# tum-pbs/DMCF

Measured on AMD Instinct MI355X. Metric: rollout_particle_steps_per_sec, higher is better.
Workload: dtype f32

## Files before the change

dmcf_amd/_lib.py:

```python
import ctypes
import os
import subprocess

_PKG = os.path.dirname(os.path.abspath(__file__))
LIB_PATH = os.path.join(_PKG, "libdmcf_hip.so")
_lib = None


class DmcfError(RuntimeError):
    pass


class CconvArgs(ctypes.Structure):
    _fields_ = [
        ("filters", ctypes.c_void_p),
        ("filter_dims", ctypes.c_int32 * 5),
        ("sym_axis", ctypes.c_int32),
        ("out_positions", ctypes.c_void_p),
        ("n_out", ctypes.c_int64),
        ("inp_positions", ctypes.c_void_p),
        ("n_inp", ctypes.c_int64),
        ("inp_features", ctypes.c_void_p),
        ("inp_importance", ctypes.c_void_p),
        ("neighbors_index", ctypes.c_void_p),
        ("neighbors_row_splits", ctypes.c_void_p),
        ("neighbors_value", ctypes.c_void_p),
        ("extent", ctypes.c_float),
        ("window_fac", ctypes.c_float),
        ("window", ctypes.c_int32),
        ("coordinate_mapping", ctypes.c_int32),
        ("interpolation", ctypes.c_int32),
        ("flags", ctypes.c_int32),
        ("bias", ctypes.c_void_p),
        ("out", ctypes.c_void_p),
        ("n_pairs", ctypes.c_int64),
        ("neighbors_row_count", ctypes.c_void_p),
        ("filter_tile_mask", ctypes.c_uint32),
        ("row_length_hint", ctypes.c_int32),
    ]


class CconvBackwardArgs(ctypes.Structure):
    _fields_ = [
        ("struct_size", ctypes.c_uint32),
        ("flags", ctypes.c_int32),
        ("grad_out", ctypes.c_void_p),
        ("inv_index", ctypes.c_void_p),
        ("inv_pair", ctypes.c_void_p),
        ("inv_row_splits", ctypes.c_void_p),
        ("inv_n_rows", ctypes.c_int64),
        ("inv_n_pairs", ctypes.c_int64),
        ("grad_filters", ctypes.c_void_p),
        ("grad_inp_features", ctypes.c_void_p),
    ]


class NeighborDenseArgs(ctypes.Structure):
    _fields_ = [
        ("struct_size", ctypes.c_uint32),
        ("flags", ctypes.c_int32),
        ("x", ctypes.c_void_p),
        ("n_in", ctypes.c_int64),
        ("cin", ctypes.c_int32),
        ("cout", ctypes.c_int32),
        ("kernel", ctypes.c_void_p),
        ("bias", ctypes.c_void_p),
        ("residual", ctypes.c_void_p),
        ("mask", ctypes.c_void_p),
        ("neighbors_index", ctypes.c_void_p),
        ("neighbors_row_splits", ctypes.c_void_p),
        ("neighbors_row_count", ctypes.c_void_p),
        ("n_out", ctypes.c_int64),
        ("n_pairs", ctypes.c_int64),
        ("host_row_splits", ctypes.c_void_p),
        ("out", ctypes.c_void_p),
        ("record_s", ctypes.c_void_p),
        ("record_count", ctypes.c_void_p),
    ]


class NeighborDenseBackwardArgs(ctypes.Structure):
    _fields_ = [
        ("struct_size", ctypes.c_uint32),
        ("flags", ctypes.c_int32),
        ("x", ctypes.c_void_p),
        ("n_in", ctypes.c_int64),
        ("cin", ctypes.c_int32),
        ("cout", ctypes.c_int32),
        ("kernel", ctypes.c_void_p),
        ("grad_out", ctypes.c_void_p),
        ("n_out", ctypes.c_int64),
# ... 63 lines not shown
        ("bias", ctypes.c_void_p),
        ("out", ctypes.c_void_p),
        ("error_flag", ctypes.c_void_p),
    ]


class AdamTensor(ctypes.Structure):
    _fields_ = [
        ("param", ctypes.c_void_p),
        ("grad", ctypes.c_void_p),
        ("m", ctypes.c_void_p),
        ("v", ctypes.c_void_p),
        ("n", ctypes.c_int64),
    ]


class AdamArgs(ctypes.Structure):
    _fields_ = [
        ("struct_size", ctypes.c_uint32),
        ("n_tensors", ctypes.c_int32),
        ("tensors", ctypes.c_void_p),
        ("device_tensors", ctypes.c_void_p),
        ("lr", ctypes.c_float),
        ("beta_1", ctypes.c_float),
        ("beta_2", ctypes.c_float),
        ("epsilon", ctypes.c_float),
        ("beta_1_power", ctypes.c_float),
        ("beta_2_power", ctypes.c_float),
        ("clip_norm", ctypes.c_float),
        ("reserved", ctypes.c_int32),
    ]


class Sph1dParams(ctypes.Structure):
    _fields_ = [
        ("struct_size", ctypes.c_uint32),
        ("bcnt", ctypes.c_int32),
        ("max_iter", ctypes.c_int32),
        ("reserved", ctypes.c_int32),
        ("h", ctypes.c_double),
        ("rest_dens", ctypes.c_double),
        ("stiffness", ctypes.c_double),
        ("visc", ctypes.c_double),
        ("gravity", ctypes.c_double),
        ("dt", ctypes.c_double),
        ("eps", ctypes.c_double),
    ]


SYMBOLS = [
    "dmcf_version", "dmcf_error_string", "dmcf_last_hip_error",
    "dmcf_frs_workspace_bytes", "dmcf_frs_build", "dmcf_frs_count", "dmcf_frs_write", "dmcf_frs_search_padded", "dmcf_frs_window_sum",
    "dmcf_radius_search_count", "dmcf_radius_search_write",
    "dmcf_cconv_workspace_bytes", "dmcf_cconv_forward", "dmcf_cconv_kernel_name",
    "dmcf_cconv_forward_extents", "dmcf_cconv_extents_kernel_name",
    "dmcf_invert_neighbors_list_workspace_bytes", "dmcf_invert_neighbors_list",
    "dmcf_cconv_backward_workspace_bytes", "dmcf_cconv_backward", "dmcf_cconv_backward_kernel_names",
    "dmcf_cconv_backward_extents", "dmcf_cconv_backward_extents_kernel_names",
    "dmcf_cconv_scatter_plan_bytes", "dmcf_cconv_scatter_plan", "dmcf_cconv_scatter_workspace_bytes", "dmcf_cconv_scatter_forward",
    "dmcf_lattice_conv_workspace_bytes", "dmcf_lattice_conv_forward",
    "dmcf_lattice_conv_batch_workspace_bytes", "dmcf_lattice_conv_forward_batch",
    "dmcf_lattice_conv_backward_workspace_bytes", "dmcf_lattice_conv_backward",
    "dmcf_reduce_subarrays_sum", "dmcf_points_aabb_workspace_bytes", "dmcf_points_aabb", "dmcf_dense_forward",
    "dmcf_fps_workspace_bytes", "dmcf_farthest_point_sample", "dmcf_gather_point",
    "dmcf_grid_pos_workspace_bytes", "dmcf_grid_pos_bounds", "dmcf_grid_pos_count", "dmcf_grid_pos_write",
    "dmcf_ghost_workspace_bytes", "dmcf_ghost_count", "dmcf_ghost_write",
    "dmcf_nn_distance_workspace_bytes", "dmcf_nn_distance", "dmcf_approx_match_workspace_bytes", "dmcf_approx_match",
    "dmcf_match_cost_workspace_bytes", "dmcf_match_cost", "dmcf_emd_workspace_bytes", "dmcf_emd",
    "dmcf_neighbor_dense_forward", "dmcf_neighbor_dense_backward_workspace_bytes", "dmcf_neighbor_dense_backward",
    "dmcf_neighbor_dense_kernel_names", "dmcf_adam_step_workspace_bytes", "dmcf_adam_step", "dmcf_adam_step_kernel_names",
    "dmcf_raster_workspace_bytes", "dmcf_raster_count", "dmcf_raster_discs",
    "dmcf_nn_distance_backward_workspace_bytes", "dmcf_nn_distance_backward", "dmcf_match_cost_backward_workspace_bytes",
    "dmcf_match_cost_backward", "dmcf_emd_with_levels", "dmcf_emd_backward_workspace_bytes", "dmcf_emd_backward",
    "dmcf_gather_point_backward_workspace_bytes", "dmcf_gather_point_backward",
    "dmcf_frs_window_sum_backward",
    "dmcf_sph1d_rollout",
]


def build(force=False):
    csrc = os.path.join(_PKG, "csrc")
    args = ["make", "-C", csrc, "-j4"]
    if force:
        args.append("-B")
    subprocess.check_call(args, stdout=subprocess.DEVNULL)
    return LIB_PATH


def lib():
    global _lib
    if _lib is not None:
        return _lib
    if not os.path.exists(LIB_PATH):
        raise DmcfError(
            f"{LIB_PATH} is missing: the HIP extension has not been built "
            "(run `python -c 'import __graft_entry__ as g; g.build()'`). There is no CPU fallback.")
    L = ctypes.CDLL(LIB_PATH)
    c = ctypes
    L.dmcf_version.restype = c.c_int
    L.dmcf_error_string.restype = c.c_char_p
    L.dmcf_error_string.argtypes = [c.c_int]
    L.dmcf_last_hip_error.restype = c.c_int
    L.dmcf_frs_workspace_bytes.restype = c.c_size_t
    L.dmcf_frs_workspace_bytes.argtypes = [c.c_int64, c.c_int64]
    L.dmcf_frs_build.restype = c.c_int
    L.dmcf_frs_build.argtypes = [c.c_void_p, c.c_int64, c.c_float, c.c_void_p, c.c_size_t, c.c_void_p]
    L.dmcf_frs_count.restype = c.c_int
    L.dmcf_frs_count.argtypes = [c.c_void_p, c.c_int64, c.c_int64, c.c_float, c.c_int, c.c_void_p, c.c_size_t,
                                 c.c_void_p, c.c_void_p]
    L.dmcf_frs_write.restype = c.c_int
    L.dmcf_frs_write.argtypes = [c.c_void_p, c.c_int64, c.c_int64, c.c_float, c.c_int, c.c_void_p, c.c_size_t,
                                 c.c_void_p, c.c_void_p, c.c_void_p, c.c_int64, c.c_void_p]
    L.dmcf_frs_search_padded.restype = c.c_int
    L.dmcf_frs_search_padded.argtypes = [c.c_void_p, c.c_int64, c.c_int64, c.c_float, c.c_int, c.c_void_p, c.c_size_t, c.c_int64,
                                         c.c_void_p, c.c_void_p, c.c_void_p, c.c_void_p, c.c_void_p, c.c_void_p]
    L.dmcf_frs_window_sum.restype = c.c_int
    L.dmcf_frs_window_sum.argtypes = [c.c_void_p, c.c_int64, c.c_int64, c.c_float, c.c_int, c.c_int, c.c_void_p, c.c_size_t,
                                      c.c_void_p, c.c_void_p]
    L.dmcf_radius_search_count.restype = c.c_int
    L.dmcf_radius_search_count.argtypes = [c.c_void_p, c.c_int64, c.c_int64, c.c_void_p, c.c_float, c.c_int, c.c_void_p, c.c_size_t,
                                           c.c_void_p, c.c_void_p]
    L.dmcf_radius_search_write.restype = c.c_int
    L.dmcf_radius_search_write.argtypes = [c.c_void_p, c.c_int64, c.c_int64, c.c_void_p, c.c_float, c.c_int, c.c_void_p, c.c_size_t,
                                           c.c_void_p, c.c_void_p, c.c_void_p, c.c_int64, c.c_void_p]
    L.dmcf_cconv_workspace_bytes.restype = c.c_size_t
    L.dmcf_cconv_workspace_bytes.argtypes = [c.POINTER(CconvArgs)]
    L.dmcf_cconv_forward.restype = c.c_int
    L.dmcf_cconv_forward.argtypes = [c.POINTER(CconvArgs), c.c_void_p, c.c_size_t, c.c_void_p]
    L.dmcf_cconv_kernel_name.restype = c.c_int
    L.dmcf_cconv_kernel_name.argtypes = [c.POINTER(CconvArgs), c.c_char_p, c.c_size_t]
    L.dmcf_cconv_forward_extents.restype = c.c_int
    L.dmcf_cconv_forward_extents.argtypes = [c.POINTER(CconvArgs), c.c_void_p, c.c_void_p, c.c_size_t, c.c_void_p]
    L.dmcf_cconv_extents_kernel_name.restype = c.c_int
    L.dmcf_cconv_extents_kernel_name.argtypes = [c.POINTER(CconvArgs), c.c_char_p, c.c_size_t]
    L.dmcf_invert_neighbors_list_workspace_bytes.restype = c.c_size_t
    L.dmcf_invert_neighbors_list_workspace_bytes.argtypes = [c.c_int64]
    L.dmcf_invert_neighbors_list.restype = c.c_int
    L.dmcf_invert_neighbors_list.argtypes = [c.c_int64, c.c_void_p, c.c_void_p, c.c_void_p, c.c_int64, c.c_int64, c.c_void_p,
                                             c.c_void_p, c.c_void_p, c.c_void_p, c.c_void_p, c.c_void_p, c.c_size_t, c.c_void_p]
    L.dmcf_cconv_backward_workspace_bytes.restype = c.c_size_t
    L.dmcf_cconv_backward_workspace_bytes.argtypes = [c.POINTER(CconvArgs), c.POINTER(CconvBackwardArgs)]
    L.dmcf_cconv_backward.restype = c.c_int
    L.dmcf_cconv_backward.argtypes = [c.POINTER(CconvArgs), c.POINTER(CconvBackwardArgs), c.c_void_p, c.c_size_t, c.c_void_p]
    L.dmcf_cconv_backward_kernel_names.restype = c.c_int
    L.dmcf_cconv_backward_kernel_names.argtypes = [c.POINTER(CconvArgs), c.POINTER(CconvBackwardArgs), c.c_char_p, c.c_size_t]
    L.dmcf_cconv_backward_extents.restype = c.c_int
    L.dmcf_cconv_backward_extents.argtypes = [c.POINTER(CconvArgs), c.POINTER(CconvBackwardArgs), c.c_void_p, c.c_void_p, c.c_size_t,
                                              c.c_void_p]
    L.dmcf_cconv_backward_extents_kernel_names.restype = c.c_int
    L.dmcf_cconv_backward_extents_kernel_names.argtypes = [c.POINTER(CconvArgs), c.POINTER(CconvBackwardArgs), c.c_char_p, c.c_size_t]
    L.dmcf_cconv_scatter_plan_bytes.restype = c.c_size_t
    L.dmcf_cconv_scatter_plan_bytes.argtypes = [c.c_int64]
    L.dmcf_cconv_scatter_plan.restype = c.c_int
    L.dmcf_cconv_scatter_plan.argtypes = [c.c_void_p, c.c_int64, c.c_void_p, c.c_int64, c.c_float, c.c_float, c.c_int32, c.c_void_p,
                                          c.c_size_t, c.c_void_p]
    L.dmcf_cconv_scatter_workspace_bytes.restype = c.c_size_t
    L.dmcf_cconv_scatter_workspace_bytes.argtypes = [c.POINTER(CconvScatterArgs)]
    L.dmcf_cconv_scatter_forward.restype = c.c_int
    L.dmcf_cconv_scatter_forward.argtypes = [c.POINTER(CconvScatterArgs), c.c_void_p, c.c_size_t, c.c_void_p]
    L.dmcf_lattice_conv_workspace_bytes.restype = c.c_size_t
    L.dmcf_lattice_conv_workspace_bytes.argtypes = [c.POINTER(LatticeConvArgs)]
    L.dmcf_lattice_conv_forward.restype = c.c_int
    L.dmcf_lattice_conv_forward.argtypes = [c.POINTER(LatticeConvArgs), c.c_void_p, c.c_size_t, c.c_void_p]
    L.dmcf_lattice_conv_batch_workspace_bytes.restype = c.c_size_t
    L.dmcf_lattice_conv_batch_workspace_bytes.argtypes = [c.POINTER(LatticeConvArgs), c.c_int32]
    L.dmcf_lattice_conv_forward_batch.restype = c.c_int
    L.dmcf_lattice_conv_forward_batch.argtypes = [c.POINTER(LatticeConvArgs), c.c_int32, c.c_void_p, c.c_size_t, c.c_void_p]
    L.dmcf_lattice_conv_backward_workspace_bytes.restype = c.c_size_t
    L.dmcf_lattice_conv_backward_workspace_bytes.argtypes = [c.POINTER(LatticeConvArgs), c.c_int32]
    L.dmcf_lattice_conv_backward.restype = c.c_int
    L.dmcf_lattice_conv_backward.argtypes = [c.POINTER(LatticeConvArgs), c.c_int32, c.c_void_p, c.c_void_p, c.c_void_p, c.c_void_p,
                                             c.c_size_t, c.c_void_p]
    L.dmcf_dense_forward.restype = c.c_int
    L.dmcf_dense_forward.argtypes = [c.c_void_p, c.c_int64, c.c_int32, c.c_void_p, c.c_int32, c.c_void_p, c.c_void_p, c.c_void_p,
                                     c.c_void_p]
    L.dmcf_ghost_workspace_bytes.restype = c.c_size_t
    L.dmcf_ghost_workspace_bytes.argtypes = [c.c_int64, c.c_int32, c.c_int32]
    L.dmcf_ghost_count.restype = c.c_int
    L.dmcf_ghost_count.argtypes = [c.c_void_p, c.c_int64, c.c_void_p, c.c_int32, c.c_void_p, c.c_int32, c.c_void_p, c.c_void_p,
                                   c.c_size_t, c.c_void_p]
    L.dmcf_ghost_write.restype = c.c_int
    L.dmcf_ghost_write.argtypes = [c.c_void_p, c.c_int64, c.c_void_p, c.c_int32, c.c_void_p, c.c_int32, c.c_void_p, c.c_void_p,
                                   c.c_void_p, c.c_void_p, c.c_size_t, c.c_void_p]
# ... 98 lines not shown
```

dmcf_amd/csrc/cconv.hip:

```cpp
#include <type_traits>

#include <stdio.h>

#include "cconv_common.h"

namespace dmcf {

constexpr int kThreads = 512;
constexpr int kWaves = kThreads / 64;
constexpr int TM = 16;
constexpr int kMaxNT = 4;
constexpr int kWStride = 8;
constexpr int kFStride = 8;
constexpr int kStage = 64 * (kWStride + kFStride + 1);


template <int CC, bool GENERIC>
__global__ __launch_bounds__(kThreads, 4) void cconv_kernel(const CconvParams p) {
    constexpr bool EXT = false;
    const float* const out_ext = nullptr;
#include "cconv_generic_body.inc"
}

template <int CC>
// ... 73 lines not shown
        const size_t kcp = KCx + ((4 - KCx % 64) + 64) % 64;
        size_t bf = (size_t)TM * kcp;
        const size_t rf = (size_t)kWaves * TM * 16 * ((cout + 15) / 16);
        if (bf < rf) bf = rf;
        return (bf + TM + (size_t)kWaves * kStage + (has_dead ? 2 * kThreads : 0)) * sizeof(float);
    };
    const int PS0 = (PR + 7) / 8 * 8;
    const size_t step = lds_bytes(PS0) <= 80 * 1024 ? 80 * 1024 : 160 * 1024;
    int best = PS0, best_bad = 1 << 30, best_group = 0;
    for (int zgroup = 0; zgroup < 2 && best_bad > 0; ++zgroup)
        for (int k = 0; k < 12; ++k) {
            const int PS = PS0 + 8 * k;
            if (k > 0 && (sz < 2 || lds_bytes(PS) > step)) break;
            const int bad = conflicts(PS, zgroup);
            if (bad < best_bad) { best_bad = bad; best = PS; best_group = zgroup; }
            if (bad == 0) break;
        }
    c.PS = best;
    c.zgroup = best_group;
    const int KC = (sz * c.PS + 15) / 16 * 16;
    c.nblocks = KC / 16;
    c.KCp = KC + ((4 - KC % 64) + 64) % 64;
    c.NT = (cout + 15) / 16;
    c.nchunks = (cin + c.CC - 1) / c.CC;
    size_t b_floats = (size_t)TM * c.KCp;
    const size_t red_floats = (size_t)kWaves * TM * 16 * c.NT;
    if (b_floats < red_floats) b_floats = red_floats;
    c.bfloats = b_floats;
    c.lds = lds_bytes(c.PS);
    c.packed_floats = (size_t)c.nchunks * c.nblocks * 4 * c.NT * 16 * 4;
    return c;
}

}

using namespace dmcf;

extern "C" {

static int validate(const dmcf_cconv_args* a, bool forward = true) {
    if (!a) return DMCF_EINVAL;
    for (int d = 0; d < 5; ++d)
        if (a->filter_dims[d] < 1) return DMCF_EINVAL;
    if (a->n_out < 0 || a->n_inp < 0) return DMCF_EINVAL;
    if (!(a->extent > 0.0f)) return DMCF_EINVAL;
    if (a->window < DMCF_WINDOW_NONE || a->window > DMCF_WINDOW_CUBIC_GRAD) return DMCF_EINVAL;
    if (a->coordinate_mapping < 0 || a->coordinate_mapping > 2) return DMCF_EINVAL;
    if (a->interpolation < 0 || a->interpolation > 2) return DMCF_EINVAL;
    if (a->flags & DMCF_FLAG_SYMMETRIC) {
        if (a->sym_axis < 0 || a->sym_axis > 2) return DMCF_EINVAL;
        if (a->n_inp < a->n_out) return DMCF_EINVAL;
    }
    if (a->filter_dims[4] > 16 * kMaxNT) return DMCF_EUNSUPPORTED;
    if (a->n_out > 0) {
        if (!a->out_positions || !a->neighbors_row_splits) return DMCF_EINVAL;
        if (forward && (!a->filters || !a->out || !a->inp_features)) return DMCF_EINVAL;
        if (a->window == DMCF_WINDOW_EXPLICIT && !a->neighbors_value) return DMCF_EINVAL;
    }
    return DMCF_OK;
}

static void full_dims(const dmcf_cconv_args* a, int& dz, int& dy, int& dx) {
    dz = a->filter_dims[0]; dy = a->filter_dims[1]; dx = a->filter_dims[2];
    if (a->flags & DMCF_FLAG_SYMMETRIC) {
        if (a->sym_axis == 0) dz *= 2;
        if (a->sym_axis == 1) dy *= 2;
        if (a->sym_axis == 2) dx *= 2;
    }
}

static void fill_params(const dmcf_cconv_args* a, int dz, int dy, int dx, CconvParams& p) {
    p.partial = nullptr;
    p.csplit = 0;
    p.cin = a->filter_dims[3];
    p.cout = a->filter_dims[4];
    p.sx = dx; p.sy = dy; p.sz = dz;
    p.K = dx * dy * dz;
    p.out_pos = a->out_positions;
    p.inp_pos = a->inp_positions;
    p.inp_feat = a->inp_features;
    p.inp_imp = a->inp_importance;
    p.idx = a->neighbors_index;
    p.rs = a->neighbors_row_splits;
    p.cnt = a->neighbors_row_count;
    p.wmask = (a->filter_tile_mask && a->filter_dims[3] <= 32 && a->filter_dims[4] <= 64) ? a->filter_tile_mask : 0xffffffffu;
    p.nval = a->neighbors_value;
    p.n_out = a->n_out;
    p.n_inp = a->n_inp;
    p.pair_cap = a->n_pairs;
    p.inv_extent = 1.0f / a->extent;
    const float radius = 0.5f * a->extent;
    p.inv_r2 = 1.0f / (radius * radius);
    p.window_fac = a->window_fac;
    p.window = a->window;
    p.mapping = a->coordinate_mapping;
    p.interp = a->interpolation;
    p.flags = a->flags;
    p.bias = a->bias;
    p.out = a->out;
}

static void generic_pick(const dmcf_cconv_args* a, int dz, int dy, int dx, bool ext, CconvPick& k) {
    const LaunchCfg cfg = make_cfg(dx, dy, dz, a->filter_dims[3], a->filter_dims[4]);
    const bool generic = !cconv_specialised(a);
    CconvKernel f;
    if (ext)
// ... 3 lines not shown
    else
        f = {generic ? (const void*)cconv_kernel<4, true> : (const void*)cconv_kernel<4, false>, "cconv_kernel<4>"};
    k = {f.fn, f.name, cfg.lds, kThreads, cfg.packed_floats};
}

static int generic_launch(CconvParams p, const dmcf_cconv_args* a, int dz, int dy, int dx, const CconvPick& k, const float* out_ext,
                          void* workspace, hipStream_t stream) {
    const LaunchCfg cfg = make_cfg(dx, dy, dz, p.cin, p.cout);
    if (cfg.lds > 160 * 1024) return DMCF_EUNSUPPORTED;
    float* packed = (float*)workspace;
    const unsigned g = (unsigned)((cfg.packed_floats + 255) / 256);
    if (out_ext || !(a->flags & DMCF_FLAG_FILTER_PACKED))
        hipLaunchKernelGGL(pack_filter, dim3(g < 2048u ? g : 2048u), dim3(256), 0, stream, a->filters, packed, dz, dy, dx,
                           p.cin, p.cout, cfg.CC, cfg.PS, cfg.nchunks, cfg.nblocks, cfg.NT,
                           (a->flags & DMCF_FLAG_SYMMETRIC) ? 1 : 0, a->sym_axis);
    p.Wp = packed;
    p.KCp = cfg.KCp;
    p.PS = cfg.PS;
    p.zgroup = cfg.zgroup;
    p.nblocks = cfg.nblocks;
    p.NT = cfg.NT;
    p.nchunks = cfg.nchunks;
    p.bfloats = (int)cfg.bfloats;
    if (!cconv_set_tiles(p, TM)) return DMCF_EUNSUPPORTED;
    void* kargs[] = {(void*)&p, (void*)&out_ext};
    return cconv_launch_kernel(k, dim3((unsigned)p.tiles_per_xcd * 8u), kargs, stream);
}

static const CconvForm generic_form = {
    0, [](const dmcf_cconv_args*, int, int, int, bool) { return true; },
    [](const dmcf_cconv_args* a, int dz, int dy, int dx, CconvPick& k) { generic_pick(a, dz, dy, dx, false, k); },
    [](const dmcf_cconv_args* a, int dz, int dy, int dx, bool) {
        return make_cfg(dx, dy, dz, a->filter_dims[3], a->filter_dims[4]).packed_floats;
    },
    [](CconvParams p, const dmcf_cconv_args* a, int dz, int dy, int dx, const CconvPick& k, void* workspace, hipStream_t stream) {
        return generic_launch(p, a, dz, dy, dx, k, nullptr, workspace, stream);
    }};

static const CconvForm* const kForms[] = {&cconv_direct_form, &cconv_ws_form,  &cconv_pair_form, &cconv_p16_form, &cconv_z3_form,
                                          &cconv_cls_form,    &cconv_blk_form, &cconv_mfma_form, &generic_form};

static bool form_accepts(const CconvForm& f, const dmcf_cconv_args* a, int dz, int dy, int dx, int forced) {
    if (f.key && forced >= 0 && forced != f.key) return false;
    return f.eligible(a, dz, dy, dx, forced >= 0);
}

static int cconv_select(const dmcf_cconv_args* a, int dz, int dy, int dx, const CconvForm*& form, CconvPick& k) {
    const int forced = cconv_forced_key();
    for (const CconvForm* f : kForms) {
        if (!form_accepts(*f, a, dz, dy, dx, forced)) continue;
        if ((a->flags & DMCF_FLAG_SKIP_SELF) && f != &cconv_direct_form) return DMCF_EUNSUPPORTED;
        form = f;
        f->pick(a, dz, dy, dx, k);
        return DMCF_OK;
    }
    return DMCF_EUNSUPPORTED;
}

size_t dmcf_cconv_workspace_bytes(const dmcf_cconv_args* a) {
    if (!a || validate(a) != DMCF_OK) return 256;
    int dz, dy, dx;
    full_dims(a, dz, dy, dx);
    const int forced = cconv_forced_key();
    size_t floats = 0;
    for (const CconvForm* f : kForms) {
        const size_t ff = f->workspace_floats(a, dz, dy, dx, form_accepts(*f, a, dz, dy, dx, forced));
        if (floats < ff) floats = ff;
    }
    return 256 + align_up(floats * sizeof(float), 256);
}

int dmcf_cconv_forward(const dmcf_cconv_args* a, void* workspace, size_t workspace_bytes, dmcf_stream_t stream_) {
    int rc = validate(a);
    if (rc != DMCF_OK) return rc;
    if (a->n_out == 0) return DMCF_OK;
    if (!workspace || ((uintptr_t)workspace & 255)) return DMCF_EINVAL;
    if (workspace_bytes < dmcf_cconv_workspace_bytes(a)) return DMCF_EWORKSPACE;

    CconvParams p;
    int dz, dy, dx;
    full_dims(a, dz, dy, dx);
    fill_params(a, dz, dy, dx, p);
    const CconvForm* form;
    CconvPick k;
    rc = cconv_select(a, dz, dy, dx, form, k);
    if (rc != DMCF_OK) return rc;
    return form->launch(p, a, dz, dy, dx, k, workspace, (hipStream_t)stream_);
}

static int validate_extents(const dmcf_cconv_args* a, const float* out_extents, dmcf_cconv_args& b) {
    if (!a) return DMCF_EINVAL;
    b = *a;
    b.extent = 1.0f;
    const int rc = validate(&b);
    if (rc != DMCF_OK) return rc;
    if (a->flags & DMCF_FLAG_SKIP_SELF) return DMCF_EUNSUPPORTED;
    if (a->n_out > 0 && !out_extents) return DMCF_EINVAL;
    return DMCF_OK;
}

int dmcf_cconv_forward_extents(const dmcf_cconv_args* a, const float* out_extents, void* workspace, size_t workspace_bytes,
                               dmcf_stream_t stream_) {
    hipStream_t stream = (hipStream_t)stream_;
    dmcf_cconv_args b;
    const int rc = validate_extents(a, out_extents, b);
    if (rc != DMCF_OK) return rc;
    if (b.n_out == 0) return DMCF_OK;
    if (!workspace || ((uintptr_t)workspace & 255)) return DMCF_EINVAL;
    if (workspace_bytes < dmcf_cconv_workspace_bytes(&b)) return DMCF_EWORKSPACE;
    CconvParams p;
    int dz, dy, dx;
    full_dims(&b, dz, dy, dx);
    fill_params(&b, dz, dy, dx, p);
    CconvPick k;
    generic_pick(&b, dz, dy, dx, true, k);
    return generic_launch(p, &b, dz, dy, dx, k, out_extents, workspace, stream);
}

int dmcf_cconv_kernel_name(const dmcf_cconv_args* a, char* name, size_t name_bytes) {
    if (!name || name_bytes < 2) return DMCF_EINVAL;
    int rc = validate(a, false);
    if (rc != DMCF_OK) return rc;
    int dz, dy, dx;
    full_dims(a, dz, dy, dx);
    const CconvForm* form;
    CconvPick k;
    rc = cconv_select(a, dz, dy, dx, form, k);
    if (rc != DMCF_OK) return rc;
    snprintf(name, name_bytes, "%s", k.name);
    return DMCF_OK;
}

int dmcf_cconv_extents_kernel_name(const dmcf_cconv_args* a, char* name, size_t name_bytes) {
    if (!name || name_bytes < 2 || !a) return DMCF_EINVAL;
    dmcf_cconv_args b = *a;
    b.extent = 1.0f;
    const int rc = validate(&b, false);
    if (rc != DMCF_OK) return rc;
    if (a->flags & DMCF_FLAG_SKIP_SELF) return DMCF_EUNSUPPORTED;
    int dz, dy, dx;
    full_dims(&b, dz, dy, dx);
    CconvPick k;
    generic_pick(&b, dz, dy, dx, true, k);
    snprintf(name, name_bytes, "%s", k.name);
    return DMCF_OK;
}

}
```

dmcf_amd/csrc/cconv_cls.hip:

```cpp

#include "cconv_common.h"

namespace dmcf {

constexpr int kCWaves = 8;
constexpr int kCThreads = 64 * kCWaves;
constexpr int CTM = 2 * kCWaves;
constexpr int kCRows = 16;
constexpr int CCH = 16;
constexpr int kCRow = 1024;
constexpr int kSlots = 96;
constexpr int kHalfSlots = 48;
constexpr int kGrp = 20;
constexpr int kXst = 512;
constexpr int kCMaxNT = 4;
constexpr int kNoPair = 9;

#define CLS_TILE_REGS                                                                                                     \
    "v92", "v93", "v94", "v95", "v96", "v97", "v98", "v99", "v100", "v101", "v102", "v103", "v104", "v105", "v106", "v107", \
        "v108", "v109", "v110", "v111", "v112", "v113", "v114", "v115", "v116", "v117", "v118", "v119", "v120", "v121",    \
        "v122", "v123", "v124", "v125", "v126", "v127"
constexpr int kClsCompilerVgprs = 46;

__device__ __forceinline__ void cls_zero_tiles() {
    asm volatile(
        "v_mov_b32 v92, 0\n\tv_mov_b32 v93, 0\n\tv_mov_b32 v94, 0\n\tv_mov_b32 v95, 0\n\t"
        "v_mov_b32 v96, 0\n\tv_mov_b32 v97, 0\n\tv_mov_b32 v98, 0\n\tv_mov_b32 v99, 0\n\t"
        "v_mov_b32 v100, 0\n\tv_mov_b32 v101, 0\n\tv_mov_b32 v102, 0\n\tv_mov_b32 v103, 0\n\t"
        "v_mov_b32 v104, 0\n\tv_mov_b32 v105, 0\n\tv_mov_b32 v106, 0\n\tv_mov_b32 v107, 0\n\t"
        "v_mov_b32 v108, 0\n\tv_mov_b32 v109, 0\n\tv_mov_b32 v110, 0\n\tv_mov_b32 v111, 0\n\t"
        "v_mov_b32 v112, 0\n\tv_mov_b32 v113, 0\n\tv_mov_b32 v114, 0\n\tv_mov_b32 v115, 0\n\t"
        "v_mov_b32 v116, 0\n\tv_mov_b32 v117, 0\n\tv_mov_b32 v118, 0\n\tv_mov_b32 v119, 0\n\t"
        "v_mov_b32 v120, 0\n\tv_mov_b32 v121, 0\n\tv_mov_b32 v122, 0\n\tv_mov_b32 v123, 0\n\t"
        "v_mov_b32 v124, 0\n\tv_mov_b32 v125, 0\n\tv_mov_b32 v126, 0\n\tv_mov_b32 v127, 0"
        ::: "memory", CLS_TILE_REGS);
}

struct ClsRec {
    float x;
    f32x4 w;
};

__device__ __forceinline__ uint32_t cls_lds_addr(const void* q) {
    return (uint32_t)(uintptr_t)(const __attribute__((address_space(3))) void*)q;
}

__device__ __forceinline__ void xfence() {
    __builtin_amdgcn_fence(__ATOMIC_RELEASE, "wavefront");
    __builtin_amdgcn_wave_barrier();
    __builtin_amdgcn_fence(__ATOMIC_ACQUIRE, "wavefront");
}

template <int NTT, bool NARROW, bool SYM, bool SINGLE, bool PLAIN>
__global__ __launch_bounds__(kCThreads, 4) __attribute__((amdgpu_num_vgpr(kClsCompilerVgprs))) void cconv_cls_kernel(const CconvParams p) {
    extern __shared__ __attribute__((aligned(16))) float smem[];
    const int tid = threadIdx.x, lane = tid & 63;
    const int wave = __builtin_amdgcn_readfirstlane(tid >> 6);
    const int cin = p.cin, cout = p.cout;
    float* Bt = smem;
    float* Gs = smem + CTM * kCRow + wave * kXst;
    unsigned char* Cst = (unsigned char*)(Gs + 24 * kGrp);
    float* Fst = Bt + (wave + kCWaves) * kCRow;
    int* Jst = (int*)(Fst + kHalfSlots * 16);
    const int tile = (int)(blockIdx.x % 8) * p.tiles_per_xcd + (int)(blockIdx.x / 8);
    if (tile >= p.ntiles) return;
    const int64_t pt0 = (int64_t)tile * CTM;
    const int window = PLAIN ? (int)DMCF_WINDOW_POLY6 : p.window;
    const float* const nval = PLAIN ? nullptr : p.nval;
    const float* const imp = PLAIN ? nullptr : p.inp_imp;
    constexpr bool symmetric = SYM;

    const int mk = lane >> 4, mn = lane & 15;
    const float xm = (float)(lane & 3);
    const int widx = (lane >> 2) & 3;
    const int mi = lane & 15, mg = lane >> 4;
    const uint32_t gs_lds = cls_lds_addr(Gs), fst_lds = cls_lds_addr(Fst);
    constexpr uint32_t kOob = 0xffffffffu;
    const uint32_t rowB = (uint32_t)cin * 4u;
    const __amdgpu_buffer_rsrc_t rF = __builtin_amdgcn_make_buffer_rsrc((void*)p.inp_feat, 0, (int)((uint32_t)p.n_inp * rowB), 0x00020000);

    f32x4 acc[NTT];
#pragma unroll
    for (int n = 0; n < NTT; ++n) acc[n] = (f32x4){0.0f, 0.0f, 0.0f, 0.0f};

    float out_prev = 0.0f;
    for (int chunk = 0; chunk < p.nchunks; ++chunk) {
        const int c0 = chunk * CCH;
        const int nch = min(CCH, cin - c0);
        constexpr bool narrow = NARROW;
        const int fr = narrow ? lane >> 1 : lane >> 2, fc4 = narrow ? lane & 1 : lane & 3;
        const int spi = narrow ? 32 : 16;
        const int fstride = narrow ? 8 : 16;
        const bool fch_ok = c0 + 4 * fc4 < cin;
        const int fch = fch_ok ? c0 + 4 * fc4 : 0;
        int64_t rbs[2];
        int nts[2], nbs[2];
        float oxs[2], oys[2], ozs[2];
#pragma unroll
        for (int pp = 0; pp < 2; ++pp) {
            const int64_t i = pt0 + wave + kCWaves * pp;
            rbs[pp] = 0;
            nts[pp] = 0;
            oxs[pp] = oys[pp] = ozs[pp] = 0.0f;
            if (i < p.n_out) {
                const int64_t rb = p.rs[i];
                int64_t re = p.cnt ? rb + p.cnt[i] : p.rs[i + 1];
                if (re > p.pair_cap) re = rb;
                rbs[pp] = rb;
                nts[pp] = (int)min(re - rb, (int64_t)0x7fffffc0);
                oxs[pp] = p.out_pos[3 * i];
                oys[pp] = p.out_pos[3 * i + 1];
                ozs[pp] = p.out_pos[3 * i + 2];
            }
            nbs[pp] = (nts[pp] + 63) >> 6;
        }
        const int nbA = nbs[0], NB = nbs[0] + nbs[1];
        cls_zero_tiles();

        const int nt0 = __builtin_amdgcn_readfirstlane(nts[0]), nt1 = __builtin_amdgcn_readfirstlane(nts[1]);
        const int64_t rb0 = ((int64_t)__builtin_amdgcn_readfirstlane((int)(rbs[0] >> 32)) << 32) | (uint32_t)__builtin_amdgcn_readfirstlane((int)rbs[0]);
        const int64_t rb1 = ((int64_t)__builtin_amdgcn_readfirstlane((int)(rbs[1] >> 32)) << 32) | (uint32_t)__builtin_amdgcn_readfirstlane((int)rbs[1]);
        const int64_t gapB = nt1 > 0 ? rb1 - rb0 : 0;
        const bool near = gapB >= 0 && gapB + nt1 < ((int64_t)1 << 29) && nt0 < (1 << 29);
        const __amdgpu_buffer_rsrc_t rI = __builtin_amdgcn_make_buffer_rsrc(
            (void*)(p.idx + rb0), 0, near ? (int)(max((int64_t)nt0, gapB + nt1) * 4) : 0, 0x00020000);
        const uint32_t offB = (uint32_t)gapB * 4u;
        auto valid = [&](int t) -> bool {
            const bool pp = t >= nbA;
            return t < NB && 64 * (t - (pp ? nbA : 0)) + lane < (pp ? nt1 : nt0);
        };
        auto ld_idx = [&](int t, int& j, float& nv) {
            const bool pp = t >= nbA, ok = valid(t);
            const int o = 64 * (t - (pp ? nbA : 0)) + lane;
            j = 0;
            nv = 0.0f;
            if (near) {
                j = (int)__builtin_amdgcn_raw_buffer_load_b32(rI, ok ? (uint32_t)o * 4u + (pp ? offB : 0u) : kOob, 0, 0);
            } else if (ok) {
                j = p.idx[(pp ? rb1 : rb0) + o];
            }
            if (nval && ok) nv = nval[(pp ? rb1 : rb0) + o];
        };
        auto ld_pos = [&](int j, float& x, float& y, float& z) {
            const float* q = (const float*)((const char*)p.inp_pos + (size_t)__umul24((uint32_t)j, 12u));
            x = q[0];
            y = q[1];
            z = q[2];
        };
        auto geom = [&](int t, int j, float nv, float x, float y, float z, int& cls) -> ClsRec {
            ClsRec c;
            const bool pp = t >= nbA;
            x -= pp ? oxs[1] : oxs[0];
            y -= pp ? oys[1] : oys[0];
            z -= pp ? ozs[1] : ozs[0];
            float a = window_value(window, nval ? nv : rel_dist2(x, y, z), p.inv_r2, p.window_fac);
            if (imp) a *= imp[j];
            filter_coords<false>(x, y, z, p);
            c.x = fminf(3.0f, fmaxf(0.0f, x));
            y = fminf(3.0f, fmaxf(0.0f, y));
            z = fminf(3.0f, fmaxf(0.0f, z));
            const float yf = fminf(floorf(y), 2.0f), zf = fminf(floorf(z), 2.0f);
            const float fy = y - yf, fz = z - zf;
            cls = valid(t) ? 3 * (int)zf + (int)yf : kNoPair;
            const float a0 = a * (1.0f - fz), a1 = a * fz;
            c.w = (f32x4){a0 * (1.0f - fy), a0 * fy, a1 * (1.0f - fy), a1 * fy};
            return c;
        };
        struct Order {
            int pos;
            int cb[10];
        };
        auto order = [&](int cls) -> Order {
            Order o;
            o.pos = 0;
            int base = 0;
#pragma unroll
            for (int c = 0; c < 9; ++c) {
                const uint64_t m = __ballot(cls == c);
                const int rank = __builtin_amdgcn_mbcnt_hi((uint32_t)(m >> 32), __builtin_amdgcn_mbcnt_lo((uint32_t)m, base));
                o.pos = cls == c ? rank : o.pos;
                o.cb[c] = base;
                base += (__builtin_popcountll(m) + 3) & ~3;
            }
            o.cb[9] = base;
            return o;
        };
        auto push_index = [&](int j, int cls, int pos) {
            Jst[lane] = -1;
            if (lane < kSlots - 64) Jst[64 + lane] = -1;
            xfence();
            if (cls != kNoPair) Jst[pos] = (int)__umul24((uint32_t)j, rowB);
        };
        auto push_rec = [&](const ClsRec& c, int cls, int pos) {
            *(f32x4*)(Gs + 4 * lane) = (f32x4){0.0f, 0.0f, 0.0f, 0.0f};
            if (lane < kGrp * 6 - 64) *(f32x4*)(Gs + 4 * (64 + lane)) = (f32x4){0.0f, 0.0f, 0.0f, 0.0f};
            xfence();
            if (cls != kNoPair) {
                float* g = Gs + (pos >> 2) * kGrp + (pos & 3);
                g[16] = c.x;
                *(f32x4*)(g + 3 * (pos & 3)) = c.w;
                if ((pos & 3) == 0) Cst[pos >> 2] = (unsigned char)(4 * cls);
            }
        };
        const uint32_t cbyte = fch_ok ? 4u * (uint32_t)fch : kOob;
        auto f_issue = [&](int h, f32x4 (&f)[3]) {
            uint32_t jo[3];
#pragma unroll
            for (int k = 0; k < 3; ++k) jo[k] = (uint32_t)Jst[kHalfSlots * h + spi * k + fr];
#pragma unroll
            for (int k = 0; k < 3; ++k)
// ... 44 lines not shown
            __builtin_amdgcn_s_setprio(3);
            asm volatile(
#include "cconv_cls_splat8.inc"
                : [xa] "=&v"(xa), [wa] "=&v"(wa), [fa] "=&v"(fa), [xb] "=&v"(xb), [wb] "=&v"(wb), [fb] "=&v"(fb),
                  [a] "=&v"(av), [sc] "=&s"(sc)
                : [px] "v"(px), [pw] "v"(pw), [pf] "v"(pf), [xm] "v"(xm), [ng] "s"(ng), [c0] "s"(c[0]), [c1] "s"(c[1]),
                  [c2] "s"(c[2]), [c3] "s"(c[3]), [c4] "s"(c[4]), [c5] "s"(c[5])
                : "scc", "m0", "memory", CLS_TILE_REGS);
            __builtin_amdgcn_s_setprio(0);
        };
        auto merge = [&](int pt) {
            float* Brow = Bt + pt * kCRow;
            const int gz = lane >> 5, gy = (lane >> 4) & 1;
            const int col = (mn ^ (pt & 15)) << 2;
            const uint32_t mb = cls_lds_addr(Brow + (gz * 4 + gy) * 64 + col);
            xfence();
            asm volatile(
                "s_nop 7\n\ts_nop 7\n\ts_nop 7\n\t"
                "ds_write_b128 %[b], v[92:95] offset:0\n\t"
                "ds_write_b128 %[b], v[100:103] offset:512\n\t"
                "ds_write_b128 %[b], v[116:119] offset:2048\n\t"
                "ds_write_b128 %[b], v[124:127] offset:2560\n\t"
                "ds_read_b128 v[92:95], %[b] offset:256\n\t"
                "s_waitcnt lgkmcnt(0)\n\t"
                "v_add_f32 v92, v92, v96\n\tv_add_f32 v93, v93, v97\n\tv_add_f32 v94, v94, v98\n\tv_add_f32 v95, v95, v99\n\t"
                "ds_write_b128 %[b], v[92:95] offset:256\n\t"
                "ds_read_b128 v[92:95], %[b] offset:2304\n\t"
                "s_waitcnt lgkmcnt(0)\n\t"
                "v_add_f32 v92, v92, v120\n\tv_add_f32 v93, v93, v121\n\tv_add_f32 v94, v94, v122\n\tv_add_f32 v95, v95, v123\n\t"
                "ds_write_b128 %[b], v[92:95] offset:2304\n\t"
                "ds_read_b128 v[92:95], %[b] offset:1024\n\t"
                "s_waitcnt lgkmcnt(0)\n\t"
                "v_add_f32 v92, v92, v104\n\tv_add_f32 v93, v93, v105\n\tv_add_f32 v94, v94, v106\n\tv_add_f32 v95, v95, v107\n\t"
                "ds_write_b128 %[b], v[92:95] offset:1024\n\t"
                "ds_read_b128 v[92:95], %[b] offset:1536\n\t"
                "s_waitcnt lgkmcnt(0)\n\t"
                "v_add_f32 v92, v92, v112\n\tv_add_f32 v93, v93, v113\n\tv_add_f32 v94, v94, v114\n\tv_add_f32 v95, v95, v115\n\t"
                "ds_write_b128 %[b], v[92:95] offset:1536\n\t"
                "ds_read_b128 v[92:95], %[b] offset:1280\n\t"
                "s_waitcnt lgkmcnt(0)\n\t"
                "v_add_f32 v92, v92, v108\n\tv_add_f32 v93, v93, v109\n\tv_add_f32 v94, v94, v110\n\tv_add_f32 v95, v95, v111\n\t"
                "ds_write_b128 %[b], v[92:95] offset:1280\n\t"
                "s_waitcnt lgkmcnt(0)"
                :
                : [b] "v"(mb)
                : "memory", CLS_TILE_REGS);
            cls_zero_tiles();
            xfence();
        };

        if (nbA == 0) merge(wave);
        if (NB > 0) {
            int jA, jB, cl;
            float nvA, nvB, px, py, pz;
            ld_idx(0, jA, nvA);
            ld_idx(1, jB, nvB);
            ld_pos(jA, px, py, pz);
            const ClsRec first = geom(0, jA, nvA, px, py, pz, cl);
            Order oc = order(cl);
            f32x4 ff[3];
            push_index(jA, cl, oc.pos);
            push_rec(first, cl, oc.pos);
            xfence();
            f_issue(0, ff);
            jA = jB;
            nvA = nvB;
            ld_pos(jA, px, py, pz);
            if constexpr (narrow) {
                for (int t = 0; t + 1 < NB; ++t) {
                    const int nslots = oc.cb[9];
                    f_publish(t, ff);
                    ld_idx(t + 2, jB, nvB);
                    const ClsRec nxt = geom(t + 1, jA, nvA, px, py, pz, cl);
                    const Order on = order(cl);
                    push_index(jA, cl, on.pos);
                    jA = jB;
                    nvA = nvB;
                    ld_pos(jA, px, py, pz);
                    xfence();
                    f_issue(0, ff);
                    splat8(nslots);
                    push_rec(nxt, cl, on.pos);
                    oc = on;
                    if (t == nbA - 1) merge(wave);
                }
                f_publish(NB - 1, ff);
                xfence();
                splat8(oc.cb[9]);
                if (NB - 1 == nbA - 1) merge(wave);
            } else {
                for (int t = 0; t + 1 < NB; ++t) {
                    const int nslots = oc.cb[9];
                    const bool two = nslots > kHalfSlots;
                    f_publish(t, ff);
                    ld_idx(t + 2, jB, nvB);
                    if (two) f_issue(1, ff);
                    xfence();
                    splat(0, nslots);
                    const ClsRec nxt = geom(t + 1, jA, nvA, px, py, pz, cl);
                    const Order on = order(cl);
                    push_index(jA, cl, on.pos);
                    xfence();
                    if (two) f_publish(t, ff);
                    jA = jB;
                    nvA = nvB;
                    ld_pos(jA, px, py, pz);
                    f_issue(0, ff);
                    if (two) {
                        xfence();
                        splat(1, nslots);
                    }
                    push_rec(nxt, cl, on.pos);
                    oc = on;
                    if (t == nbA - 1) merge(wave);
                }
                {
                    const int nslots = oc.cb[9];
                    const bool two = nslots > kHalfSlots;
                    f_publish(NB - 1, ff);
                    if (two) f_issue(1, ff);
                    xfence();
                    splat(0, nslots);
                    if (two) {
                        xfence();
                        f_publish(NB - 1, ff);
                        xfence();
                        splat(1, nslots);
                    }
                    if (NB - 1 == nbA - 1) merge(wave);
                }
            }
        }
        if (chunk == p.nchunks - 1) out_prev = epilogue_prefetch(p, pt0, CTM, tid);
        const int nq = (nch + 3) >> 2;
        constexpr int kIt = 64 / kCWaves;
        constexpr int kPre = SINGLE ? (NTT <= 1 ? 8 : (NTT <= 2 ? 4 : 2)) : (NTT <= 1 ? 4 : (NTT <= 2 ? 2 : 1));
        const __amdgpu_buffer_rsrc_t rW = __builtin_amdgcn_make_buffer_rsrc(
            (void*)p.Wp, 0, (int)((uint32_t)p.nchunks * 64u * (uint32_t)p.NT * 1024u), 0x00020000);
        const uint32_t w_lane = ((uint32_t)mg * (uint32_t)p.NT * 16u + (uint32_t)mi) * 16u;
        auto w_issue = [&](int it0, f32x4 (&bw)[kPre][NTT]) {
#pragma unroll
            for (int q = 0; q < kPre; ++q) {
                const int t = wave + kCWaves * (it0 + q);
                if (t < 16 * nq) {
                    int tq, tr;
                    blk_divmod(t, nq, tq, tr);
                    const int blk = tq * 4 + tr;
                    const uint32_t w_blk = (uint32_t)(chunk * 64 + blk) * (uint32_t)p.NT * 1024u;
                    const int wq = 4 * chunk + tr;
                    const uint32_t wm = wq < 8 ? p.wmask >> (4 * wq) : 0xfu;
#pragma unroll
                    for (int n = 0; n < NTT; ++n)
                        if (n < p.NT && ((wm >> n) & 1))
                            bw[q][n] = __builtin_bit_cast(f32x4, __builtin_amdgcn_raw_buffer_load_b128(rW, w_lane, w_blk + 256u * (uint32_t)n, 0));
                }
            }
        };
        f32x4 bw[kPre][NTT];
#pragma unroll
// ... 74 lines not shown
                       (symmetric && sym_axis == 2) ? 2 : 4};
    for (int64_t e = (int64_t)blockIdx.x * blockDim.x + threadIdx.x; e < total; e += (int64_t)gridDim.x * blockDim.x) {
        int64_t s = e;
        const int q = (int)(s & 3); s >>= 2;
        const int j = (int)(s & 15); s >>= 4;
        const int n = (int)(s % NT); s /= NT;
        const int g = (int)(s & 3); s >>= 2;
        const int blk = (int)(s & 63); s >>= 6;
        const int chunk = (int)s;
        const int ci = chunk * CCH + 4 * (blk & 3) + g, o = 16 * n + j;
        float v = 0.0f;
        if (chunk < nchunks && ci < cin && o < cout) {
            int c3[3] = {blk >> 4, (blk >> 2) & 3, q};
            float sign = 1.0f;
            if (symmetric) {
                const int hh = hd[sym_axis];
                if (c3[sym_axis] >= hh) {
                    c3[sym_axis] -= hh;
                } else {
                    sign = -1.0f;
                    for (int a = 0; a < 3; ++a) c3[a] = hd[a] - 1 - c3[a];
                }
            }
            v = sign * src[((((int64_t)c3[0] * hd[1] + c3[1]) * hd[2] + c3[2]) * cin + ci) * cout + o];
        }
        dst[e] = v;
    }
}

static bool cls_eligible(const dmcf_cconv_args* a, int dz, int dy, int dx, bool forced) {
    if (!cconv_fast444(a, dz, dy, dx) || !cconv_offsets_fit_24bit(a)) return false;
    if (a->filter_dims[4] > 16 * kCMaxNT) return false;
    if (forced) return true;
    return a->filter_dims[3] >= 8;
}

size_t cconv_cls_workspace_floats(const dmcf_cconv_args* a, int, int, int, bool) {
    return cconv_cls_packed_floats(a->filter_dims[3], a->filter_dims[4]);
}

bool cconv_cls_prepare(CconvParams& p, const dmcf_cconv_args* a, int tm, void* workspace, hipStream_t stream) {
    float* packed = (float*)workspace;
    p.NT = (p.cout + 15) / 16;
    p.nchunks = (p.cin + CCH - 1) / CCH;
    const int64_t total = (int64_t)cconv_cls_packed_floats(p.cin, p.cout);
    const unsigned g = (unsigned)((total + 255) / 256);
    if (!(a->flags & DMCF_FLAG_FILTER_PACKED))
        hipLaunchKernelGGL(pack_filter_cls, dim3(g < 2048u ? g : 2048u), dim3(256), 0, stream, a->filters, packed, p.cin, p.cout,
                           p.nchunks, p.NT, (a->flags & DMCF_FLAG_SYMMETRIC) ? 1 : 0, a->sym_axis);
    p.Wp = packed;
    return cconv_set_tiles(p, tm);
}

static void cls_pick(const dmcf_cconv_args* a, int, int, int, CconvPick& k) {
    const int cin = a->filter_dims[3], NT = (a->filter_dims[4] + 15) / 16;
    const bool sym = (a->flags & DMCF_FLAG_SYMMETRIC) != 0;
    const bool plain = !sym && cconv_plain(a);
#define CLS_PICK(NARROW, SINGLE)                                                                \
    (sym ? CCONV_KERNEL_NT(NT, cconv_cls_kernel, NARROW, true, SINGLE, false)                   \
         : (plain ? CCONV_KERNEL_NT(NT, cconv_cls_kernel, NARROW, false, SINGLE, true)          \
                  : CCONV_KERNEL_NT(NT, cconv_cls_kernel, NARROW, false, SINGLE, false)))
    const CconvKernel f = cin <= 8 ? CLS_PICK(true, true) : (cin <= CCH ? CLS_PICK(false, true) : CLS_PICK(false, false));
#undef CLS_PICK
    k = {f.fn, f.name, kClsLds, kCThreads, cconv_cls_packed_floats(cin, a->filter_dims[4])};
}

static int cls_launch(CconvParams p, const dmcf_cconv_args* a, int, int, int, const CconvPick& k, void* workspace, hipStream_t stream) {
    if (!cconv_cls_prepare(p, a, CTM, workspace, stream)) return DMCF_EUNSUPPORTED;
    void* kargs[] = {(void*)&p};
    return cconv_launch_kernel(k, dim3((unsigned)p.tiles_per_xcd * 8u), kargs, stream);
}

CconvForm cconv_cls_form = {'c', cls_eligible, cls_pick, cconv_cls_workspace_floats, cls_launch};

}
```

dmcf_amd/csrc/cconv_common.h:

```cpp
#pragma once
#include <stdlib.h>

#include "common.h"

namespace dmcf {

typedef float f32x4_t __attribute__((ext_vector_type(4)));

struct CconvParams {
    const float* Wp;
    int sx, sy, sz, K, cin, cout;
    const float* out_pos;
    const float* inp_pos;
    const float* inp_feat;
    const float* inp_imp;
    const int32_t* idx;
    const int64_t* rs;
    const int32_t* cnt;
    const float* nval;
    int64_t n_out;
    int64_t n_inp;
    int64_t pair_cap;
    float inv_extent, inv_r2, window_fac;
    int window, mapping, interp, flags;
// ... 124 lines not shown
            if (q <= 1.0f) r = (s <= 0.5f) ? 18.0f * q - 12.0f * s : -6.0f * (1.0f - s) * (1.0f - s);
            return fac * (4.0f / 3.0f) * r;
        }
    }
    return 1.0f;
}

__device__ __forceinline__ void axis_weights(float x, int s, int interp, int& b, float& w0, float& w1) {
    const int bmax = s >= 2 ? s - 2 : 0;
    if (interp == DMCF_INTERP_NEAREST) {
        int c = (int)roundf(x);
        c = min(max(c, 0), s - 1);
        b = min(c, bmax);
        w0 = (c == b) ? 1.0f : 0.0f;
        w1 = 1.0f - w0;
        return;
    }
    if (interp == DMCF_INTERP_LINEAR) {
        x = fminf((float)(s - 1), fmaxf(0.0f, x));
        const float xf = fminf(floorf(x), (float)bmax);
        b = (int)xf;
        const float a = x - xf;
        w0 = 1.0f - a;
        w1 = a;
        if (s == 1) { w0 = 1.0f; w1 = 0.0f; }
        return;
    }
    const float xf = floorf(x);
    const float a = x - xf;
    const float c0 = xf, c1 = xf + 1.0f;
    const bool in0 = c0 >= 0.0f && c0 <= (float)(s - 1), in1 = c1 >= 0.0f && c1 <= (float)(s - 1);
    const float v0 = in0 ? 1.0f - a : 0.0f, v1 = in1 ? a : 0.0f;
    if (!in0 && !in1) { b = 0; w0 = w1 = 0.0f; return; }
    if (in0 && in1) { b = (int)c0; w0 = v0; w1 = v1; return; }
    if (in0) {
        if (s >= 2) { b = s - 2; w0 = 0.0f; w1 = v0; } else { b = 0; w0 = v0; w1 = 0.0f; }
        return;
    }
    b = 0; w0 = v1; w1 = 0.0f;
}

__device__ __forceinline__ void axis_weights_linear(float x, int s, int& b, float& w0, float& w1) {
    const float bmax = (float)(s >= 2 ? s - 2 : 0);
    x = fminf((float)(s - 1), fmaxf(0.0f, x));
    const float xf = fminf(floorf(x), bmax);
    b = (int)xf;
    const float a = x - xf;
    w0 = 1.0f - a;
    w1 = a;
}

typedef float f32x4 __attribute__((ext_vector_type(4)));
typedef float f32x2 __attribute__((ext_vector_type(2)));

__device__ __forceinline__ void blk_divmod(int t, int nq, int& quot, int& rem) {
    const int m = nq == 1 ? 128 : (nq == 2 ? 64 : (nq == 3 ? 43 : 32));
    quot = (t * m) >> 7;
    rem = t - quot * nq;
}



__global__ void pack_filter(const float* __restrict__ src, float* __restrict__ dst, int d0, int d1, int d2, int cin,
                            int cout, int CC, int PS, int nchunks, int nblocks, int NT, int symmetric, int sym_axis);

__device__ __forceinline__ float epilogue_prefetch(const CconvParams& p, int64_t pt0, int pts, int tid) {
    if (!(p.flags & DMCF_FLAG_ACCUMULATE)) return 0.0f;
    const int64_t lim = min((int64_t)pts, p.n_out - pt0) * p.cout;
    return tid < lim ? p.out[pt0 * p.cout + tid] : 0.0f;
}


struct CconvPick {
    const void* fn;
    const char* name;
    size_t lds;
    int threads;
    size_t packed_floats;
};

struct CconvKernel {
    const void* fn;
    const char* name;
};
#define CCONV_KERNEL(...) CconvKernel{(const void*)__VA_ARGS__, #__VA_ARGS__}
#define CCONV_KERNEL_NT(nt, K, ...) \
    ((nt) <= 1 ? CCONV_KERNEL(K<1, __VA_ARGS__>) : ((nt) <= 2 ? CCONV_KERNEL(K<2, __VA_ARGS__>) : CCONV_KERNEL(K<4, __VA_ARGS__>)))

struct CconvForm {
    char key;
    bool (*eligible)(const dmcf_cconv_args* a, int dz, int dy, int dx, bool forced);
    void (*pick)(const dmcf_cconv_args* a, int dz, int dy, int dx, CconvPick& k);
    size_t (*workspace_floats)(const dmcf_cconv_args* a, int dz, int dy, int dx, bool selectable);
    int (*launch)(CconvParams p, const dmcf_cconv_args* a, int dz, int dy, int dx, const CconvPick& k, void* workspace,
                  hipStream_t stream);
};
extern CconvForm cconv_direct_form, cconv_ws_form, cconv_pair_form, cconv_p16_form, cconv_z3_form, cconv_cls_form,
    cconv_blk_form, cconv_mfma_form;

inline int cconv_forced_key() {
    const char* e = getenv("DMCF_CCONV_KERNEL");
    return e ? (unsigned char)e[0] : -1;
}

inline bool cconv_specialised(const dmcf_cconv_args* a) {
    return a->coordinate_mapping == DMCF_MAP_BALL_TO_CUBE_VOLUME_PRESERVING && a->interpolation == DMCF_INTERP_LINEAR &&
           (a->flags & DMCF_FLAG_ALIGN_CORNERS);
}

inline bool cconv_fast444(const dmcf_cconv_args* a, int dz, int dy, int dx) {
    return dx == 4 && dy == 4 && dz == 4 && cconv_specialised(a) && !(a->flags & DMCF_FLAG_NORMALIZE) && !(a->filter_dims[3] & 3) &&
           !((uintptr_t)a->inp_features & 15);
}

inline bool cconv_offsets_fit_24bit(const dmcf_cconv_args* a) {
    return a->n_inp < (1 << 24) && a->n_inp * (int64_t)a->filter_dims[3] * 4 < ((int64_t)1 << 31);
}

inline bool cconv_plain(const dmcf_cconv_args* a) {
    return a->window == DMCF_WINDOW_POLY6 && !a->neighbors_value && !a->inp_importance;
}

inline bool cconv_set_tiles(CconvParams& p, int tm) {
    const int64_t ntiles = (p.n_out + tm - 1) / tm;
    if (ntiles > 0x7fffffff / 8) return false;
    p.ntiles = (int)ntiles;
    p.tiles_per_xcd = (int)((ntiles + 7) / 8);
    return true;
}

inline int cconv_launch_kernel(const CconvPick& k, dim3 grid, void** kargs, hipStream_t stream) {
    hipError_t e = hipFuncSetAttribute(k.fn, hipFuncAttributeMaxDynamicSharedMemorySize, (int)k.lds);
// ... 14 lines not shown
```

dmcf_amd/csrc/cconv_ws.hip:

```cpp

#include "cconv_common.h"

namespace dmcf {

#ifdef WS_TRACE
__device__ unsigned long long g_wtrace[32];
#define WT(k) { const uint64_t now_ = __builtin_readcyclecounter(); wt[k] += now_ - wlast; wlast = now_; }
#else
#define WT(k)
#endif

constexpr int kWProd = 4, kWCons = 4;
constexpr int kWThreads = 64 * (kWProd + kWCons);
constexpr int WTM = 16;
constexpr int kWPts = WTM / kWProd;
constexpr int kWRow = 2048;
constexpr int kWRecG = 36;
constexpr int kWRec = 16 * kWRecG;
constexpr int kWWaveF = kWRec + 64 + 384;
constexpr int kWMaxNT = 2;
constexpr int kWRed = 2 * kWCons * WTM * 16 * kWMaxNT;
constexpr int kWCompilerVgprs = 56;

#define WS_FIXED_REGS                                                                                                      \
// ... 31 lines not shown
};

constexpr uint32_t kWOob = 0xffffffffu;

typedef const __attribute__((address_space(4))) CconvParams* WsKP;

__device__ __forceinline__ void ws_filter_coords(float& x, float& y, float& z, float inv_extent) {
    const float s = 2.0f * inv_extent;
    x *= s; y *= s; z *= s;
    sphere_to_cyl(x, y, z);
    cyl_to_cube(x, y);
    x *= 0.5f; y *= 0.5f; z *= 0.5f;
    x = (x + 0.5f) * 3.0f;
    y = (y + 0.5f) * 3.0f;
    z = (z + 0.5f) * 3.0f;
}

#define WS_PULL(IT, ADDR) \
    asm volatile("ds_read_b128 v[128+4*(" #IT "):128+4*(" #IT ")+3], %0" ::"v"(ADDR) : "memory", WS_FIXED_REGS)
#define WS_MFMA(IT, N, BV)                                                                                                  \
    asm volatile("v_mfma_f32_16x16x4_f32 v[112+4*" #N ":112+4*" #N "+3], v[128+4*(" #IT ")+0], %0, v[112+4*" #N ":112+4*" #N "+3]\n\t" \
                 "v_mfma_f32_16x16x4_f32 v[112+4*" #N ":112+4*" #N "+3], v[128+4*(" #IT ")+1], %1, v[112+4*" #N ":112+4*" #N "+3]\n\t" \
                 "v_mfma_f32_16x16x4_f32 v[112+4*" #N ":112+4*" #N "+3], v[128+4*(" #IT ")+2], %2, v[112+4*" #N ":112+4*" #N "+3]\n\t" \
                 "v_mfma_f32_16x16x4_f32 v[112+4*" #N ":112+4*" #N "+3], v[128+4*(" #IT ")+3], %3, v[112+4*" #N ":112+4*" #N "+3]"       \
                 :                                                                                                          \
                 : "v"((BV).x), "v"((BV).y), "v"((BV).z), "v"((BV).w)                                                      \
                 : WS_FIXED_REGS)
#define WS_MFMA2(IT, BV0, BV1)                                                                                              \
    asm volatile("v_mfma_f32_16x16x4_f32 v[112:115], v[128+4*(" #IT ")+0], %0, v[112:115]\n\t"                               \
                 "v_mfma_f32_16x16x4_f32 v[116:119], v[128+4*(" #IT ")+0], %4, v[116:119]\n\t"                               \
                 "v_mfma_f32_16x16x4_f32 v[112:115], v[128+4*(" #IT ")+1], %1, v[112:115]\n\t"                               \
                 "v_mfma_f32_16x16x4_f32 v[116:119], v[128+4*(" #IT ")+1], %5, v[116:119]\n\t"                               \
                 "v_mfma_f32_16x16x4_f32 v[112:115], v[128+4*(" #IT ")+2], %2, v[112:115]\n\t"                               \
                 "v_mfma_f32_16x16x4_f32 v[116:119], v[128+4*(" #IT ")+2], %6, v[116:119]\n\t"                               \
                 "v_mfma_f32_16x16x4_f32 v[112:115], v[128+4*(" #IT ")+3], %3, v[112:115]\n\t"                               \
                 "v_mfma_f32_16x16x4_f32 v[116:119], v[128+4*(" #IT ")+3], %7, v[116:119]"                                    \
                 :                                                                                                          \
                 : "v"((BV0).x), "v"((BV0).y), "v"((BV0).z), "v"((BV0).w), "v"((BV1).x), "v"((BV1).y), "v"((BV1).z), "v"((BV1).w) \
                 : WS_FIXED_REGS)
#define WS_ACC_READ(N, DST)                                                                                                 \
    asm volatile("v_mov_b32 %0, v[112+4*" #N "+0]\n\tv_mov_b32 %1, v[112+4*" #N "+1]\n\tv_mov_b32 %2, v[112+4*" #N "+2]\n\t"     \
                 "v_mov_b32 %3, v[112+4*" #N "+3]"                                                                          \
                 : "=v"((DST).x), "=v"((DST).y), "=v"((DST).z), "=v"((DST).w)                                             \
                 :                                                                                                          \
                 : WS_FIXED_REGS)



struct WsRing {
    int start, end, rblo, rbhi, span;
};

__device__ __forceinline__ void ws_ld_idx(int sp, int r4, int o1, int o2, int o3, const float* Tab, __amdgpu_buffer_rsrc_t rI, const float* nval,
                                          int64_t rb0, int& j, float& nv, int& kk) {
    kk = (r4 + (sp >= o1 ? 1 : 0) + (sp >= o2 ? 1 : 0) + (sp >= o3 ? 1 : 0)) & 63;
    const f32x2 ed = *(const f32x2*)(Tab + 2 * kk);
    const int e = __float_as_int(ed.x), d = __float_as_int(ed.y);
    const bool ok = sp < e;
    const uint32_t o = (uint32_t)sp * 4u + (uint32_t)d;
    j = (int)__builtin_amdgcn_raw_buffer_load_b32(rI, ok ? o : kWOob, 0, 0);
    nv = 0.0f;
    if (nval && ok) nv = nval[rb0 + (o >> 2)];
}

__device__ __forceinline__ void ws_ld_pos(const float* inp_pos, int j, float& x, float& y, float& z) {
    const float* q = (const float*)((const char*)inp_pos + (size_t)__umul24((uint32_t)j, 12u));
    x = q[0];
    y = q[1];
    z = q[2];
}

__device__ __forceinline__ WsRec ws_geom(int sp, int kk, const float* Tab, int window, const float* nval, const float* imp,
                                         float inv_r2, float window_fac, float inv_extent, int j, float nv, float x, float y, float z, bool& ok) {
    WsRec c;
    const f32x4 o = *(const f32x4*)(Tab + 128 + 4 * kk);
    ok = sp < __float_as_int(o.w);
    x -= o.x;
    y -= o.y;
    z -= o.z;
    float a = window_value(window, nval ? nv : rel_dist2(x, y, z), inv_r2, window_fac);
    if (imp) a *= imp[j];
    a = ok ? a : 0.0f;
    ws_filter_coords(x, y, z, inv_extent);
    x = fminf(3.0f, fmaxf(0.0f, x));
    y = fminf(3.0f, fmaxf(0.0f, y));
    z = fminf(3.0f, fmaxf(0.0f, z));
    const float xf = fminf(floorf(x), 2.0f), yf = fminf(floorf(y), 2.0f), zf = fminf(floorf(z), 2.0f);
    const float fx = x - xf, fy = y - yf, fz = z - zf;
    c.cls4 = ok ? 4 * (((int)zf * 3 + (int)yf) * 3 + (int)xf) : 0;
    const float a0 = a * (1.0f - fz), a1 = a * fz;
    const float y00 = (1.0f - fy) * (1.0f - fx), y01 = (1.0f - fy) * fx, y10 = fy * (1.0f - fx), y11 = fy * fx;
    c.lo = (f32x4){a0 * y00, a0 * y01, a0 * y10, a0 * y11};
    c.hi = (f32x4){a1 * y00, a1 * y01, a1 * y10, a1 * y11};
    return c;
}

__device__ __forceinline__ void ws_refill(WsKP kp0, int wi, int lane, int wave, int t_begin, int t_end, int nslots, float* Tab, int& stream_end,
                                          WsRing& ring) {
    WsKP kp = kp0;
    asm volatile("" : "+s"(kp));
    const int lb = 32 * (wi & 1);
    const bool act = (unsigned)(lane - lb) < 32u;
    const int r = 32 * wi + (lane - lb);
    const int tile = t_begin + (r >> 2) * nslots;
    const int64_t i = (int64_t)tile * WTM + kWPts * wave + (r & 3);
    int64_t rb = 0;
    int nt = 0;
    float ox = 0.0f, oy = 0.0f, oz = 0.0f;
    if (act && tile < t_end && i < kp->n_out) {
        const int64_t* const rs = kp->rs;
        const int32_t* const cnt = kp->cnt;
        const float* const out_pos = kp->out_pos;
        const int64_t b = rs[i];
        int64_t e = cnt ? b + cnt[i] : rs[i + 1];
        if (e > kp->pair_cap) e = b;
        rb = b;
        nt = (int)min(e - b, (int64_t)0x01ffffc0);
        ox = out_pos[3 * i];
        oy = out_pos[3 * i + 1];
        oz = out_pos[3 * i + 2];
    }
    const int slots = (max(nt, 1) + 7) & ~7;
    const int q = lane & 3;
    const int s1 = __shfl_up(slots, 1), s2 = __shfl_up(slots, 2), s3 = __shfl_up(slots, 3);
    const int intra = (q >= 1 ? s1 : 0) + (q >= 2 ? s2 : 0) + (q >= 3 ? s3 : 0);
    const int ttot = (__shfl(intra + slots, lane | 3) + 63) & ~63;
    int tp = 0, wtot = 0;
#pragma unroll
    for (int m = 0; m < 8; ++m) {
        const int tm = __builtin_amdgcn_readlane(ttot, lb + 4 * m);
        if (((lane - lb) >> 2) > m) tp += tm;
        wtot += tm;
    }
    const int start = stream_end + tp + intra;
    const int64_t rb0 = ((int64_t)__shfl((int)(rb >> 32), lane & ~3) << 32) | (uint32_t)__shfl((int)rb, lane & ~3);
    const int64_t gap = nt > 0 ? rb - rb0 : 0;
    if (__builtin_amdgcn_ballot_w64(act && (gap < 0 || gap + nt >= ((int64_t)1 << 29))) != 0) __builtin_trap();
    int sp = (int)gap + nt;
    sp = max(sp, __shfl_xor(sp, 1));
    sp = max(sp, __shfl_xor(sp, 2));
    if (act) {
        const int e = start + nt;
        const int d = (int)(((uint32_t)(int)gap - (uint32_t)start) * 4u);
        *(f32x2*)(Tab + 2 * lane) = (f32x2){__int_as_float(e), __int_as_float(d)};
        *(f32x4*)(Tab + 128 + 4 * lane) = (f32x4){ox, oy, oz, __int_as_float(e)};
        ring.start = start;
        ring.end = e;
        ring.rblo = (int)rb0;
        ring.rbhi = (int)(rb0 >> 32);
        ring.span = sp;
    }
    stream_end += wtot;
    wfence();
}

template <int NTT, bool PLAIN>
__global__ __launch_bounds__(kWThreads, 1) __attribute__((amdgpu_num_vgpr(kWCompilerVgprs))) void cconv_ws_kernel(const CconvParams p_arg) {
    extern __shared__ __attribute__((aligned(16))) float smem[];
    const WsKP kp0 = (WsKP)__builtin_amdgcn_kernarg_segment_ptr();
    const int tid = threadIdx.x, lane = tid & 63;
    const int wave = wsgpr(tid >> 6);
    const int cin = kp0->cin, cout = kp0->cout;
    float* Bt = smem;
    const int xcd = (int)(blockIdx.x & 7), slot = (int)(blockIdx.x >> 3), nslots = (int)(gridDim.x >> 3);
    const int t_begin = xcd * kp0->tiles_per_xcd + slot;
    const int t_end = min((xcd + 1) * kp0->tiles_per_xcd, kp0->ntiles);
    if (t_begin >= t_end) return;

    if (wave < kWProd) {
        float* Rec = smem + WTM * kWRow + wave * kWWaveF;
        uint32_t* Jof = (uint32_t*)(Rec + kWRec);
        float* Tab = Rec + kWRec + 64;
        float* Fst = Bt + (kWPts * wave + kWPts - 1) * kWRow;
        const int ch = lane & 31, half = lane >> 5;
        const int fr = lane >> 3, fq = lane & 7;
        const uint32_t rowBy = (uint32_t)cin * 4u;
        const uint32_t cbyte = 4 * fq < cin ? 16u * (uint32_t)fq : kWOob;
        const int pg = fr >> 2, ptq = fr & 3;
        float* const w01 = Fst + pg * 128 + 4 * fq + ptq;
        float* const w23 = Fst + pg * 128 + 4 * ((fq + 4) & 7) + ptq;
        const uint32_t a_rec0 = wlds(Rec + 4 * (4 * half + (lane & 3)));
        const uint32_t a_fst0 = wlds(Fst + 4 * (8 * (ch & 3) + (((ch >> 2) + 4 * ((ch >> 1) & 1)) & 7)));
        const uint32_t row_lane = wlds(Bt + (ch >> 4) * 1024 + half * 512);

        asm volatile(
            ".irp r,148,150,152,154,156,158,160,162,164,166,168,170,172,174,176,178,180,182,184,186,188,190,192,194,196,198,200,202,"
            "204,206,208,210,212,214,216,218,220,222,224,226,228,230,232,234,236,238,240,242,244,246,248,250,252,254\n\t"
            "v_mov_b64 v[\\r:\\r+1], 0\n\t.endr" ::: "memory", WS_FIXED_REGS);

        const int T = (t_end - t_begin + nslots - 1) / nslots;
        WsRing ring = {0, 0, 0, 0, 0};
        int stream_end = 0;
        ws_refill(kp0, 0, lane, wave, t_begin, t_end, nslots, Tab, stream_end, ring);
        ws_refill(kp0, 1, lane, wave, t_begin, t_end, nslots, Tab, stream_end, ring);

        WsKP kp = kp0;
        asm volatile("" : "+s"(kp));
        const int window = PLAIN ? (int)DMCF_WINDOW_POLY6 : kp->window;
        const float* const nval = PLAIN ? nullptr : kp->nval;
        const float* const imp = PLAIN ? nullptr : kp->inp_imp;
        const float inv_r2 = kp->inv_r2, window_fac = kp->window_fac, inv_extent = kp->inv_extent;
        const float* const inp_pos = kp->inp_pos;
        const int32_t* const idx = kp->idx;
        const __amdgpu_buffer_rsrc_t rF = __builtin_amdgcn_make_buffer_rsrc((void*)kp->inp_feat, 0, (int)((uint32_t)kp->n_inp * rowBy), 0x00020000);

        auto push_index = [=](int j, bool ok) { Jof[lane] = ok ? __umul24((uint32_t)j, rowBy) : kWOob; };
        auto push_rec = [=](const WsRec& c) {
            float* r = Rec + (lane >> 2) * kWRecG + (lane & 3);
            r[0] = c.lo.x; r[4] = c.lo.y; r[8] = c.lo.z; r[12] = c.lo.w;
            r[16] = c.hi.x; r[20] = c.hi.y; r[24] = c.hi.z; r[28] = c.hi.w;
        };
        int pk_cur = 0;
        auto pack_classes = [=](int cls4, uint32_t (&c)[16]) -> int {
            int pk = cls4 | (__builtin_amdgcn_mov_dpp(cls4, 0xb1, 0xf, 0xf, true) << 8);
            pk = pk | (__builtin_amdgcn_mov_dpp(pk, 0x4e, 0xf, 0xf, true) << 16);
#pragma unroll
            for (int m = 0; m < 16; ++m) c[m] = (uint32_t)__builtin_amdgcn_readlane(pk, 4 * m);
            return pk;
        };
        auto f_issue = [=](int np, f32x4 (&f)[8]) {
#pragma unroll
            for (int hh = 0; hh < 2; ++hh) {
                if (hh == 0 || np > 32) {
                    uint32_t jo[4];
#pragma unroll
                    for (int r = 0; r < 4; ++r) jo[r] = Jof[8 * (4 * hh + r) + fr];
#pragma unroll
                    for (int r = 0; r < 4; ++r)
                        f[4 * hh + r] = __builtin_bit_cast(f32x4, __builtin_amdgcn_raw_buffer_load_b128(rF, __builtin_elementwise_add_sat(jo[r], cbyte), 0, 0));
                }
            }
        };
        auto f_publish = [=](int np, const f32x4 (&f)[8]) {
#pragma unroll
            for (int r = 0; r < 8; ++r) {
                if (r < 4 || np > 32) {
                    w01[256 * r] = f[r].x;
                    w01[256 * r + 32] = f[r].y;
                    w23[256 * r + 64] = f[r].z;
                    w23[256 * r + 96] = f[r].w;
                }
            }
        };
        auto splat = [=](int nblk, const uint32_t (&c)[16], uint32_t a_rec, uint32_t a_fst) {
            uint32_t s0;
            __builtin_amdgcn_s_setprio(3);
            asm volatile(
#include "cconv_pair_splat.inc"
                : [s0] "=&s"(s0)
                : [pa] "v"(a_rec), [pf] "v"(a_fst), [nb] "s"(wsgpr(nblk)), [c0] "s"(wsgpr(c[0])), [c1] "s"(wsgpr(c[1])), [c2] "s"(wsgpr(c[2])),
                  [c3] "s"(wsgpr(c[3])), [c4] "s"(wsgpr(c[4])), [c5] "s"(wsgpr(c[5])), [c6] "s"(wsgpr(c[6])), [c7] "s"(wsgpr(c[7])),
                  [c8] "s"(wsgpr(c[8])), [c9] "s"(wsgpr(c[9])), [c10] "s"(wsgpr(c[10])), [c11] "s"(wsgpr(c[11])), [c12] "s"(wsgpr(c[12])),
                  [c13] "s"(wsgpr(c[13])), [c14] "s"(wsgpr(c[14])), [c15] "s"(wsgpr(c[15]))
                : "scc", "m0", "memory", WS_FIXED_REGS);
            __builtin_amdgcn_s_setprio(0);
        };

        int tq = 0, gq = 0, o1 = 0, o2 = 0, o3 = 0, gendq = 0, elastq = 0;
        int64_t rb0q = 0;
        __amdgpu_buffer_rsrc_t rI;
#define WS_TILE_CTX()                                                                                                        \
    {                                                                                                                        \
        const int l0_ = (4 * tq) & 63;                                                                                       \
        o1 = __builtin_amdgcn_readlane(ring.start, l0_ + 1);                                                                 \
        o2 = __builtin_amdgcn_readlane(ring.start, l0_ + 2);                                                                 \
        o3 = __builtin_amdgcn_readlane(ring.start, l0_ + 3);                                                                 \
        elastq = __builtin_amdgcn_readlane(ring.end, l0_ + 3);                                                               \
        gendq = __builtin_amdgcn_readlane(ring.start, (l0_ + 4) & 63) >> 6;                                                  \
        rb0q = ((int64_t)__builtin_amdgcn_readlane(ring.rbhi, l0_) << 32) | (uint32_t)__builtin_amdgcn_readlane(ring.rblo, l0_); \
        rI = __builtin_amdgcn_make_buffer_rsrc((void*)(idx + rb0q), 0, __builtin_amdgcn_readlane(ring.span, l0_) * 4, 0x00020000); \
    }
#define WS_IDX_STAGE(J, NV, KK, NP)                                                                                          \
    {                                                                                                                        \
        if (gq >= gendq) {                                                                                                   \
            ++tq;                                                                                                            \
            WS_TILE_CTX()                                                                                                    \
        }                                                                                                                    \
        ws_ld_idx(64 * gq + lane, 4 * tq, o1, o2, o3, Tab, rI, nval, rb0q, J, NV, KK);                                       \
        NP = max(0, min(64, elastq - 64 * gq));                                                                              \
        ++gq;                                                                                                                \
    }
        WS_TILE_CTX()

        int ti = 0;
        int rdone = 0;
        auto complete = [=, &rdone]() {
            const int row = kWPts * wave + (rdone & 3);
            const uint32_t b = row_lane + (uint32_t)row * (kWRow * 4u) + ((uint32_t)((ch & 15) ^ (row & 15)) << 4);
            asm volatile(
#include "cconv_pair_merge.inc"
                ::: "memory", WS_FIXED_REGS);
            asm volatile(
#include "cconv_ws_store.inc"
                :: [b] "v"(b) : "memory", WS_FIXED_REGS);
            asm volatile(
#include "cconv_pair_zero.inc"
                ::: "memory", WS_FIXED_REGS);
            ++rdone;
        };

#ifdef WS_TRACE
        uint64_t wt[16] = {0, 0, 0, 0, 0, 0, 0, 0, 0, 0, 0, 0, 0, 0, 0, 0};
        uint64_t wlast = __builtin_readcyclecounter();
        const uint64_t wstart = wlast;
        int nbatches = 0;
#endif
        int j1, j2, kk1, kk2, np0, np1, np2;
        float nv1, nv2, px, py, pz;
        uint32_t cc[16];
        f32x4 ff[8];
        {
            int j0, kk0;
            float nv0, qx, qy, qz;
            bool ok0;
            WS_IDX_STAGE(j0, nv0, kk0, np0)
            WS_IDX_STAGE(j1, nv1, kk1, np1)
            WS_IDX_STAGE(j2, nv2, kk2, np2)
            ws_ld_pos(inp_pos, j0, qx, qy, qz);
            ws_ld_pos(inp_pos, j1, px, py, pz);
            const WsRec first = ws_geom(lane, kk0, Tab, window, nval, imp, inv_r2, window_fac, inv_extent, j0, nv0, qx, qy, qz, ok0);
            push_index(j0, ok0);
            push_rec(first);
            pk_cur = pack_classes(first.cls4, cc);
            wfence();
            f_issue(np0, ff);
        }
        WT(0)
        WS_BARRIER();
        WT(5)
        f_publish(np0, ff);
        wfence();
        WT(6)
        int nblk_tile = (max(__builtin_amdgcn_readlane(ring.end, 3), __builtin_amdgcn_readlane(ring.start, 3) + 1) + 7) >> 3;
        int gend = __builtin_amdgcn_readlane(ring.start, 4) >> 6;
#pragma unroll 1
        for (int g = 0;; ++g) {
            const bool tile_last = g + 1 == gend;
            const bool more = !(tile_last && ti + 1 == T);
            WsRec nxt;
            int jn, kkn, npn;
            float nvn, qx, qy, qz;
            if (more) {
                bool ok1;
                nxt = ws_geom(64 * (g + 1) + lane, kk1, Tab, window, nval, imp, inv_r2, window_fac, inv_extent, j1, nv1, px, py, pz, ok1);
                push_index(j1, ok1);
                wfence();
                f_issue(np1, ff);
            }
            ws_ld_pos(inp_pos, j2, qx, qy, qz);
            WS_IDX_STAGE(jn, nvn, kkn, npn)
            WT(0)
            const int blo = 8 * g, bhi = min(8 * g + 8, nblk_tile);
            int b0 = blo;
            bool tile_done = false;
            for (;;) {
                const int gbk = (rdone & 3) == 3 ? nblk_tile : (__builtin_amdgcn_readlane(ring.start, (rdone + 1) & 63) >> 3);
                const int b1 = min(gbk, bhi);
                if (b1 > b0) {
                    const int sh = b0 - blo;
                    if (sh > 0) {
#pragma unroll
                        for (int m = 0; m < 16; ++m) cc[m] = (uint32_t)__builtin_amdgcn_readlane(pk_cur, (4 * m + 8 * sh) & 63);
                    }
                    splat(b1 - b0, cc, a_rec0 + (uint32_t)(2 * kWRecG * 4) * (uint32_t)sh, a_fst0 + 1024u * (uint32_t)sh);
                    b0 = b1;
                    WT(1)
                }
                if (gbk > bhi) break;
                const bool last_row = (rdone & 3) == 3;
                complete();
                WT(2)
                if (last_row) {
                    tile_done = true;
                    break;
                }
            }
            asm volatile("" : "+v"(jn), "+v"(nvn), "+v"(qx), "+v"(qy), "+v"(qz), "+v"(kkn));
#ifdef WS_TRACE
            ++nbatches;
#endif
            WT(7)
            if (tile_done) {
                WS_BARRIER();
                WT(3)
                ++ti;
                if ((ti & 7) == 0) ws_refill(kp0, (ti >> 3) + 1, lane, wave, t_begin, t_end, nslots, Tab, stream_end, ring);
                nblk_tile = (max(__builtin_amdgcn_readlane(ring.end, (4 * ti + 3) & 63), __builtin_amdgcn_readlane(ring.start, (4 * ti + 3) & 63) + 1) + 7) >> 3;
                gend = __builtin_amdgcn_readlane(ring.start, (4 * ti + 4) & 63) >> 6;
                WT(4)
                WS_BARRIER();
                WT(5)
            }
            if (!more) break;
            wfence();
            f_publish(np1, ff);
            push_rec(nxt);
            pk_cur = pack_classes(nxt.cls4, cc);
            j1 = j2;
            nv1 = nv2;
            kk1 = kk2;
            np1 = np2;
            j2 = jn;
            nv2 = nvn;
            kk2 = kkn;
            np2 = npn;
            px = qx;
            py = qy;
            pz = qz;
            wfence();
            WT(6)
        }
        WS_BARRIER();
#ifdef WS_TRACE
        if (lane == 0 && wave == 0 && (blockIdx.x & 15) == 0) {
            for (int k = 0; k < 8; ++k) atomicAdd(&g_wtrace[k], wt[k]);
            atomicAdd(&g_wtrace[8], wlast - wstart);
            atomicAdd(&g_wtrace[9], (unsigned long long)T);
            atomicAdd(&g_wtrace[10], (unsigned long long)nbatches);
        }
#endif
    } else {
        const int cw = wave - kWProd;
        const int ctid = tid - 64 * kWProd;
        const int mi = lane & 15, mg = lane >> 4;
        float* const red0 = smem + WTM * kWRow + kWProd * kWWaveF;
        const int red_half = kWCons * WTM * 16 * kWMaxNT;
        int tpar = 0;
        const int NT = kp0->NT, ncol = 16 * NT;
        constexpr int kRing = 8;
        const int cin_ring = (cin + kRing - 1) & ~(kRing - 1);
        const int nqt = cin >> 2;
        int a_tab, w_tab, w_next;
        {
            const int b = cw + 4 * (lane & 31);
            const int zy = b / nqt, qg = b - zy * nqt;
            const int chunk = qg >> 2, blk = zy * 4 + (qg & 3);
            const bool real = (lane & 31) < cin;
            a_tab = real ? chunk * 4096 + blk * 64 : -1;
            w_tab = real ? (chunk * 64 + blk) * NT * 1024 : 0x7fff0000;
            int nx = (lane & 31) + kRing;
            if (nx >= cin_ring) nx -= cin_ring;
            w_next = __shfl(w_tab, nx);
        }
        const __amdgpu_buffer_rsrc_t rW = __builtin_amdgcn_make_buffer_rsrc(
            (void*)kp0->Wp, 0, (int)((uint32_t)kp0->nchunks * 64u * (uint32_t)NT * 1024u), 0x00020000);
        uint32_t w_lane = ((uint32_t)mg * (uint32_t)NT * 16u + (uint32_t)mi) * 16u;
        f32x4 bw[kRing][NTT];
        uint32_t a_lane = wlds(Bt + mi * kWRow);
        const uint32_t lane_x = (uint32_t)((mg << 2) ^ (mi << 2)) << 2;
        int e_pt[NTT], e_o[NTT];
        float e_bias[NTT];
        const float* const bias = kp0->bias;
        const bool accumulate = (kp0->flags & DMCF_FLAG_ACCUMULATE) != 0;
#pragma unroll
        for (int r = 0; r < NTT; ++r) {
            const int e = ctid + 256 * r;
            e_pt[r] = e / cout;
            e_o[r] = e - e_pt[r] * cout;
            e_bias[r] = (bias && e < WTM * cout) ? bias[e_o[r]] : 0.0f;
        }
        float prev[NTT];
// ... 97 lines not shown
                WS_ACC_READ(3, acc[3 % NTT]);
            }
#pragma unroll
            for (int n = 0; n < NTT; ++n) {
                if (n < NT) {
#pragma unroll
                    for (int r = 0; r < 4; ++r) red0[tpar * red_half + (cw * 16 + 4 * mg + r) * ncol + n * 16 + mi] = acc[n][r];
                }
            }
            tpar ^= 1;
            WT(3)
        }
        WS_BARRIER();
#ifdef WS_TRACE
        if (lane == 0 && cw == 0 && (blockIdx.x & 15) == 0) {
            for (int k = 0; k < 4; ++k) atomicAdd(&g_wtrace[16 + k], wt[k]);
            atomicAdd(&g_wtrace[20], wlast - wstart);
        }
#endif
#ifndef WS_DBG_NOCONS
        reduce_store(kp0, red0 + (tpar ^ 1) * red_half);
#endif
    }
}

#ifdef WS_TRACE
}
extern "C" int dmcf_wtrace(unsigned long long* out) {
    unsigned long long z[32] = {0};
    (void)hipMemcpyFromSymbol(out, HIP_SYMBOL(dmcf::g_wtrace), sizeof(z));
    (void)hipMemcpyToSymbol(HIP_SYMBOL(dmcf::g_wtrace), z, sizeof(z));
    return 0;
}
namespace dmcf {
#endif

static constexpr size_t kWsLds = (size_t)(WTM * kWRow + kWProd * kWWaveF + kWRed) * sizeof(float);

static bool ws_eligible(const dmcf_cconv_args* a, int dz, int dy, int dx, bool forced) {
    if (!cconv_fast444(a, dz, dy, dx) || !cconv_offsets_fit_24bit(a) || (a->flags & DMCF_FLAG_SYMMETRIC)) return false;
    const int cin = a->filter_dims[3], cout = a->filter_dims[4];
    if (cin > 32 || cout > 16 * kWMaxNT) return false;
    if (forced) return true;
    return a->row_length_hint == 1 && cin >= 24;
}

static void ws_pick(const dmcf_cconv_args* a, int, int, int, CconvPick& k) {
    const int NT = (a->filter_dims[4] + 15) / 16;
    CconvKernel f;
    if (cconv_plain(a))
        f = NT <= 1 ? CCONV_KERNEL(cconv_ws_kernel<1, true>) : CCONV_KERNEL(cconv_ws_kernel<2, true>);
    else
        f = NT <= 1 ? CCONV_KERNEL(cconv_ws_kernel<1, false>) : CCONV_KERNEL(cconv_ws_kernel<2, false>);
    k = {f.fn, f.name, kWsLds, kWThreads, cconv_cls_packed_floats(a->filter_dims[3], a->filter_dims[4])};
}

static int ws_launch(CconvParams p, const dmcf_cconv_args* a, int, int, int, const CconvPick& k, void* workspace, hipStream_t stream) {
    if (!cconv_cls_prepare(p, a, WTM, workspace, stream)) return DMCF_EUNSUPPORTED;
    const int per_xcd = max(1, min(device_cu_count() / 8, p.tiles_per_xcd));
    void* kargs[] = {(void*)&p};
    return cconv_launch_kernel(k, dim3((unsigned)per_xcd * 8u), kargs, stream);
}

CconvForm cconv_ws_form = {'w', ws_eligible, ws_pick, cconv_cls_workspace_floats, ws_launch};

}
```

dmcf_amd/csrc/misc.hip:

```cpp
#include "common.h"

namespace dmcf {

thread_local int g_last_hip_error = 0;

constexpr int kScanThreads = 256;
constexpr int kScanItems = 8;
constexpr int kScanTile = kScanThreads * kScanItems;

template <typename T>
__device__ __forceinline__ T wave_inclusive_scan(T v) {
#pragma unroll
    for (int d = 1; d < kWave; d <<= 1) {
        T o = __shfl_up(v, d, kWave);
        if (lane_id() >= d) v += o;
    }
    return v;
}

template <typename T>
__device__ __forceinline__ T block_exclusive_scan(T v, T* total, T* smem ) {
    const int wave = threadIdx.x >> 6;
    const T inc = wave_inclusive_scan(v);
    if (lane_id() == kWave - 1) smem[wave] = inc;
// ... 188 lines not shown
        float* o = part + (size_t)blockIdx.x * 8;
        const bool b = fmaxf(fmaxf(red[2][a][0], red[2][a][1]), fmaxf(red[2][a][2], red[2][a][3])) > 0.0f;
        o[a] = b ? NAN : fminf(fminf(red[0][a][0], red[0][a][1]), fminf(red[0][a][2], red[0][a][3]));
        o[3 + a] = b ? NAN : fmaxf(fmaxf(red[1][a][0], red[1][a][1]), fmaxf(red[1][a][2], red[1][a][3]));
    }
}

__global__ void aabb_finish(const float* __restrict__ part, int nblocks, float* __restrict__ out) {
    const int lane = lane_id();
#pragma unroll
    for (int a = 0; a < 3; ++a) {
        float mn = INFINITY, mx = -INFINITY, b = 0.0f;
        for (int k = lane; k < nblocks; k += kWave) {
            const float lo = part[(size_t)k * 8 + a], hi = part[(size_t)k * 8 + 3 + a];
            b = fmaxf(b, lo != lo ? 1.0f : 0.0f);
            mn = fminf(mn, lo);
            mx = fmaxf(mx, hi);
        }
#pragma unroll
        for (int d = 32; d >= 1; d >>= 1) {
            mn = fminf(mn, __shfl_xor(mn, d, kWave));
            mx = fmaxf(mx, __shfl_xor(mx, d, kWave));
            b = fmaxf(b, __shfl_xor(b, d, kWave));
        }
        if (lane == 0) {
            out[a] = b > 0.0f ? NAN : mn;
            out[3 + a] = b > 0.0f ? NAN : mx;
        }
    }
}

__global__ __launch_bounds__(256) void reduce_subarrays_sum_kernel(const float* __restrict__ values,
                                                                   const int64_t* __restrict__ row_splits,
                                                                   int64_t n_rows, float* __restrict__ out) {
    const int64_t row = ((int64_t)blockIdx.x * blockDim.x + threadIdx.x) >> 4;
    const int sub = threadIdx.x & 15;
    if (row >= n_rows) return;
    const int64_t b = row_splits[row], e = row_splits[row + 1];
    float s = 0.0f;
    if (values) {
        for (int64_t k = b + sub; k < e; k += 16) s += values[k];
    } else {
        for (int64_t k = b + sub; k < e; k += 16) s += 1.0f;
    }
#pragma unroll
    for (int d = 8; d >= 1; d >>= 1) s += __shfl_xor(s, d, 16);
    if (sub == 0) out[row] = s;
}

}

extern "C" {

int dmcf_version(void) { return 21700; }

const char* dmcf_error_string(int code) {
    switch (code) {
        case DMCF_OK: return "ok";
        case DMCF_EINVAL: return "invalid argument";
        case DMCF_EWORKSPACE: return "workspace too small";
        case DMCF_ELAUNCH: return "HIP error while enqueuing (see dmcf_last_hip_error)";
        case DMCF_EUNSUPPORTED: return "option not implemented on the HIP path";
        default: return "unknown error code";
    }
}

int dmcf_last_hip_error(void) { return dmcf::g_last_hip_error; }

int dmcf_dense_forward(const float* x, int64_t n, int32_t k, const float* W, int32_t m, const float* bias,
                       const float* residual, float* out, dmcf_stream_t stream) {
    if (n < 0 || k <= 0 || m <= 0 || (n > 0 && (!x || !W || !out))) return DMCF_EINVAL;
    if ((k & 3) || k > 64 || m > 64) return DMCF_EUNSUPPORTED;
    if ((uintptr_t)x & 15) return DMCF_EUNSUPPORTED;
    if (n == 0) return DMCF_OK;
    const int64_t ntiles = (n + 15) / 16;
    const int64_t want = (ntiles + 3) / 4;
    const unsigned grid = (unsigned)(want < 2048 ? want : 2048);
    const int nt = (m + 15) / 16;
#define DMCF_DENSE(NTT)                                                                                                   \
    hipLaunchKernelGGL(dmcf::dense_rows<NTT>, dim3(grid), dim3(256), 0, (hipStream_t)stream, x, n, (int)k, W, (int)m, bias,  \
                       residual, out, ntiles)
    if (nt <= 1) DMCF_DENSE(1);
    else if (nt == 2) DMCF_DENSE(2);
    else DMCF_DENSE(4);
#undef DMCF_DENSE
    return dmcf::check_launch();
}

size_t dmcf_points_aabb_workspace_bytes(void) { return (size_t)dmcf::kAabbBlocks * 8 * sizeof(float); }

int dmcf_points_aabb(const float* points, int64_t n, float* out, void* workspace, size_t workspace_bytes,
                     dmcf_stream_t stream) {
    if (n < 0 || !out || (n > 0 && !points)) return DMCF_EINVAL;
    if (!workspace || workspace_bytes < dmcf_points_aabb_workspace_bytes()) return DMCF_EWORKSPACE;
    const int64_t want = (n + 1023) / 1024;
    const int nb = (int)(want < 1 ? 1 : (want > dmcf::kAabbBlocks ? dmcf::kAabbBlocks : want));
    hipLaunchKernelGGL(dmcf::aabb_partial, dim3(nb), dim3(256), 0, (hipStream_t)stream, points, n, (float*)workspace);
    hipLaunchKernelGGL(dmcf::aabb_finish, dim3(1), dim3(64), 0, (hipStream_t)stream, (const float*)workspace, nb, out);
    return dmcf::check_launch();
}

int dmcf_reduce_subarrays_sum(const float* values, const int64_t* row_splits, int64_t n_rows, float* out,
                              dmcf_stream_t stream) {
    if (n_rows < 0 || (n_rows > 0 && (!row_splits || !out))) return DMCF_EINVAL;
    if (n_rows == 0) return DMCF_OK;
    const int64_t threads = n_rows * 16;
    const unsigned grid = (unsigned)((threads + 255) / 256);
// ... 7 lines not shown
```

dmcf_amd/models/pbf_model.py:

```python
import os

import numpy as np
import torch

from .. import ops
from ..utils import convolutions as _convs
from ..utils.convolutions import ContinuousConv, PointSampling
from ..utils.tools.losses import (get_loss, compute_density, compute_pressure, compute_transformed_dx, get_dilated_pos,
                                  get_window_func)
from .base_model import BaseModel, Dense


def align_vector(v0, v1):
    v0n = v0 / (torch.linalg.norm(v0) + 1e-9)
    v1n = v1 / (torch.linalg.norm(v1) + 1e-9)
    v = torch.linalg.cross(v0n, v1n)
    c = torch.dot(v0n, v1n)
    s = torch.linalg.norm(v)
    if float(s) < 1e-6:
        return torch.eye(3, device=v0.device) * (-1.0 if float(c) < 0 else 1.0)
    zero = torch.zeros((), device=v0.device)
    vx = torch.stack([torch.stack([zero, -v[2], v[1]]), torch.stack([v[2], zero, -v[0]]),
                      torch.stack([-v[1], v[0], zero])])
    return torch.eye(3, device=v0.device) + vx + (vx @ vx) / (1 + c)
# ... 237 lines not shown
        if self.shard is not None:
            dilated_pos, idx = self.shard.dilated_pos(all_pos if self.use_bnds else pos)
        else:
            dilated_pos, _, idx = get_dilated_pos(all_pos if self.use_bnds else pos, self.strides,
                                                  voxel_size=self.voxel_size, centralize=self.centralize,
                                                  pad=self.sample_pad, hyst=self.sample_hyst)
        if self.dens_norm:
            dens = [(dens if self.use_bnds else dens[:pos.shape[0]]).unsqueeze(-1)]
            for scale in range(1, len(self.dens_radius)):
                d = self.sampling(dens[-1], dilated_pos[scale - 1], dilated_pos[scale], self.dens_radius[scale], None)
                dens.append(torch.clamp(d, min=1e-2))
        else:
            dens = None
        self.dilated_pos = dilated_pos
        return [dilated_pos, fluid_feats, idx, dens]

    def fused_input_operands(self, fluid_feats, box_feats):
        a, b = self.fluid_convs, self.obs_convs
        if (os.environ.get("DMCF_FUSE_INPUT_CONVS", "1") == "0" or _convs._CACHE.depth == 0 or not fluid_feats.is_cuda
                or self.recording()):
            return None
        if ops.search_set() != "distance":
            return None
        wa, wb = a.window_function, b.window_function
        if a.kernel is None or b.kernel is None:
            return None
        same = (isinstance(wa, _convs.WindowFunction) and isinstance(wb, _convs.WindowFunction) and wa.name == wb.name
                and wa.fac == wb.fac and tuple(a.kernel.shape[:3]) == tuple(b.kernel.shape[:3]) and a.filters == b.filters
                and all(getattr(a, k) == getattr(b, k) for k in (
                    "align_corners", "coordinate_mapping", "interpolation", "normalize", "use_bias",
                    "radius_search_ignore_query_points", "radius_search_metric", "use_dense_layer_for_center"))
                and not (a.symmetric or b.symmetric or a.circular or b.circular or a.normalize
                         or a.radius_search_ignore_query_points or a.use_dense_layer_for_center)
                and a.activation is None and b.activation is None
                and a.kernel.shape[3] == fluid_feats.shape[1] and b.kernel.shape[3] == box_feats.shape[1])
        if not same:
            return None
        n, m, cf, cb, co = fluid_feats.shape[0], box_feats.shape[0], fluid_feats.shape[1], box_feats.shape[1], a.filters
        cin = -(-(cf + cb) // 4) * 4
        feats = fluid_feats.new_zeros((n + m, cin))
        feats[:n, :cf] = fluid_feats * self.part_scale
        feats[n:, cf:cf + cb] = box_feats * self.part_scale
        kernel = a.kernel.new_zeros(tuple(a.kernel.shape[:3]) + (cin, 2 * co))
        kernel[..., :cf, :co] = a.kernel
        kernel[..., cf:cf + cb, co:] = b.kernel
        bias = torch.cat([a.bias, b.bias]) if a.use_bias else None
        return feats, kernel, bias

    def fused_input_conv(self, kernel, bias, feats, inp_pos, out_pos, extent):
        a = self.fluid_convs
        radius = float(np.float32(0.5) * np.float32(extent))
        nns = _convs._CACHE.search(a.fixed_radius_search, inp_pos, out_pos, radius, distances=False)
        index, row_splits, raw_dist = nns.raw()
        out = ops.cconv_forward(kernel, out_pos, extent, inp_pos, feats, index, row_splits, neighbors_value=raw_dist,
                                window=a.window_function.name, window_fac=a.window_function.fac,
                                align_corners=a.align_corners, coordinate_mapping=a.coordinate_mapping,
                                interpolation=a.interpolation, bias=bias, n_pairs_ref=_convs.pairs_ref(nns),
                                neighbors_row_count=getattr(nns, "row_count", None))
        a.nns = self.obs_convs.nns = None
        return out, nns

    def _fused_input_convs(self, fluid_feats, box_feats, pos, all_pos, extent):
        operands = self.fused_input_operands(fluid_feats, box_feats)
        if operands is None:
            return None
        feats, kernel, bias = operands
        n, co = fluid_feats.shape[0], self.fluid_convs.filters
        if self.conv_hook is not None:
            out = self.apply_conv(lambda f, pi, po, ext, _: self.fused_input_conv(kernel, bias, f, pi, po, ext)[0],
                                  feats, all_pos, all_pos, extent)
            self._fluid_counts = None
            return out[:, :co].contiguous(), out[:, co:].contiguous()
        out, nns = self.fused_input_conv(kernel, bias, feats, all_pos, all_pos, extent)
        index = nns.raw()[0]
        row_count = getattr(nns, "row_count", None)
        if row_count is not None:
            stride = nns.stride

            def count():
                rows = index[:n * stride].view(n, stride)
                cols = torch.arange(stride, device=index.device, dtype=torch.int32)
                return ((rows < n) & (cols[None, :] < row_count[:n, None])).sum(dim=1).to(torch.float32)
        else:
            idx, rs = nns.neighbors_index, nns.neighbors_row_splits

            def count():
                return ops.reduce_subarrays_sum((idx < n).to(torch.float32), rs)[:n]
        self._fluid_counts = count
        return out[:, :co].contiguous(), out[:, co:].contiguous()

    def loss_keys(self):
        return self.loss_fn.keys()

    def loss(self, results, data):
        pred, target = results[0], data[1]
        return {n: l(target, pred, num_fluid_neighbors=self.num_fluid_neighbors, input=data[0], target_prev=data[2],
                     pre_steps=data[3], pos_correction=self.pos_correction)
                for n, l in self.loss_fn.items()}

    def postprocess(self, prev, data, training=True, vel_corr=None, **kwargs):
        pos, vel, acc = data[:3]
        pcnt = pos.shape[0]
        if self.shard is not None:
            self._num_fluid_neighbors = None
        elif self.fluid_convs.nns is None and getattr(self, "_fluid_counts", None) is not None:
            self._num_fluid_neighbors = None
        else:
            counts = ops.neighbor_counts(self.fluid_convs.nns)
            self.num_fluid_neighbors = counts[:pcnt]

        out = prev
# ... 24 lines not shown
```

dmcf_amd/ops.py:

```python
import collections
import os
import ctypes

import threading

import numpy as np
import torch

from . import _lib

class NeighborCapacityExceeded(RuntimeError):
    """A search enqueued with estimated buffer sizes produced more pairs than the buffers hold."""


class NeighborSearchResult:

    def __init__(self, index_buf, row_splits, dist_buf, total=None, redo=None):
        self._index_buf, self._dist_buf = index_buf, dist_buf
        self.neighbors_row_splits = row_splits
        self._total = total
        self._redo = redo

    def raw(self):
        return self._index_buf, self.neighbors_row_splits, self._dist_buf

    def release(self):
        if self._index_buf is not None:
            self._capacity = self._index_buf.shape[0]
        self._index_buf = self._dist_buf = None
        self._redo = None

    @property
    def total_ref(self):
        return self.neighbors_row_splits[-1]

    @property
    def capacity(self):
        return self._index_buf.shape[0] if self._index_buf is not None else self._capacity

    def resolve(self):
        if self._total is None:
            total = int(self.neighbors_row_splits[-1].item())
            if total > self._index_buf.shape[0]:
                self._index_buf, self._dist_buf = self._redo(pair_capacity(total))
            self._total = total
        return self._total

    def overflowed(self, total):
        return self._total is None and total > self.capacity

    @property
    def neighbors_index(self):
        return self._index_buf[:self.resolve()]

    @property
    def neighbors_distance(self):
        n = self.resolve()
        return self._dist_buf[:n] if self._dist_buf.shape[0] >= n else self._dist_buf

    def __iter__(self):
        return iter((self.neighbors_index, self.neighbors_row_splits, self.neighbors_distance))

    def __getitem__(self, i):
        return tuple(self)[i]

    def __len__(self):
        return 3

class PaddedNeighborList(NeighborSearchResult):

    def __init__(self, index_buf, row_begin, dist_buf, counts, max_count, stride, redo_exact):
        super().__init__(index_buf, row_begin, dist_buf, total=None, redo=None)
        self.row_count = counts
        self.max_count = max_count
        self.stride = int(stride)
        self._redo_exact = redo_exact
        self._compact = None

    @property
    def total_ref(self):
        t = getattr(self, "_total_ref", None)
        if t is None:
            small = self.row_count.shape[0] * self.stride < 2 ** 31
            t = self._total_ref = self.row_count.sum(dtype=torch.int32) if small else self.row_count.sum()
        return t

    def release(self):
        super().release()
        self._redo_exact = None
        self._compact = None

    def overflowed(self, max_count):
        return max_count > self.stride

    def resolve(self):
        if self._compact is None:
            if int(self.max_count.item()) > self.stride:
                self._compact = self._redo_exact()
            else:
                m = self.row_count.shape[0]
                cnt = self.row_count.long()
                rs = torch.zeros(m + 1, dtype=torch.int64, device=cnt.device)
                torch.cumsum(cnt, 0, out=rs[1:])
                total = int(rs[-1].item())
                row = torch.repeat_interleave(torch.arange(m, device=cnt.device), cnt, output_size=total)
                src = row * self.stride + (torch.arange(total, device=cnt.device) - rs[:-1][row])
                dist = self._dist_buf[src] if self._dist_buf.shape[0] else self._dist_buf
                self._compact = NeighborSearchResult(self._index_buf[src], rs, dist, total=total)
        return self._compact

    @property
    def neighbors_index(self):
        return self.resolve().neighbors_index

    @property
    def neighbors_distance(self):
        return self.resolve().neighbors_distance

    @property
    def csr_row_splits(self):
        return self.resolve().neighbors_row_splits

    def __iter__(self):
        c = self.resolve()
        return iter((c.neighbors_index, c.neighbors_row_splits, c.neighbors_distance))


MAPPINGS = {"ball_to_cube_radial": 0, "ball_to_cube_volume_preserving": 1, "identity": 2}
INTERPOLATIONS = {"linear": 0, "linear_border": 1, "nearest_neighbor": 2}
WINDOWS = {None: 0, "explicit": 1, "poly6": 2, "cubic": 3, "linear": 4, "peak": 5, "cubic_grad": 6}

FLAG_ALIGN_CORNERS, FLAG_NORMALIZE, FLAG_SYMMETRIC, FLAG_ACCUMULATE, FLAG_SKIP_SELF, FLAG_FILTER_PACKED = 1, 2, 4, 8, 16, 32


class LaunchTimer:

    def __init__(self):
        self.records = []

    def begin(self):
        ev = torch.cuda.Event(enable_timing=True)
        ev.record(torch.cuda.current_stream())
        return ev

    def end(self, kind, meta, start):
        ev = torch.cuda.Event(enable_timing=True)
        ev.record(torch.cuda.current_stream())
        self.records.append((kind, meta, start, ev))

    def results(self):
        out = []
        for k, m, s, e in self.records:
            m = {a: (int(b.item()) if isinstance(b, torch.Tensor) else b) for a, b in m.items()}
            out.append((k, m, s.elapsed_time(e)))
        return out


timer = None


_raw_stream = getattr(torch._C, "_cuda_getCurrentRawStream", None)


def _stream():
    if _raw_stream is not None:
        return ctypes.c_void_p(_raw_stream(torch.cuda.current_device()))
    return ctypes.c_void_p(torch.cuda.current_stream().cuda_stream)


def _dev_f32(t, name, cols=None):
    if not isinstance(t, torch.Tensor):
        raise TypeError(f"{name} must be a torch tensor")
    if not t.is_cuda:
        raise _lib.DmcfError(f"{name} is on {t.device}: the DMCF hot path runs on the GPU only (no CPU fallback)")
    if t.dtype != torch.float32:
        raise TypeError(f"{name} must be float32, got {t.dtype}")
    if cols is not None and (t.dim() != 2 or t.shape[1] != cols):
        raise ValueError(f"{name} must have shape [n,{cols}], got {tuple(t.shape)}")
    t = t.contiguous()
    if t.data_ptr() % 16:
        t = t.clone()
    return t


def _ptr(t):
# ... 238 lines not shown
        self.normalize_distances = normalize_distances

    def __call__(self, points, queries, radii, points_row_splits=None, queries_row_splits=None):
        if points_row_splits is not None or queries_row_splits is not None:
            raise NotImplementedError("batched row_splits are not used by DMCF (batch items are looped, "
                                      "pipelines/simulator.py:68-70)")
        return radius_search(points, queries, radii, self.ignore_query_point, self.return_distances, self.normalize_distances)

    call = __call__

    def index_only(self):
        twin = getattr(self, "_index_only", None)
        if twin is None:
            twin = self._index_only = RadiusSearch(self.metric, self.ignore_query_point, False, False)
        return twin


def per_point_extents(extent, n_out):
    if not isinstance(extent, torch.Tensor) or extent.numel() == 1:
        return None
    if extent.dim() == 2 and extent.shape[1] == 3:
        raise NotImplementedError("anisotropic extents [n, 3] are not implemented")
    if tuple(extent.shape) not in ((n_out,), (n_out, 1)):
        raise ValueError(f"per-point extents must have shape [{n_out}] or [{n_out}, 1], got {tuple(extent.shape)}")
    return extent.reshape(n_out)


def _empty(t):
    return t is None or (isinstance(t, torch.Tensor) and t.numel() == 0)


def _extent_operands(extent, n_out):
    ext = per_point_extents(extent, n_out)
    if ext is None:
        return None, extent
    ext = _dev_f32(ext, "extents")
    if n_out > 0 and not bool((torch.isfinite(ext) & (ext > 0)).all()):
        raise ValueError("per-point extents must be finite and positive")
    return ext, 1.0


def _kernel_name(fn, *args, size=96, what=None):
    name = ctypes.create_string_buffer(size)
    rc = fn(*args, name, size)
    if what is not None:
        _lib.check(rc, what)
    return name.value


def _cconv_args(filters, out_positions, extent, inp_positions, inp_features, neighbors_index, neighbors_row_splits, *,
                neighbors_value=None, window=None, window_fac=1.0, inp_importance=None, align_corners=True,
                coordinate_mapping="ball_to_cube_volume_preserving", interpolation="linear", normalize=False, symmetric=False,
                sym_axis=2, bias=None, out=None, accumulate=False, neighbors_row_count=None, filter_tile_mask=0,
                skip_self=False, row_length_hint=0):
    filters = _dev_f32(filters, "filters")
    if filters.dim() != 5:
        raise ValueError("filters must have shape [D,H,W,Cin,Cout]")
    out_positions = _dev_f32(out_positions, "out_positions", 3)
    inp_positions = _dev_f32(inp_positions, "inp_positions", 3)
    cin, cout = filters.shape[3], filters.shape[4]
    if inp_features is not None:
        inp_features = _dev_f32(inp_features, "inp_features", cin)
        if inp_features.shape[0] != inp_positions.shape[0]:
            raise ValueError("inp_features and inp_positions disagree on the number of points")
    n_out = out_positions.shape[0]
    if neighbors_index.dtype != torch.int32 or neighbors_row_splits.dtype != torch.int64:
        raise TypeError("neighbors_index must be int32 and neighbors_row_splits int64")
    if neighbors_row_splits.shape[0] != n_out + 1:
        raise ValueError("neighbors_row_splits must have n_out+1 entries")
    if window not in WINDOWS:
        raise NotImplementedError(f"window {window!r}")
    if window is not None:
        if _empty(neighbors_value):
            if window == "explicit" and neighbors_index.numel() > 0:
                raise ValueError("explicit window but no per-neighbour values")
            neighbors_value = None
        else:
            neighbors_value = _dev_f32(neighbors_value, "neighbors_value")
            if neighbors_value.shape[0] != neighbors_index.shape[0]:
                raise ValueError("neighbors_value and neighbors_index disagree on the number of pairs")
    inp_importance = None if _empty(inp_importance) else _dev_f32(inp_importance, "inp_importance")
    if bias is not None:
        bias = _dev_f32(bias, "bias")
    neighbors_index = neighbors_index.contiguous()
    neighbors_row_splits = neighbors_row_splits.contiguous()
    a = _lib.CconvArgs()
    a.filters = filters.data_ptr()
    for d in range(5):
        a.filter_dims[d] = filters.shape[d]
    a.sym_axis = int(sym_axis)
    a.out_positions = out_positions.data_ptr()
    a.n_out = n_out
    a.inp_positions = inp_positions.data_ptr()
    a.n_inp = inp_positions.shape[0]
    a.inp_features = None if inp_features is None else inp_features.data_ptr()
    a.inp_importance = None if inp_importance is None else inp_importance.data_ptr()
    a.neighbors_index = neighbors_index.data_ptr()
    a.neighbors_row_splits = neighbors_row_splits.data_ptr()
    a.neighbors_value = None if window is None or neighbors_value is None else neighbors_value.data_ptr()
    a.extent = float(extent)
    a.window_fac = float(window_fac)
    a.window = WINDOWS[window]
    a.coordinate_mapping = MAPPINGS[coordinate_mapping]
    a.interpolation = INTERPOLATIONS[interpolation]
    a.flags = ((FLAG_ALIGN_CORNERS if align_corners else 0) | (FLAG_NORMALIZE if normalize else 0) |
               (FLAG_SYMMETRIC if symmetric else 0) | (FLAG_ACCUMULATE if accumulate else 0) | (FLAG_SKIP_SELF if skip_self else 0))
    a.bias = None if bias is None else bias.data_ptr()
    a.out = None if out is None else out.data_ptr()
    a.n_pairs = neighbors_index.shape[0]
    a.neighbors_row_count = None
    a.filter_tile_mask = int(filter_tile_mask) & 0xffffffff
    a.row_length_hint = int(row_length_hint)
    if neighbors_row_count is not None:
        if neighbors_row_count.dtype != torch.int32 or neighbors_row_count.shape[0] != n_out:
            raise TypeError("neighbors_row_count must be int32 [n_out]")
        neighbors_row_count = neighbors_row_count.contiguous()
        a.neighbors_row_count = neighbors_row_count.data_ptr()
    keep = (neighbors_row_count, filters, out_positions, inp_positions, inp_features, inp_importance, neighbors_index, neighbors_row_splits,
            neighbors_value, bias, out)
    return a, keep


_STENCILS = {}


def lattice_offsets(voxel, radius, device, shift=(0.0, 0.0, 0.0)):
    return _stencil(voxel, radius, device, shift)[0]


def lattice_reach(voxel, radius, device, shift=(0.0, 0.0, 0.0)):
    return list(_stencil(voxel, radius, device, shift)[1])


def _stencil(voxel, radius, device, shift):
    key = (tuple(float(v) for v in voxel), float(radius), tuple(float(v) for v in shift), str(device))
    st = _STENCILS.get(key)
    if st is None:
        v, sh = np.asarray(voxel, np.float32), np.asarray(shift, np.float32)
        reach = [int(np.floor((radius + abs(float(c))) / float(x))) + 1 if x > 0 else 0 for x, c in zip(v, sh)]
        ax = [np.arange(-r, r + 1, dtype=np.int32) for r in reach]
        dz, dy, dx = np.meshgrid(ax[2], ax[1], ax[0], indexing="ij")
        x, y, z = dx.astype(np.float32) * v[0] - sh[0], dy.astype(np.float32) * v[1] - sh[1], dz.astype(np.float32) * v[2] - sh[2]
        d2 = (x * x + y * y) + z * z
        keep = d2 <= np.float32(radius) * np.float32(radius)
        off = np.stack([dx[keep], dy[keep], dz[keep], np.zeros(int(keep.sum()), np.int32)], axis=1).astype(np.int32)
        rch = [int(np.abs(off[:, k]).max()) if off.shape[0] else 0 for k in range(3)]
        st = (torch.from_numpy(np.ascontiguousarray(off)).to(device), rch)
        _STENCILS[key] = st
    return st


def lattice_volume_box(base_min, base_dims, inp_step, reach, points_min=None, points_dims=None):
    lo, hi = [], []
    for k in range(3):
        ext = (int(base_dims[k]) + 15) // 16 * 16 if k == 0 else int(base_dims[k])
        l = int(base_min[k]) * inp_step - int(reach[k])
        h = (int(base_min[k]) + ext - 1) * inp_step + int(reach[k])
        if points_min is not None:
            l, h = min(l, int(points_min[k])), max(h, int(points_min[k]) + int(points_dims[k]) - 1)
        lo.append(l)
        hi.append(h)
    return lo, [hi[k] - lo[k] + 1 for k in range(3)]


def _lattice_args(filters, inp_volume, inp_min, out_table, out_min, n_out, voxel, extent, *, inp_step=1, out_stride=1,
                  out_phase=(0, 0, 0), rel_shift=(0.0, 0.0, 0.0), base_min=None, base_dims=None, window="poly6", window_fac=1.0,
                  align_corners=True, coordinate_mapping="ball_to_cube_volume_preserving", interpolation="linear", bias=None,
                  out=None, accumulate=False, parts=None):
    if inp_volume.dim() != 4 or inp_volume.shape[3] != filters.shape[3] or not inp_volume.is_contiguous() or not out_table.is_contiguous():
        raise ValueError("inp_volume must be a contiguous [dz, dy, dx, Cin] tensor, out_table a contiguous [dz, dy, dx] one")
    if parts is None:
        parts = [dict(out_phase=out_phase, rel_shift=rel_shift, base_min=base_min, base_dims=base_dims)]
# ... 96 lines not shown
    _lib.check(L.dmcf_lattice_conv_backward(arr, len(arr), _ptr(grad_out), _ptr(gv), _ptr(gw), _ptr(ws), nbytes, _stream()),
               "dmcf_lattice_conv_backward")
    if timer is not None:
        timer.end("cconv_backward", dict(n_out=int(n_out), cin=int(filters.shape[3]), cout=int(filters.shape[4]),
                                         filters=bool(need_filters), features=bool(need_volume), lattice=True, parts=len(arr),
                                         kernel="lat_bwd_filter;lat_bwd_input"), t0)
    del keep
    return gv, gw


class LatticeConvFunction(torch.autograd.Function):

    @staticmethod
    def forward(ctx, filters, inp_volume, bias, geo, info):
        ctx.geo = geo
        ctx.has_bias = bias is not None
        ctx.save_for_backward(filters, inp_volume)
        return lattice_conv(filters, inp_volume, bias=bias, **geo, **info)

    @staticmethod
    def backward(ctx, grad_out):
        filters, inp_volume = ctx.saved_tensors
        need_w, need_v = ctx.needs_input_grad[0], ctx.needs_input_grad[1]
        need_b = ctx.has_bias and ctx.needs_input_grad[2]
        grad_out = grad_out.contiguous()
        gv, gw = lattice_conv_backward(filters.detach(), inp_volume.detach(), grad_out=grad_out, need_volume=need_v,
                                       need_filters=need_w, **ctx.geo)
        gb = None
        if need_b:
            n_out = int(ctx.geo["n_out"])
            rows = ctx.geo["out_table"].reshape(-1).long()
            hit = torch.zeros(n_out + 1, dtype=grad_out.dtype, device=grad_out.device)
            hit[torch.where(rows >= 0, rows, torch.full_like(rows, n_out))] = 1.0
            gb = (grad_out * hit[:n_out, None]).sum(0)
        return gw, gv, gb, None, None


def block_diagonal_tile_mask(blocks):
    mask = 0
    for c0, c1, o0, o1 in blocks:
        if c1 > 32 or o1 > 64:
            return 0
        for q in range(c0 // 4, (c1 + 3) // 4):
            for n in range(o0 // 16, (o1 + 15) // 16):
                mask |= 1 << (4 * q + n)
    return mask


def cconv_forward(filters, out_positions, extent, inp_positions, inp_features, neighbors_index,
                  neighbors_row_splits, neighbors_value=None, window=None, window_fac=1.0, inp_importance=None,
                  align_corners=True, coordinate_mapping="ball_to_cube_volume_preserving", interpolation="linear",
                  normalize=False, symmetric=False, sym_axis=2, bias=None, out=None, accumulate=False,
                  n_pairs_ref=None, neighbors_row_count=None, filter_tile_mask=0, skip_self=False, name_only=False,
                  row_length_hint=0, packed_cache=None, record_per_point_extents=False):
    if not name_only and torch.is_grad_enabled() and (
            (isinstance(filters, torch.Tensor) and filters.requires_grad) or
            (isinstance(inp_features, torch.Tensor) and inp_features.requires_grad) or
            (isinstance(bias, torch.Tensor) and bias.requires_grad)):
        if out is not None or accumulate:
            raise ValueError("out= / accumulate=True cannot be recorded by autograd: use the returned tensor")
        ext = per_point_extents(extent, out_positions.shape[0])
        if ext is not None and not record_per_point_extents:
            raise NotImplementedError("recording CConv with per-point extents is opt-in: pass record_per_point_extents=True "
                                      "(the backward is dmcf_cconv_backward_extents; the extents get no gradient)")
        geo = dict(out_positions=out_positions, extent=float(extent) if ext is None else ext.detach(), inp_positions=inp_positions,
                   neighbors_index=neighbors_index, neighbors_row_splits=neighbors_row_splits, neighbors_value=neighbors_value,
                   window=window, window_fac=window_fac, inp_importance=inp_importance, align_corners=align_corners,
                   coordinate_mapping=coordinate_mapping, interpolation=interpolation, normalize=normalize, symmetric=symmetric,
                   sym_axis=sym_axis, neighbors_row_count=neighbors_row_count, skip_self=skip_self)
        res = CconvFunction.apply(filters, inp_features, geo, dict(filter_tile_mask=filter_tile_mask, row_length_hint=row_length_hint,
                                                                   n_pairs_ref=n_pairs_ref, packed_cache=packed_cache))
        if bias is not None:
            res = res + bias
        return res
    L = _lib.lib()
    n_out, cout = out_positions.shape[0], filters.shape[4]
    ext, extent = _extent_operands(extent, n_out)
    if out is None:
        if accumulate:
            raise ValueError("accumulate=True needs an out tensor")
        out = torch.empty((n_out, cout), dtype=torch.float32, device=filters.device)
    elif out.shape != (n_out, cout) or out.dtype != torch.float32 or not out.is_contiguous():
        raise ValueError("out has the wrong shape / dtype / layout")
    if inp_positions.shape[0] == 0 or n_out == 0:
        b = 0.0 if bias is None else bias.to(torch.float32)
        if accumulate:
            out += b
        else:
            out[:] = b
        return out
    a, keep = _cconv_args(filters, out_positions, extent, inp_positions, inp_features, neighbors_index, neighbors_row_splits,
                          neighbors_value=neighbors_value, window=window, window_fac=window_fac, inp_importance=inp_importance,
                          align_corners=align_corners, coordinate_mapping=coordinate_mapping, interpolation=interpolation,
                          normalize=normalize, symmetric=symmetric, sym_axis=sym_axis, bias=bias, out=out, accumulate=accumulate,
                          neighbors_row_count=neighbors_row_count, filter_tile_mask=filter_tile_mask, skip_self=skip_self,
                          row_length_hint=row_length_hint)
    kernel_name = L.dmcf_cconv_kernel_name if ext is None else L.dmcf_cconv_extents_kernel_name
    if name_only:
        return _kernel_name(kernel_name, ctypes.byref(a), what="dmcf_cconv_kernel_name").decode()
    nbytes = L.dmcf_cconv_workspace_bytes(ctypes.byref(a))
    ws = None
    if packed_cache is not None and ext is None:
        key = (filters._version, tuple(filters.shape), bool(symmetric), int(sym_axis),
               _kernel_name(L.dmcf_cconv_kernel_name, ctypes.byref(a)), str(filters.device))
        ws = packed_cache.get("ws")
        if packed_cache.get("src") is filters and packed_cache.get("key") == key and ws is not None and ws.numel() >= nbytes:
            a.flags |= FLAG_FILTER_PACKED
        else:
            ws = torch.empty(nbytes + nbytes // 4, dtype=torch.uint8, device=filters.device)
            packed_cache["key"], packed_cache["ws"], packed_cache["src"] = key, ws, filters
        nbytes = ws.numel()
    if ws is None:
        ws = torch.empty(nbytes, dtype=torch.uint8, device=filters.device)
    t0 = timer.begin() if timer is not None else None
    if ext is None:
        _lib.check(L.dmcf_cconv_forward(ctypes.byref(a), _ptr(ws), nbytes, _stream()), "dmcf_cconv_forward")
    else:
        _lib.check(L.dmcf_cconv_forward_extents(ctypes.byref(a), _ptr(ext), _ptr(ws), nbytes, _stream()), "dmcf_cconv_forward_extents")
    if timer is not None:
        kdims = [int(d) for d in filters.shape[:3]]
        if symmetric:
            kdims[int(sym_axis)] *= 2
        timer.end("cconv", dict(pairs=n_pairs_ref if n_pairs_ref is not None else int(a.n_pairs), n_out=n_out, cin=int(filters.shape[3]), cout=cout,
                                K=kdims[0] * kdims[1] * kdims[2], symmetric=bool(symmetric), kernel=_kernel_name(kernel_name, ctypes.byref(a)).decode(),
                                pair_values=bool(a.neighbors_value), accumulate=bool(accumulate)), t0)
    return out


InvertedNeighbors = collections.namedtuple("InvertedNeighbors",
                                           ["neighbors_index", "neighbors_row_splits", "neighbors_attributes", "pair_index"])


def invert_neighbors_list(num_points, inp_neighbors_index, inp_neighbors_row_splits, inp_neighbors_attributes=None,
                          neighbors_row_count=None):
    L = _lib.lib()
    index = inp_neighbors_index
    rs = inp_neighbors_row_splits
    if index.dtype != torch.int32 or rs.dtype != torch.int64:
        raise TypeError("inp_neighbors_index must be int32 and inp_neighbors_row_splits int64")
    if not index.is_cuda or not rs.is_cuda:
        raise _lib.DmcfError("invert_neighbors_list runs on the GPU only (no CPU fallback)")
    index, rs = index.contiguous(), rs.contiguous()
    n_inp, n_out, P = int(num_points), rs.shape[0] - 1, index.shape[0]
    dev = index.device
    attrs = None if _empty(inp_neighbors_attributes) else _dev_f32(inp_neighbors_attributes, "inp_neighbors_attributes")
    if attrs is not None and attrs.shape != (P,):
        raise ValueError("inp_neighbors_attributes must be a float32 [P] tensor")
    if neighbors_row_count is not None:
        if neighbors_row_count.dtype != torch.int32 or neighbors_row_count.shape[0] != n_out:
            raise TypeError("neighbors_row_count must be int32 [n_out]")
        neighbors_row_count = neighbors_row_count.contiguous()
    inv_index = torch.empty(P, dtype=torch.int32, device=dev)
    inv_pair = torch.empty(P, dtype=torch.int32, device=dev)
    inv_rs = torch.empty(n_inp + 1, dtype=torch.int64, device=dev)
    inv_attr = torch.empty(P, dtype=torch.float32, device=dev) if attrs is not None else torch.empty(0, dtype=torch.float32, device=dev)
    nbytes = int(L.dmcf_invert_neighbors_list_workspace_bytes(P))
    ws = torch.empty(nbytes, dtype=torch.uint8, device=dev)
    t0 = timer.begin() if timer is not None else None
    _lib.check(L.dmcf_invert_neighbors_list(n_inp, _ptr(index), _ptr(rs), _ptr(neighbors_row_count), n_out, P, _ptr(attrs),
                                            _ptr(inv_index), _ptr(inv_rs), _ptr(inv_pair), _ptr(inv_attr) if attrs is not None else None,
                                            _ptr(ws), nbytes, _stream()), "dmcf_invert_neighbors_list")
    if timer is not None:
        timer.end("invert", dict(pairs=P, n_inp=n_inp), t0)
    return InvertedNeighbors(inv_index, inv_rs, inv_attr, inv_pair)


def cconv_backward(filters, out_positions, extent, inp_positions, inp_features, neighbors_index, neighbors_row_splits, grad_out,
                   neighbors_value=None, window=None, window_fac=1.0, inp_importance=None, align_corners=True,
                   coordinate_mapping="ball_to_cube_volume_preserving", interpolation="linear", normalize=False, symmetric=False,
                   sym_axis=2, neighbors_row_count=None, skip_self=False, need_filters=True, need_features=True, inverted=None,
                   grad_filters=None, grad_inp_features=None, accumulate=False):
    L = _lib.lib()
    n_out, n_inp = out_positions.shape[0], inp_positions.shape[0]
    cin = filters.shape[3]
    dev = filters.device
    ext, extent = _extent_operands(extent, n_out)
    grad_out = _dev_f32(grad_out, "grad_out", filters.shape[4])
    if grad_out.shape[0] != n_out:
        raise ValueError("grad_out must be [n_out, Cout]")
# ... 1203 lines not shown
```

dmcf_amd/utils/convolutions.py:

```python
import math
import os
import threading

import numpy as np
import torch

from .. import ops
from .tools.losses import WindowFunction

__all__ = ["ContinuousConv", "neighbor_cache"]

SCATTER_OUT_CHANNELS = (4,)
SCATTER_MIN_INPUTS = 4096
SCATTER_MAX_LATTICE_CELLS = 1 << 16
SMALL_LIST_ENTRIES = 1 << 21


class _NeighborCache:

    def __init__(self):
        self.depth = 0
        self.hints = {}
        self.caps = {}
        self.totals = {}
        self.last_overflow = []
        self.expect = {}
        self.uses = {}
        self.slot_of = {}
        self.done = []
        self.use_hints = False
        self.nth = {}
        self.pending = []
        self.reports = []
        self.lists = {}
        self.tables = {}
        self.plans = {}
        self.keepalive = []
        self.key = None
        self.states = {}

    def select(self, key):
        if key == self.key:
            return
        self.states[self.key] = (self.hints, self.caps, self.expect, self.totals)
        while len(self.states) > 16:
            self.states.pop(next(iter(self.states)))
        self.hints, self.caps, self.expect, self.totals = self.states.pop(key, ({}, {}, {}, {}))
        self.key = key

    def __enter__(self):
        if self.depth == 0:
            self.nth = {}
            self.pending = []
            self.reports = []
        self.depth += 1
        return self

    def report(self, values, callback):
        if self.depth == 0:
            return bool(callback(values.flatten().tolist()))
        self.reports.append((values.flatten().long(), callback))
        return False

    def __exit__(self, exc_type, exc, tb):
        self.depth -= 1
        if self.depth == 0:
            pending, self.pending = self.pending, []
            self._flush()
            for _, _, r in pending:
                r.release()
            if exc_type is None:
                self.expect = dict(self.uses)
            self._maxc = None
            self.uses = {}
            self.slot_of = {}
            from .. import lattice
            lattice.clear()
            self.lists.clear()
            self.tables.clear()
            self.plans.clear()
            self.keepalive.clear()
            reports, self.reports = self.reports, []
            outgrown = False
            if exc_type is None and reports:
                flat = torch.cat([v for v, _ in reports]).tolist()
                at = 0
                for v, cb in reports:
                    outgrown = bool(cb(flat[at: at + v.shape[0]])) or outgrown
                    at += v.shape[0]
            if exc_type is None and outgrown and not pending:
                raise ops.NeighborCapacityExceeded("an estimated capacity was outgrown; repeat the step")
            if exc_type is None and pending:
                pad = [k for k, (_, _, r) in enumerate(pending) if isinstance(r, ops.PaddedNeighborList)]
                oth = [k for k, (_, _, r) in enumerate(pending) if not isinstance(r, ops.PaddedNeighborList)]
                parts = []
                if pad:
                    parts.append(torch.cat([pending[k][2].max_count for k in pad]).long())
                    small = [pending[k][2].row_count.shape[0] * pending[k][2].stride <= SMALL_LIST_ENTRIES for k in pad]
                    zero = ops.const_tensor([0], torch.int64, pending[pad[0]][2].row_count.device)[0]
                    parts.append(torch.stack([zero if sm else pending[k][2].total_ref.long() for k, sm in zip(pad, small)]))
                for k in oth:
                    rs = pending[k][2].neighbors_row_splits
                    parts.append(torch.stack([torch.diff(rs).max() if rs.shape[0] > 1 else rs.new_zeros(()), rs[-1]]))
                flat = torch.cat(parts).tolist()
                vals = [None] * len(pending)
                for i, k in enumerate(pad):
                    vals[k] = (flat[i], None if small[i] else flat[len(pad) + i])
                for i, k in enumerate(oth):
                    vals[k] = (flat[2 * len(pad) + 2 * i], flat[2 * len(pad) + 2 * i + 1])
                fresh, tot = {}, {}
                over = []
                for (hkey, slot, r), (mx, total) in zip(pending, vals):
                    if isinstance(r, ops.PaddedNeighborList):
                        if r.overflowed(mx):
                            over.append((hkey, "row", r.stride, int(mx)))
                    elif r.overflowed(total):
                        over.append((hkey, "pairs", r.capacity, int(total)))
                    fresh[hkey] = max(fresh.get(hkey, 0), int(mx))
                    if total is not None:
                        tot[slot] = int(total)
                self.hints.clear()
                self.hints.update(fresh)
                self.totals.clear()
                self.totals.update(tot)
                if over or self.use_hints:
                    self.last_overflow = over
                if over or outgrown:
                    raise ops.NeighborCapacityExceeded("a neighbour list outgrew its estimated capacity; repeat the step")
        return False

    @staticmethod
    def _key(t):
        return (t.data_ptr(), tuple(t.shape), t._version)

    def _max_count_slot(self, device):
        pool = getattr(self, "_maxc", None)
        if pool is None or pool[1] >= pool[0].shape[0] or pool[0].device != device:
            pool = self._maxc = [torch.zeros(64, dtype=torch.int32, device=device), 0]
        pool[1] += 1
        return pool[0][pool[1] - 1: pool[1]]

    def _flush(self):
        for r in self.done:
            r.release()
        self.done = []

    def _consumer(self, key, res):
        slot = self.slot_of[key]
        self.uses[slot] = self.uses.get(slot, 0) + 1
        if self.expect.get(slot) == self.uses[slot]:
            self.lists.pop(key, None)
            self.done.append(res)

    def scatter_plan(self, inp_positions, out_positions, voxel, radius, block_cells):
        key = (self._key(inp_positions), self._key(out_positions), float(radius), int(block_cells))
        plan = self.plans.get(key) if self.depth > 0 else None
        if plan is None:
            plan = ops.scatter_plan(inp_positions, out_positions, voxel, radius, block_cells)
            if self.depth > 0:
                self.plans[key] = plan
        return plan

    def with_query_points(self, frs, points, queries, radius):
        if self.depth == 0 or not frs.ignore_query_point:
            return None
        points = points.contiguous()
        queries = queries.contiguous()
        if self._key(points) != self._key(queries):
            return None
        key = ((self._key(points), float(radius)), self._key(queries), False, False)
        hit = self.lists.get(key)
        if hit is not None:
            self._flush()
            self._consumer(key, hit)
        return hit

    def search(self, frs, points, queries, radius, distances=True):
        if self.depth == 0:
            return frs(points, queries, radius)
        if not distances and frs.return_distances:
            frs = frs.index_only()
        self._flush()
        points = points.contiguous()
        queries = queries.contiguous()
        tkey = (self._key(points), float(radius))
        key = (tkey, self._key(queries), frs.ignore_query_point, frs.return_distances)
        hit = self.lists.get(key)
        if hit is not None:
            self._consumer(key, hit)
            return hit
        table = self.tables.get(tkey)
        if table is None or table.n_queries_capacity < queries.shape[0]:
            table = ops.build_spatial_hash_table(points, radius, n_queries=max(points.shape[0], queries.shape[0]))
            self.tables[tkey] = table
        hkey = _hint_key(frs, points, queries, radius)
        nth = self.nth.get(hkey, 0)
        self.nth[hkey] = nth + 1
        slot = (hkey, nth)
        hint = self.hints.get(hkey) if self.use_hints else None
        if hint is not None:
            stride, total = row_stride(hint), self.totals.get(slot)
            if total is not None and queries.shape[0] * stride > 4 * total + (1 << 22):
                res = frs(points, queries, radius, hash_table=table, capacity_hint=total + total // 4)
            else:
                res = frs(points, queries, radius, hash_table=table, row_stride=stride, capacity_hint=self.caps.get(slot),
                          max_count=self._max_count_slot(points.device))
                self.caps[slot] = getattr(res, "capacity", None)
        else:
            res = frs(points, queries, radius, hash_table=table)
        self.pending.append((hkey, slot, res))
        self.lists[key] = res
        self.slot_of[key] = slot
        self._consumer(key, res)
        self.keepalive.append((points, queries))
        return res


class _PerThreadCache:

    def __init__(self):
        object.__setattr__(self, "_tls", threading.local())

    def _get(self):
        c = getattr(self._tls, "cache", None)
        if c is None:
            c = self._tls.cache = _NeighborCache()
        return c

    def __getattr__(self, name):
        return getattr(self._get(), name)

    def __setattr__(self, name, value):
        setattr(self._get(), name, value)

    def __enter__(self):
        return self._get().__enter__()

    def __exit__(self, *exc):
        return self._get().__exit__(*exc)


_CACHE = _PerThreadCache()

class _CacheScope:

    def __init__(self, estimate, key=None):
        self.estimate = estimate
        self.key = key

    def __enter__(self):
        if _CACHE.depth == 0:
            self.prev = _CACHE.use_hints
            _CACHE.use_hints = bool(self.estimate) and os.environ.get("DMCF_NO_ESTIMATE") != "1"
            _CACHE._get().select(self.key)
            self.outer = True
        else:
            self.outer = False
        return _CACHE.__enter__()

    def __exit__(self, *exc):
        try:
            return _CACHE.__exit__(*exc)
# ... 86 lines not shown

    def __init__(self, filters, kernel_size, activation=None, use_bias=True, kernel_initializer="uniform",
                 bias_initializer="zeros", kernel_regularizer=None, bias_regularizer=None, align_corners=True,
                 coordinate_mapping="ball_to_cube_radial", interpolation="linear", normalize=True,
                 radius_search_ignore_query_points=False, radius_search_metric="L2", offset=None,
                 window_function=None, use_dense_layer_for_center=False,
                 dense_kernel_initializer="glorot_uniform", dense_kernel_regularizer=None, in_channels=None,
                 symmetric=False, sym_axis=2, circular=False, name=None, trainable=True, device=None,
                 record_per_point_extents=False, record_lattice_form=False, **kwargs):
        super().__init__()
        self.layer_name = name
        self.record_per_point_extents = bool(record_per_point_extents)
        self.record_lattice_form = bool(record_lattice_form)
        self.filters = filters
        self.kernel_size = [int(k) for k in kernel_size]
        if activation not in _ACTIVATIONS and not callable(activation):
            raise NotImplementedError(f"activation {activation!r}")
        self.activation = _ACTIVATIONS.get(activation, activation) if not callable(activation) else activation
        self.use_bias = use_bias
        self.kernel_initializer = kernel_initializer
        self.bias_initializer = bias_initializer
        self.align_corners = align_corners
        if coordinate_mapping not in ops.MAPPINGS:
            raise ValueError(f"coordinate_mapping {coordinate_mapping!r}")
        if interpolation not in ops.INTERPOLATIONS:
            raise ValueError(f"interpolation {interpolation!r}")
        self.coordinate_mapping = coordinate_mapping
        self.interpolation = interpolation
        self.normalize = normalize
        self.radius_search_ignore_query_points = radius_search_ignore_query_points
        self.radius_search_metric = radius_search_metric
        self.dense_kernel_initializer = dense_kernel_initializer
        self.symmetric = symmetric
        self.sym_axis = sym_axis
        self.circular = circular
        if offset is not None and any(float(o) != 0.0 for o in torch.as_tensor(offset).reshape(-1)):
            raise NotImplementedError("non-zero offset (never used by DMCF, convolutions.py:200-201)")
        self.offset = torch.zeros(3)
        self.window_function = window_function
        self.fixed_radius_search = ops.FixedRadiusSearch(
            metric=self.radius_search_metric, ignore_query_point=self.radius_search_ignore_query_points,
            return_distances=self.window_function is not None)
        self.radius_search = ops.RadiusSearch(
            metric=self.radius_search_metric, ignore_query_point=self.radius_search_ignore_query_points,
            return_distances=self.window_function is not None, normalize_distances=self.window_function is not None)
        self.use_dense_layer_for_center = use_dense_layer_for_center
        self.dense = None
        self.in_channels = None
        self.kernel = None
        self.bias = None
        self._device = device
        self.nns = None
        self._direct_kernel = None
        self.row_length_hint = 0
        self.accumulate_into = None
        self.extra_bias = None
        self._packed = {}

    def invalidate_packed(self):
        self._packed.clear()

    def _load_from_state_dict(self, *args, **kwargs):
        self._packed.clear()
        return super()._load_from_state_dict(*args, **kwargs)

    def build(self, in_channels, device=None):
        self._packed.clear()
        device = device or self._device or "cuda"
        self.in_channels = int(in_channels)
        if self.circular:
            kshape = (math.ceil(max(self.kernel_size) / 2), self.in_channels, self.filters)
        elif self.symmetric:
            sh = list(self.kernel_size)
            assert sh[self.sym_axis] % 2 == 0
            sh[self.sym_axis] = sh[self.sym_axis] // 2
            kshape = (*sh, self.in_channels, self.filters)
        else:
            kshape = (*self.kernel_size, self.in_channels, self.filters)
        self.kernel = torch.nn.Parameter(_init_tensor(self.kernel_initializer, kshape, device), requires_grad=False)
        if self.use_bias:
            self.bias = torch.nn.Parameter(_init_tensor(self.bias_initializer, (self.filters,), device),
                                           requires_grad=False)
        if self.use_dense_layer_for_center:
            w = _init_tensor(self.dense_kernel_initializer, (self.in_channels, self.filters), device)
            self.dense = torch.nn.Parameter(w, requires_grad=False)

    def _expanded_kernel(self):
        ks = self.kernel_size
        zr, yr, xr = torch.meshgrid(*[torch.arange(k, device=self.kernel.device) for k in ks], indexing="ij")
        size_xyz = torch.tensor(ks[::-1], dtype=torch.float32, device=self.kernel.device)
        gp = torch.stack([xr, yr, zr], dim=-1).to(torch.float32) - size_xyz / 2.0 + 0.5
        mask = (gp * 2.0) / size_xyz
        idx = torch.floor(gp.abs()).max(dim=-1).values.to(torch.int64)
        kernel = self.kernel[idx]
        if self.symmetric:
            kernel = kernel * mask.unsqueeze(-2)
        return kernel

    def forward(self, inp_features, inp_positions, out_positions, extents, inp_importance=None,
                fixed_radius_search_hash_table=None, user_neighbors_index=None, user_neighbors_row_splits=None,
                user_neighbors_importance=None):
        if self.kernel is None:
            with torch.no_grad():
                self.build(inp_features.shape[-1], inp_features.device)
        if self.recording(inp_features):
            return self._forward_train(inp_features, inp_positions, out_positions, extents, inp_importance,
# ... 166 lines not shown
                d["nns"] = None
                d["_n_out_last"] = out_positions.shape[0]
                d["_pairs_last"] = tl
                fuse_bias = self.use_bias and not self.use_dense_layer_for_center
                flag = _CACHE._max_count_slot(inp_positions.device) if _CACHE.depth > 0 else torch.zeros(1, dtype=torch.int32, device=inp_positions.device)
                out_features = ops.cconv_scatter_forward(
                    self.kernel, out_positions, extent, inp_positions, inp_features, t_idx, t_rb, getattr(tl, "row_count", None),
                    _CACHE.scatter_plan(inp_positions, out_positions, voxel, radius, m), window=self.window_function.name,
                    window_fac=self.window_function.fac, bias=self._epilogue_bias(fuse_bias, extra_bias), out=acc,
                    accumulate=acc is not None, n_pairs_ref=pairs_ref(tl), error_flag=flag)
                _CACHE.report(flag, _scatter_guard)
                d["_conv_values"], d["_conv_output"] = None, (None if _CACHE.depth > 0 else out_features)
                return self._finish(out_features, inp_features, extra_bias if self.use_dense_layer_for_center else None)
            if fixed_radius_search_hash_table is not None:
                d["nns"] = self.fixed_radius_search(inp_positions, out_positions, radius,
                                                    hash_table=fixed_radius_search_hash_table)
            else:
                shared = None
                if self._shares_list():
                    shared = _CACHE.with_query_points(self.fixed_radius_search, inp_positions, out_positions, radius)
                skip_self = shared is not None
                d["nns"] = shared if skip_self else _CACHE.search(
                    self.fixed_radius_search, inp_positions, out_positions, radius,
                    distances=not isinstance(self.window_function, WindowFunction))
            neighbors_index, neighbors_row_splits, raw_dist = self.nns.raw()
            row_count = getattr(self.nns, "row_count", None)
            n_pairs_ref = pairs_ref(self.nns)
            if self.window_function is not None:
                if isinstance(self.window_function, WindowFunction):
                    window, window_fac = self.window_function.name, self.window_function.fac
                    neighbors_value = raw_dist
                else:
                    q = self.nns.neighbors_distance / (np.float32(radius) * np.float32(radius))
                    neighbors_index = self.nns.neighbors_index
                    if row_count is not None:
                        neighbors_row_splits, row_count = self.nns.csr_row_splits, None
                    window, neighbors_value = "explicit", self.window_function(q).to(torch.float32)
        d["_n_out_last"] = out_positions.shape[0]
        d["_pairs_last"] = self.nns if (n_pairs_ref is None and getattr(self, "nns", None) is not None and user_neighbors_index is None) \
            else (n_pairs_ref if n_pairs_ref is not None else neighbors_index.shape[0])

        kernel, symmetric = self._conv_kernel()
        in_step = _CACHE.depth > 0
        d["_conv_values"] = {
            "filters": kernel, "out_positions": out_positions, "extents": extent, "offset": self.offset,
            "inp_positions": inp_positions, "inp_features": None if in_step else inp_features,
            "inp_importance": inp_importance,
            "neighbors_index": None if in_step else neighbors_index, "neighbors_row_splits": neighbors_row_splits,
            "neighbors_importance": None if in_step else neighbors_value, "align_corners": self.align_corners,
            "coordinate_mapping": self.coordinate_mapping, "interpolation": self.interpolation,
            "normalize": self.normalize,
        }
        fuse_bias = self.use_bias and not self.use_dense_layer_for_center
        out_features = ops.cconv_forward(
            kernel, out_positions, extent, inp_positions, inp_features, neighbors_index, neighbors_row_splits,
            neighbors_value=neighbors_value, window=window, window_fac=window_fac, inp_importance=inp_importance,
            align_corners=self.align_corners, coordinate_mapping=self.coordinate_mapping,
            interpolation=self.interpolation, normalize=self.normalize, symmetric=symmetric, sym_axis=self.sym_axis,
            bias=self._epilogue_bias(fuse_bias, extra_bias), n_pairs_ref=n_pairs_ref,
            neighbors_row_count=row_count, skip_self=skip_self, row_length_hint=self.row_length_hint,
            out=acc, accumulate=acc is not None,
            packed_cache=self._packed if (kernel is self.kernel and os.environ.get("DMCF_CACHE_PACKED_FILTERS", "1") != "0")
            else None)
        if self._direct_kernel is None and in_step and self.radius_search_ignore_query_points:
            self._direct_kernel = ops.cconv_forward(
                kernel, out_positions, extent, inp_positions, inp_features, neighbors_index, neighbors_row_splits,
                neighbors_value=neighbors_value, window=window, window_fac=window_fac, inp_importance=inp_importance,
                align_corners=self.align_corners, coordinate_mapping=self.coordinate_mapping,
                interpolation=self.interpolation, normalize=self.normalize, symmetric=symmetric, sym_axis=self.sym_axis,
                neighbors_row_count=row_count, name_only=True).startswith("cconv_direct_kernel")
            if self._shares_list() and user_neighbors_index is None and fixed_radius_search_hash_table is None:
                _CACHE.with_query_points(self.fixed_radius_search, inp_positions, out_positions,
                                         float(np.float32(0.5) * np.float32(extent)))
        d["_conv_output"] = None if in_step else out_features
        return self._finish(out_features, inp_features, extra_bias if self.use_dense_layer_for_center else None)

    def _conv_kernel(self):
        kernel, symmetric = self.kernel, self.symmetric
        if self.circular:
            if self.symmetric:
                raise NotImplementedError("circular + symmetric kernels (filters must be 3 in the reference; "
                                          "no shipped config uses circular: True)")
            kernel = self._expanded_kernel()
            symmetric = False
        if symmetric and self.normalize:
            raise NotImplementedError("symmetric=True with normalize=True (DMCF always uses normalize=False, "
                                      "models/pbf_model.py:203)")
        return kernel, symmetric

    def _extents_lists(self, inp_positions, out_positions, extents, user_neighbors_index, user_neighbors_row_splits,
                       user_neighbors_importance):
        n_out = out_positions.shape[0]
        if extents.shape[0] != n_out:
            raise ValueError(f"extents of rank 1 must hold one value per output point ({n_out}), got {extents.shape[0]}")
        window, window_fac, neighbors_value = None, 1.0, None
        if user_neighbors_index is not None and user_neighbors_row_splits is not None:
            neighbors_index, neighbors_row_splits = user_neighbors_index, user_neighbors_row_splits
            if user_neighbors_importance is not None and user_neighbors_importance.numel() > 0:
                window, neighbors_value = "explicit", user_neighbors_importance
        else:
            radii = 0.5 * extents
            named = isinstance(self.window_function, WindowFunction)
            search = self.radius_search.index_only() if named else self.radius_search
            self.__dict__["nns"] = search(inp_positions, out_positions, radii)
            neighbors_index, neighbors_row_splits, dist = self.nns
            if self.window_function is not None:
                if named:
                    window, window_fac = self.window_function.name, self.window_function.fac
                else:
                    window, neighbors_value = "explicit", self.window_function(dist).to(torch.float32)
        return neighbors_index, neighbors_row_splits, window, window_fac, neighbors_value

    def _forward_extents(self, inp_features, inp_positions, out_positions, extents, inp_importance, user_neighbors_index,
                         user_neighbors_row_splits, user_neighbors_importance, acc, extra_bias):
# ... 177 lines not shown
```

include/dmcf_hip.h:

```cpp
#ifndef DMCF_HIP_H_
#define DMCF_HIP_H_

#include <stddef.h>
#include <stdint.h>

#ifdef __cplusplus
extern "C" {
#endif

#define DMCF_OK 0
#define DMCF_EINVAL (-1)
#define DMCF_EWORKSPACE (-2)
#define DMCF_ELAUNCH (-3)
#define DMCF_EUNSUPPORTED (-4)

typedef void* dmcf_stream_t;

int dmcf_version(void);
const char* dmcf_error_string(int code);
int dmcf_last_hip_error(void);

#define DMCF_FRS_IGNORE_QUERY_POINT 1
#define DMCF_FRS_OPEN3D_CORNER_VOXELS 2
#define DMCF_FRS_OPEN3D_VOXEL_WALK 4
// ... 28 lines not shown
                             int64_t* row_splits, dmcf_stream_t stream);
int dmcf_radius_search_write(const float* queries, int64_t n_queries, int64_t n_points, const float* radii,
                             float max_radius, int flags, const void* workspace, size_t workspace_bytes,
                             const int64_t* row_splits, int32_t* neighbors_index, float* neighbors_distance,
                             int64_t pair_capacity, dmcf_stream_t stream);

enum dmcf_mapping {
    DMCF_MAP_BALL_TO_CUBE_RADIAL = 0,
    DMCF_MAP_BALL_TO_CUBE_VOLUME_PRESERVING = 1,
    DMCF_MAP_IDENTITY = 2
};
enum dmcf_interpolation { DMCF_INTERP_LINEAR = 0, DMCF_INTERP_LINEAR_BORDER = 1, DMCF_INTERP_NEAREST = 2 };
enum dmcf_window {
    DMCF_WINDOW_NONE = 0,
    DMCF_WINDOW_EXPLICIT = 1,
    DMCF_WINDOW_POLY6 = 2,
    DMCF_WINDOW_CUBIC = 3,
    DMCF_WINDOW_LINEAR = 4,
    DMCF_WINDOW_PEAK = 5,
    DMCF_WINDOW_CUBIC_GRAD = 6
};
#define DMCF_FLAG_ALIGN_CORNERS 1
#define DMCF_FLAG_NORMALIZE 2
#define DMCF_FLAG_SYMMETRIC 4
#define DMCF_FLAG_ACCUMULATE 8
#define DMCF_FLAG_FILTER_PACKED 32
#define DMCF_FLAG_SKIP_SELF 16

typedef struct dmcf_cconv_args {
    const float* filters;
    int32_t filter_dims[5];
    int32_t sym_axis;
    const float* out_positions;
    int64_t n_out;
    const float* inp_positions;
    int64_t n_inp;
    const float* inp_features;
    const float* inp_importance;
    const int32_t* neighbors_index;
    const int64_t* neighbors_row_splits;
    const float* neighbors_value;
    float extent;
    float window_fac;
    int32_t window;
    int32_t coordinate_mapping;
    int32_t interpolation;
    int32_t flags;
    const float* bias;
    float* out;
    int64_t n_pairs;
    const int32_t* neighbors_row_count;
    uint32_t filter_tile_mask;
    int32_t row_length_hint;
} dmcf_cconv_args;

size_t dmcf_cconv_workspace_bytes(const dmcf_cconv_args* args);

int dmcf_cconv_forward(const dmcf_cconv_args* args, void* workspace, size_t workspace_bytes,
                       dmcf_stream_t stream);
int dmcf_cconv_kernel_name(const dmcf_cconv_args* args, char* name, size_t name_bytes);

int dmcf_cconv_forward_extents(const dmcf_cconv_args* args, const float* out_extents, void* workspace,
                               size_t workspace_bytes, dmcf_stream_t stream);
int dmcf_cconv_extents_kernel_name(const dmcf_cconv_args* args, char* name, size_t name_bytes);

size_t dmcf_invert_neighbors_list_workspace_bytes(int64_t n_pairs);
int dmcf_invert_neighbors_list(int64_t n_inp, const int32_t* neighbors_index, const int64_t* neighbors_row_splits,
                               const int32_t* neighbors_row_count, int64_t n_out, int64_t n_pairs, const float* values,
                               int32_t* inv_index, int64_t* inv_row_splits, int32_t* inv_pair, float* inv_values,
                               void* workspace, size_t workspace_bytes, dmcf_stream_t stream);

#define DMCF_BWD_ACCUMULATE 1
typedef struct dmcf_cconv_backward_args {
    uint32_t struct_size;
    int32_t flags;
    const float* grad_out;
    const int32_t* inv_index;
    const int32_t* inv_pair;
    const int64_t* inv_row_splits;
    int64_t inv_n_rows;
    int64_t inv_n_pairs;
    float* grad_filters;
    float* grad_inp_features;
} dmcf_cconv_backward_args;

size_t dmcf_cconv_backward_workspace_bytes(const dmcf_cconv_args* fwd, const dmcf_cconv_backward_args* bwd);
int dmcf_cconv_backward(const dmcf_cconv_args* fwd, const dmcf_cconv_backward_args* bwd, void* workspace,
                        size_t workspace_bytes, dmcf_stream_t stream);
int dmcf_cconv_backward_kernel_names(const dmcf_cconv_args* fwd, const dmcf_cconv_backward_args* bwd, char* names,
                                     size_t name_bytes);

int dmcf_cconv_backward_extents(const dmcf_cconv_args* fwd, const dmcf_cconv_backward_args* bwd, const float* out_extents,
                                void* workspace, size_t workspace_bytes, dmcf_stream_t stream);
int dmcf_cconv_backward_extents_kernel_names(const dmcf_cconv_args* fwd, const dmcf_cconv_backward_args* bwd, char* names,
                                             size_t name_bytes);

size_t dmcf_cconv_scatter_plan_bytes(int64_t n_inp);
int dmcf_cconv_scatter_plan(const float* inp_positions, int64_t n_inp, const float* out_positions, int64_t n_out, float voxel,
                            float extent, int32_t block_cells, void* plan, size_t plan_bytes, dmcf_stream_t stream);

typedef struct dmcf_cconv_scatter_args {
    const float* filters;
    int32_t filter_dims[5];
    const float* out_positions;
    int64_t n_out;
    const float* inp_positions;
    int64_t n_inp;
// ... 237 lines not shown
```

Measured before the change: 13.39 million.

## Record per-pair filter geometry once and reuse it across CConv layers sharing neighbors

Adds an optional per-pair geometry record (filter coordinates plus window weight, 16 bytes per pair) that the first plain CConv layer writes while computing, and later layers sharing the same neighbor list read back instead of gathering input positions and recomputing window and coordinate mapping. A cache in the Python layer tracks which layers write and read, using the previous step's usage pattern. This trades gathered position loads and ALU work for an extra 16-byte streaming store and load per pair, plus new kernel template instantiations and bookkeeping.

```diff
diff --git a/dmcf_amd/_lib.py b/dmcf_amd/_lib.py
--- a/dmcf_amd/_lib.py
+++ b/dmcf_amd/_lib.py
@@ -37,6 +37,8 @@
         ("neighbors_row_count", ctypes.c_void_p),
         ("filter_tile_mask", ctypes.c_uint32),
         ("row_length_hint", ctypes.c_int32),
+        ("pair_geometry_out", ctypes.c_void_p),
+        ("pair_geometry", ctypes.c_void_p),
     ]
 
 
@@ -206,7 +208,7 @@
     "dmcf_version", "dmcf_error_string", "dmcf_last_hip_error",
     "dmcf_frs_workspace_bytes", "dmcf_frs_build", "dmcf_frs_count", "dmcf_frs_write", "dmcf_frs_search_padded", "dmcf_frs_window_sum",
     "dmcf_radius_search_count", "dmcf_radius_search_write",
-    "dmcf_cconv_workspace_bytes", "dmcf_cconv_forward", "dmcf_cconv_kernel_name",
+    "dmcf_cconv_workspace_bytes", "dmcf_cconv_forward", "dmcf_cconv_kernel_name", "dmcf_cconv_geometry_caps",
     "dmcf_cconv_forward_extents", "dmcf_cconv_extents_kernel_name",
     "dmcf_invert_neighbors_list_workspace_bytes", "dmcf_invert_neighbors_list",
     "dmcf_cconv_backward_workspace_bytes", "dmcf_cconv_backward", "dmcf_cconv_backward_kernel_names",
@@ -283,6 +285,8 @@
     L.dmcf_cconv_forward.argtypes = [c.POINTER(CconvArgs), c.c_void_p, c.c_size_t, c.c_void_p]
     L.dmcf_cconv_kernel_name.restype = c.c_int
     L.dmcf_cconv_kernel_name.argtypes = [c.POINTER(CconvArgs), c.c_char_p, c.c_size_t]
+    L.dmcf_cconv_geometry_caps.restype = c.c_int
+    L.dmcf_cconv_geometry_caps.argtypes = [c.POINTER(CconvArgs)]
     L.dmcf_cconv_forward_extents.restype = c.c_int
     L.dmcf_cconv_forward_extents.argtypes = [c.POINTER(CconvArgs), c.c_void_p, c.c_void_p, c.c_size_t, c.c_void_p]
     L.dmcf_cconv_extents_kernel_name.restype = c.c_int
diff --git a/dmcf_amd/csrc/cconv.hip b/dmcf_amd/csrc/cconv.hip
--- a/dmcf_amd/csrc/cconv.hip
+++ b/dmcf_amd/csrc/cconv.hip
@@ -149,6 +149,8 @@
         if (a->n_inp < a->n_out) return DMCF_EINVAL;
     }
     if (a->filter_dims[4] > 16 * kMaxNT) return DMCF_EUNSUPPORTED;
+    if (a->pair_geometry_out && a->pair_geometry) return DMCF_EINVAL;
+    if (((uintptr_t)a->pair_geometry_out | (uintptr_t)a->pair_geometry) & 15) return DMCF_EINVAL;
     if (a->n_out > 0) {
         if (!a->out_positions || !a->neighbors_row_splits) return DMCF_EINVAL;
         if (forward && (!a->filters || !a->out || !a->inp_features)) return DMCF_EINVAL;
@@ -258,6 +260,7 @@
         if ((a->flags & DMCF_FLAG_SKIP_SELF) && f != &cconv_direct_form) return DMCF_EUNSUPPORTED;
         form = f;
         f->pick(a, dz, dy, dx, k);
+        if (cconv_geo_mode(a) & ~k.geo_caps) return DMCF_EUNSUPPORTED;
         return DMCF_OK;
     }
     return DMCF_EUNSUPPORTED;
@@ -301,6 +304,7 @@
     const int rc = validate(&b);
     if (rc != DMCF_OK) return rc;
     if (a->flags & DMCF_FLAG_SKIP_SELF) return DMCF_EUNSUPPORTED;
+    if (a->pair_geometry_out || a->pair_geometry) return DMCF_EUNSUPPORTED;
     if (a->n_out > 0 && !out_extents) return DMCF_EINVAL;
     return DMCF_OK;
 }
@@ -337,6 +341,21 @@
     return DMCF_OK;
 }
 
+int dmcf_cconv_geometry_caps(const dmcf_cconv_args* a) {
+    if (!a) return DMCF_EINVAL;
+    dmcf_cconv_args b = *a;
+    b.pair_geometry_out = nullptr;
+    b.pair_geometry = nullptr;
+    int rc = validate(&b, false);
+    if (rc != DMCF_OK) return rc;
+    int dz, dy, dx;
+    full_dims(&b, dz, dy, dx);
+    const CconvForm* form;
+    CconvPick k;
+    rc = cconv_select(&b, dz, dy, dx, form, k);
+    return rc != DMCF_OK ? rc : k.geo_caps;
+}
+
 int dmcf_cconv_extents_kernel_name(const dmcf_cconv_args* a, char* name, size_t name_bytes) {
     if (!name || name_bytes < 2 || !a) return DMCF_EINVAL;
     dmcf_cconv_args b = *a;
diff --git a/dmcf_amd/csrc/cconv_cls.hip b/dmcf_amd/csrc/cconv_cls.hip
--- a/dmcf_amd/csrc/cconv_cls.hip
+++ b/dmcf_amd/csrc/cconv_cls.hip
@@ -51,8 +51,9 @@
     __builtin_amdgcn_fence(__ATOMIC_ACQUIRE, "wavefront");
 }
 
-template <int NTT, bool NARROW, bool SYM, bool SINGLE, bool PLAIN>
-__global__ __launch_bounds__(kCThreads, 4) __attribute__((amdgpu_num_vgpr(kClsCompilerVgprs))) void cconv_cls_kernel(const CconvParams p) {
+template <int NTT, bool NARROW, bool SYM, bool SINGLE, bool PLAIN, int GEO = 0>
+__global__ __launch_bounds__(kCThreads, 4) __attribute__((amdgpu_num_vgpr(kClsCompilerVgprs))) void cconv_cls_kernel(const CconvParams p, float* geo) {
+    static_assert(GEO == 0 || (PLAIN && SINGLE && !SYM), "the record serves the plain single-chunk layers");
     extern __shared__ __attribute__((aligned(16))) float smem[];
     const int tid = threadIdx.x, lane = tid & 63;
     const int wave = __builtin_amdgcn_readfirstlane(tid >> 6);
@@ -125,15 +126,26 @@
         const __amdgpu_buffer_rsrc_t rI = __builtin_amdgcn_make_buffer_rsrc(
             (void*)(p.idx + rb0), 0, near ? (int)(max((int64_t)nt0, gapB + nt1) * 4) : 0, 0x00020000);
         const uint32_t offB = (uint32_t)gapB * 4u;
+        const bool near16 = GEO != 0 && near && max((int64_t)nt0, gapB + nt1) < ((int64_t)1 << 27);
+        const __amdgpu_buffer_rsrc_t rG = __builtin_amdgcn_make_buffer_rsrc(
+            (void*)(geo + (GEO != 0 ? 4 * rb0 : 0)), 0, near16 ? (int)(max((int64_t)nt0, gapB + nt1) * 16) : 0, 0x00020000);
         auto valid = [&](int t) -> bool {
             const bool pp = t >= nbA;
             return t < NB && 64 * (t - (pp ? nbA : 0)) + lane < (pp ? nt1 : nt0);
         };
-        auto ld_idx = [&](int t, int& j, float& nv) {
+        auto ld_idx = [&](int t, int& j, float& nv, f32x4& g) {
             const bool pp = t >= nbA, ok = valid(t);
             const int o = 64 * (t - (pp ? nbA : 0)) + lane;
             j = 0;
             nv = 0.0f;
+            g = (f32x4){0.0f, 0.0f, 0.0f, 0.0f};
+            if constexpr (GEO == DMCF_GEOMETRY_READ) {
+                if (near16) {
+                    g = __builtin_bit_cast(f32x4, __builtin_amdgcn_raw_buffer_load_b128(rG, ok ? (uint32_t)o * 16u + (pp ? 4u * offB : 0u) : kOob, 0, kGeoAux));
+                } else if (ok) {
+                    g = *(const f32x4*)(geo + 4 * ((pp ? rb1 : rb0) + o));
+                }
+            }
             if (near) {
                 j = (int)__builtin_amdgcn_raw_buffer_load_b32(rI, ok ? (uint32_t)o * 4u + (pp ? offB : 0u) : kOob, 0, 0);
             } else if (ok) {
@@ -141,21 +153,42 @@
             }
             if (nval && ok) nv = nval[(pp ? rb1 : rb0) + o];
         };
-        auto ld_pos = [&](int j, float& x, float& y, float& z) {
-            const float* q = (const float*)((const char*)p.inp_pos + (size_t)__umul24((uint32_t)j, 12u));
-            x = q[0];
-            y = q[1];
-            z = q[2];
-        };
-        auto geom = [&](int t, int j, float nv, float x, float y, float z, int& cls) -> ClsRec {
+        auto ld_pos = [&](int j, const f32x4& g, float& x, float& y, float& z, float& w) {
+            if constexpr (GEO == DMCF_GEOMETRY_READ) {
+                x = g.x;
+                y = g.y;
+                z = g.z;
+                w = g.w;
+            } else {
+                const float* q = (const float*)((const char*)p.inp_pos + (size_t)__umul24((uint32_t)j, 12u));
+                x = q[0];
+                y = q[1];
+                z = q[2];
+                w = 0.0f;
+            }
+        };
+        auto st_geo = [&](int t, f32x4 g) {
+            const bool pp = t >= nbA, ok = valid(t);
+            const int o = 64 * (t - (pp ? nbA : 0)) + lane;
+            if (near16) {
+                __builtin_amdgcn_raw_buffer_store_b128(__builtin_bit_cast(u32v4, g), rG, ok ? (uint32_t)o * 16u + (pp ? 4u * offB : 0u) : kOob, 0, kGeoAux);
+            } else if (ok) {
+                *(f32x4*)(geo + 4 * ((pp ? rb1 : rb0) + o)) = g;
+            }
+        };
+        auto geom = [&](int t, int j, float nv, float x, float y, float z, float w, int& cls) -> ClsRec {
             ClsRec c;
-            const bool pp = t >= nbA;
-            x -= pp ? oxs[1] : oxs[0];
-            y -= pp ? oys[1] : oys[0];
-            z -= pp ? ozs[1] : ozs[0];
-            float a = window_value(window, nval ? nv : rel_dist2(x, y, z), p.inv_r2, p.window_fac);
-            if (imp) a *= imp[j];
-            filter_coords<false>(x, y, z, p);
+            float a = w;
+            if constexpr (GEO != DMCF_GEOMETRY_READ) {
+                const bool pp = t >= nbA;
+                x -= pp ? oxs[1] : oxs[0];
+                y -= pp ? oys[1] : oys[0];
+                z -= pp ? ozs[1] : ozs[0];
+                a = window_value(window, nval ? nv : rel_dist2(x, y, z), p.inv_r2, p.window_fac);
+                if (imp) a *= imp[j];
+                filter_coords<false>(x, y, z, p);
+                if constexpr (GEO == DMCF_GEOMETRY_WRITE) st_geo(t, (f32x4){x, y, z, a});
+            }
             c.x = fminf(3.0f, fmaxf(0.0f, x));
             y = fminf(3.0f, fmaxf(0.0f, y));
             z = fminf(3.0f, fmaxf(0.0f, z));
@@ -306,11 +339,12 @@
         if (nbA == 0) merge(wave);
         if (NB > 0) {
             int jA, jB, cl;
-            float nvA, nvB, px, py, pz;
-            ld_idx(0, jA, nvA);
-            ld_idx(1, jB, nvB);
-            ld_pos(jA, px, py, pz);
-            const ClsRec first = geom(0, jA, nvA, px, py, pz, cl);
+            float nvA, nvB, px, py, pz, pw;
+            f32x4 gA, gB;
+            ld_idx(0, jA, nvA, gA);
+            ld_idx(1, jB, nvB, gB);
+            ld_pos(jA, gA, px, py, pz, pw);
+            const ClsRec first = geom(0, jA, nvA, px, py, pz, pw, cl);
             Order oc = order(cl);
             f32x4 ff[3];
             push_index(jA, cl, oc.pos);
@@ -319,18 +353,20 @@
             f_issue(0, ff);
             jA = jB;
             nvA = nvB;
-            ld_pos(jA, px, py, pz);
+            gA = gB;
+            ld_pos(jA, gA, px, py, pz, pw);
             if constexpr (narrow) {
                 for (int t = 0; t + 1 < NB; ++t) {
                     const int nslots = oc.cb[9];
                     f_publish(t, ff);
-                    ld_idx(t + 2, jB, nvB);
-                    const ClsRec nxt = geom(t + 1, jA, nvA, px, py, pz, cl);
+                    ld_idx(t + 2, jB, nvB, gB);
+                    const ClsRec nxt = geom(t + 1, jA, nvA, px, py, pz, pw, cl);
                     const Order on = order(cl);
                     push_index(jA, cl, on.pos);
                     jA = jB;
                     nvA = nvB;
-                    ld_pos(jA, px, py, pz);
+                    gA = gB;
+                    ld_pos(jA, gA, px, py, pz, pw);
                     xfence();
                     f_issue(0, ff);
                     splat8(nslots);
@@ -347,18 +383,19 @@
                     const int nslots = oc.cb[9];
                     const bool two = nslots > kHalfSlots;
                     f_publish(t, ff);
-                    ld_idx(t + 2, jB, nvB);
+                    ld_idx(t + 2, jB, nvB, gB);
                     if (two) f_issue(1, ff);
                     xfence();
                     splat(0, nslots);
-                    const ClsRec nxt = geom(t + 1, jA, nvA, px, py, pz, cl);
+                    const ClsRec nxt = geom(t + 1, jA, nvA, px, py, pz, pw, cl);
                     const Order on = order(cl);
                     push_index(jA, cl, on.pos);
                     xfence();
                     if (two) f_publish(t, ff);
                     jA = jB;
                     nvA = nvB;
-                    ld_pos(jA, px, py, pz);
+                    gA = gB;
+                    ld_pos(jA, gA, px, py, pz, pw);
                     f_issue(0, ff);
                     if (two) {
                         xfence();
@@ -539,6 +576,13 @@
     return cconv_set_tiles(p, tm);
 }
 
+template <bool NARROW, int GEO>
+static const void* cls_geo_fn(int NT) {
+    return NT <= 1 ? (const void*)cconv_cls_kernel<1, NARROW, false, true, true, GEO>
+                   : (NT <= 2 ? (const void*)cconv_cls_kernel<2, NARROW, false, true, true, GEO>
+                              : (const void*)cconv_cls_kernel<4, NARROW, false, true, true, GEO>);
+}
+
 static void cls_pick(const dmcf_cconv_args* a, int, int, int, CconvPick& k) {
     const int cin = a->filter_dims[3], NT = (a->filter_dims[4] + 15) / 16;
     const bool sym = (a->flags & DMCF_FLAG_SYMMETRIC) != 0;
@@ -549,12 +593,17 @@
                   : CCONV_KERNEL_NT(NT, cconv_cls_kernel, NARROW, false, SINGLE, false)))
     const CconvKernel f = cin <= 8 ? CLS_PICK(true, true) : (cin <= CCH ? CLS_PICK(false, true) : CLS_PICK(false, false));
 #undef CLS_PICK
-    k = {f.fn, f.name, kClsLds, kCThreads, cconv_cls_packed_floats(cin, a->filter_dims[4])};
+    const int caps = plain && cin <= CCH ? DMCF_GEOMETRY_WRITE | DMCF_GEOMETRY_READ : 0;
+    k = {f.fn, f.name, kClsLds, kCThreads, cconv_cls_packed_floats(cin, a->filter_dims[4]), caps};
+    const int mode = cconv_geo_mode(a) & caps;
+    if (mode == DMCF_GEOMETRY_WRITE) k.fn = cin <= 8 ? cls_geo_fn<true, DMCF_GEOMETRY_WRITE>(NT) : cls_geo_fn<false, DMCF_GEOMETRY_WRITE>(NT);
+    if (mode == DMCF_GEOMETRY_READ) k.fn = cin <= 8 ? cls_geo_fn<true, DMCF_GEOMETRY_READ>(NT) : cls_geo_fn<false, DMCF_GEOMETRY_READ>(NT);
 }
 
 static int cls_launch(CconvParams p, const dmcf_cconv_args* a, int, int, int, const CconvPick& k, void* workspace, hipStream_t stream) {
     if (!cconv_cls_prepare(p, a, CTM, workspace, stream)) return DMCF_EUNSUPPORTED;
-    void* kargs[] = {(void*)&p};
+    float* geo = cconv_geo_ptr(a);
+    void* kargs[] = {(void*)&p, (void*)&geo};
     return cconv_launch_kernel(k, dim3((unsigned)p.tiles_per_xcd * 8u), kargs, stream);
 }
 
diff --git a/dmcf_amd/csrc/cconv_common.h b/dmcf_amd/csrc/cconv_common.h
--- a/dmcf_amd/csrc/cconv_common.h
+++ b/dmcf_amd/csrc/cconv_common.h
@@ -200,6 +200,7 @@
 
 typedef float f32x4 __attribute__((ext_vector_type(4)));
 typedef float f32x2 __attribute__((ext_vector_type(2)));
+typedef unsigned int u32v4 __attribute__((__vector_size__(16)));
 
 __device__ __forceinline__ void blk_divmod(int t, int nq, int& quot, int& rem) {
     const int m = nq == 1 ? 128 : (nq == 2 ? 64 : (nq == 3 ? 43 : 32));
@@ -225,7 +226,14 @@
     size_t lds;
     int threads;
     size_t packed_floats;
+    int geo_caps = 0;
 };
+
+constexpr int kGeoAux = 2;
+inline int cconv_geo_mode(const dmcf_cconv_args* a) {
+    return a->pair_geometry ? DMCF_GEOMETRY_READ : (a->pair_geometry_out ? DMCF_GEOMETRY_WRITE : 0);
+}
+inline float* cconv_geo_ptr(const dmcf_cconv_args* a) { return a->pair_geometry ? (float*)a->pair_geometry : a->pair_geometry_out; }
 
 struct CconvKernel {
     const void* fn;
diff --git a/dmcf_amd/csrc/cconv_ws.hip b/dmcf_amd/csrc/cconv_ws.hip
--- a/dmcf_amd/csrc/cconv_ws.hip
+++ b/dmcf_amd/csrc/cconv_ws.hip
@@ -107,13 +107,14 @@
 };
 
 __device__ __forceinline__ void ws_ld_idx(int sp, int r4, int o1, int o2, int o3, const float* Tab, __amdgpu_buffer_rsrc_t rI, const float* nval,
-                                          int64_t rb0, int& j, float& nv, int& kk) {
+                                          int64_t rb0, int& j, float& nv, int& kk, uint32_t& gofs) {
     kk = (r4 + (sp >= o1 ? 1 : 0) + (sp >= o2 ? 1 : 0) + (sp >= o3 ? 1 : 0)) & 63;
     const f32x2 ed = *(const f32x2*)(Tab + 2 * kk);
     const int e = __float_as_int(ed.x), d = __float_as_int(ed.y);
     const bool ok = sp < e;
     const uint32_t o = (uint32_t)sp * 4u + (uint32_t)d;
     j = (int)__builtin_amdgcn_raw_buffer_load_b32(rI, ok ? o : kWOob, 0, 0);
+    gofs = ok ? o * 4u + (uint32_t)rb0 * 16u : kWOob;
     nv = 0.0f;
     if (nval && ok) nv = nval[rb0 + (o >> 2)];
 }
@@ -125,18 +126,23 @@
     z = q[2];
 }
 
+template <bool GEO>
 __device__ __forceinline__ WsRec ws_geom(int sp, int kk, const float* Tab, int window, const float* nval, const float* imp,
-                                         float inv_r2, float window_fac, float inv_extent, int j, float nv, float x, float y, float z, bool& ok) {
+                                         float inv_r2, float window_fac, float inv_extent, int j, float nv, float x, float y, float z, float w,
+                                         bool& ok) {
     WsRec c;
     const f32x4 o = *(const f32x4*)(Tab + 128 + 4 * kk);
     ok = sp < __float_as_int(o.w);
-    x -= o.x;
-    y -= o.y;
-    z -= o.z;
-    float a = window_value(window, nval ? nv : rel_dist2(x, y, z), inv_r2, window_fac);
-    if (imp) a *= imp[j];
+    float a = w;
+    if constexpr (!GEO) {
+        x -= o.x;
+        y -= o.y;
+        z -= o.z;
+        a = window_value(window, nval ? nv : rel_dist2(x, y, z), inv_r2, window_fac);
+        if (imp) a *= imp[j];
+    }
     a = ok ? a : 0.0f;
-    ws_filter_coords(x, y, z, inv_extent);
+    if constexpr (!GEO) ws_filter_coords(x, y, z, inv_extent);
     x = fminf(3.0f, fmaxf(0.0f, x));
     y = fminf(3.0f, fmaxf(0.0f, y));
     z = fminf(3.0f, fmaxf(0.0f, z));
@@ -209,8 +215,10 @@
     wfence();
 }
 
-template <int NTT, bool PLAIN>
-__global__ __launch_bounds__(kWThreads, 1) __attribute__((amdgpu_num_vgpr(kWCompilerVgprs))) void cconv_ws_kernel(const CconvParams p_arg) {
+template <int NTT, bool PLAIN, int GEO = 0>
+__global__ __launch_bounds__(kWThreads, 1) __attribute__((amdgpu_num_vgpr(kWCompilerVgprs))) void cconv_ws_kernel(const CconvParams p_arg, float* geo) {
+    static_assert(GEO == 0 || (GEO == DMCF_GEOMETRY_READ && PLAIN), "this form reads the record of plain layers");
+    constexpr bool GR = GEO == DMCF_GEOMETRY_READ;
     extern __shared__ __attribute__((aligned(16))) float smem[];
     const WsKP kp0 = (WsKP)__builtin_amdgcn_kernarg_segment_ptr();
     const int tid = threadIdx.x, lane = tid & 63;
@@ -258,6 +266,19 @@
         const float* const inp_pos = kp->inp_pos;
         const int32_t* const idx = kp->idx;
         const __amdgpu_buffer_rsrc_t rF = __builtin_amdgcn_make_buffer_rsrc((void*)kp->inp_feat, 0, (int)((uint32_t)kp->n_inp * rowBy), 0x00020000);
+        const __amdgpu_buffer_rsrc_t rG = __builtin_amdgcn_make_buffer_rsrc((void*)geo, 0, GR ? (int)((uint32_t)kp->pair_cap * 16u) : 0, 0x00020000);
+        auto ld_pos = [=](int j, uint32_t gofs, float& x, float& y, float& z, float& w) {
+            if constexpr (GR) {
+                const f32x4 g = __builtin_bit_cast(f32x4, __builtin_amdgcn_raw_buffer_load_b128(rG, gofs, 0, kGeoAux));
+                x = g.x;
+                y = g.y;
+                z = g.z;
+                w = g.w;
+            } else {
+                ws_ld_pos(inp_pos, j, x, y, z);
+                w = 0.0f;
+            }
+        };
 
         auto push_index = [=](int j, bool ok) { Jof[lane] = ok ? __umul24((uint32_t)j, rowBy) : kWOob; };
         auto push_rec = [=](const WsRec& c) {
@@ -325,13 +346,13 @@
         rb0q = ((int64_t)__builtin_amdgcn_readlane(ring.rbhi, l0_) << 32) | (uint32_t)__builtin_amdgcn_readlane(ring.rblo, l0_); \
         rI = __builtin_amdgcn_make_buffer_rsrc((void*)(idx + rb0q), 0, __builtin_amdgcn_readlane(ring.span, l0_) * 4, 0x00020000); \
     }
-#define WS_IDX_STAGE(J, NV, KK, NP)                                                                                          \
+#define WS_IDX_STAGE(J, NV, KK, NP, GO)                                                                                       \
     {                                                                                                                        \
         if (gq >= gendq) {                                                                                                   \
             ++tq;                                                                                                            \
             WS_TILE_CTX()                                                                                                    \
         }                                                                                                                    \
-        ws_ld_idx(64 * gq + lane, 4 * tq, o1, o2, o3, Tab, rI, nval, rb0q, J, NV, KK);                                       \
+        ws_ld_idx(64 * gq + lane, 4 * tq, o1, o2, o3, Tab, rI, nval, rb0q, J, NV, KK, GO);                                   \
         NP = max(0, min(64, elastq - 64 * gq));                                                                              \
         ++gq;                                                                                                                \
     }
@@ -361,19 +382,21 @@
         int nbatches = 0;
 #endif
         int j1, j2, kk1, kk2, np0, np1, np2;
-        float nv1, nv2, px, py, pz;
+        uint32_t go2;
+        float nv1, nv2, px, py, pz, pw;
         uint32_t cc[16];
         f32x4 ff[8];
         {
             int j0, kk0;
-            float nv0, qx, qy, qz;
+            uint32_t go0, go1;
+            float nv0, qx, qy, qz, qw;
             bool ok0;
-            WS_IDX_STAGE(j0, nv0, kk0, np0)
-            WS_IDX_STAGE(j1, nv1, kk1, np1)
-            WS_IDX_STAGE(j2, nv2, kk2, np2)
-            ws_ld_pos(inp_pos, j0, qx, qy, qz);
-            ws_ld_pos(inp_pos, j1, px, py, pz);
-            const WsRec first = ws_geom(lane, kk0, Tab, window, nval, imp, inv_r2, window_fac, inv_extent, j0, nv0, qx, qy, qz, ok0);
+            WS_IDX_STAGE(j0, nv0, kk0, np0, go0)
+            WS_IDX_STAGE(j1, nv1, kk1, np1, go1)
+            WS_IDX_STAGE(j2, nv2, kk2, np2, go2)
+            ld_pos(j0, go0, qx, qy, qz, qw);
+            ld_pos(j1, go1, px, py, pz, pw);
+            const WsRec first = ws_geom<GR>(lane, kk0, Tab, window, nval, imp, inv_r2, window_fac, inv_extent, j0, nv0, qx, qy, qz, qw, ok0);
             push_index(j0, ok0);
             push_rec(first);
             pk_cur = pack_classes(first.cls4, cc);
@@ -394,16 +417,17 @@
             const bool more = !(tile_last && ti + 1 == T);
             WsRec nxt;
             int jn, kkn, npn;
-            float nvn, qx, qy, qz;
+            uint32_t gon;
+            float nvn, qx, qy, qz, qw;
             if (more) {
                 bool ok1;
-                nxt = ws_geom(64 * (g + 1) + lane, kk1, Tab, window, nval, imp, inv_r2, window_fac, inv_extent, j1, nv1, px, py, pz, ok1);
+                nxt = ws_geom<GR>(64 * (g + 1) + lane, kk1, Tab, window, nval, imp, inv_r2, window_fac, inv_extent, j1, nv1, px, py, pz, pw, ok1);
                 push_index(j1, ok1);
                 wfence();
                 f_issue(np1, ff);
             }
-            ws_ld_pos(inp_pos, j2, qx, qy, qz);
-            WS_IDX_STAGE(jn, nvn, kkn, npn)
+            ld_pos(j2, go2, qx, qy, qz, qw);
+            WS_IDX_STAGE(jn, nvn, kkn, npn, gon)
             WT(0)
             const int blo = 8 * g, bhi = min(8 * g + 8, nblk_tile);
             int b0 = blo;
@@ -431,6 +455,7 @@
                 }
             }
             asm volatile("" : "+v"(jn), "+v"(nvn), "+v"(qx), "+v"(qy), "+v"(qz), "+v"(kkn));
+            if constexpr (GR) asm volatile("" : "+v"(qw), "+v"(gon));
 #ifdef WS_TRACE
             ++nbatches;
 #endif
@@ -459,9 +484,11 @@
             nv2 = nvn;
             kk2 = kkn;
             np2 = npn;
+            go2 = gon;
             px = qx;
             py = qy;
             pz = qz;
+            pw = qw;
             wfence();
             WT(6)
         }
@@ -665,13 +692,17 @@
         f = NT <= 1 ? CCONV_KERNEL(cconv_ws_kernel<1, true>) : CCONV_KERNEL(cconv_ws_kernel<2, true>);
     else
         f = NT <= 1 ? CCONV_KERNEL(cconv_ws_kernel<1, false>) : CCONV_KERNEL(cconv_ws_kernel<2, false>);
-    k = {f.fn, f.name, kWsLds, kWThreads, cconv_cls_packed_floats(a->filter_dims[3], a->filter_dims[4])};
+    const int caps = cconv_plain(a) && a->n_pairs < ((int64_t)1 << 28) ? DMCF_GEOMETRY_READ : 0;
+    k = {f.fn, f.name, kWsLds, kWThreads, cconv_cls_packed_floats(a->filter_dims[3], a->filter_dims[4]), caps};
+    if (cconv_geo_mode(a) & caps)
+        k.fn = NT <= 1 ? (const void*)cconv_ws_kernel<1, true, DMCF_GEOMETRY_READ> : (const void*)cconv_ws_kernel<2, true, DMCF_GEOMETRY_READ>;
 }
 
 static int ws_launch(CconvParams p, const dmcf_cconv_args* a, int, int, int, const CconvPick& k, void* workspace, hipStream_t stream) {
     if (!cconv_cls_prepare(p, a, WTM, workspace, stream)) return DMCF_EUNSUPPORTED;
     const int per_xcd = max(1, min(device_cu_count() / 8, p.tiles_per_xcd));
-    void* kargs[] = {(void*)&p};
+    float* geo = cconv_geo_ptr(a);
+    void* kargs[] = {(void*)&p, (void*)&geo};
     return cconv_launch_kernel(k, dim3((unsigned)per_xcd * 8u), kargs, stream);
 }
 
diff --git a/dmcf_amd/csrc/misc.hip b/dmcf_amd/csrc/misc.hip
--- a/dmcf_amd/csrc/misc.hip
+++ b/dmcf_amd/csrc/misc.hip
@@ -264,7 +264,7 @@
 
 extern "C" {
 
-int dmcf_version(void) { return 21700; }
+int dmcf_version(void) { return 21800; }
 
 const char* dmcf_error_string(int code) {
     switch (code) {
diff --git a/dmcf_amd/models/pbf_model.py b/dmcf_amd/models/pbf_model.py
--- a/dmcf_amd/models/pbf_model.py
+++ b/dmcf_amd/models/pbf_model.py
@@ -313,11 +313,19 @@
         radius = float(np.float32(0.5) * np.float32(extent))
         nns = _convs._CACHE.search(a.fixed_radius_search, inp_pos, out_pos, radius, distances=False)
         index, row_splits, raw_dist = nns.raw()
+        geo = {}
+        if raw_dist is None and tuple(kernel.shape[:3]) == (4, 4, 4):
+            caps = ops.cconv_geometry_caps(kernel, out_pos, extent, inp_pos, feats, index, row_splits,
+                                           window=a.window_function.name, window_fac=a.window_function.fac,
+                                           align_corners=a.align_corners, coordinate_mapping=a.coordinate_mapping,
+                                           interpolation=a.interpolation, neighbors_row_count=getattr(nns, "row_count", None))
+            geo = _convs._CACHE.pair_geometry(nns, (float(np.float32(extent)), a.window_function.name, float(a.window_function.fac),
+                                                    (4, 4, 4)), caps, index)
         out = ops.cconv_forward(kernel, out_pos, extent, inp_pos, feats, index, row_splits, neighbors_value=raw_dist,
                                 window=a.window_function.name, window_fac=a.window_function.fac,
                                 align_corners=a.align_corners, coordinate_mapping=a.coordinate_mapping,
                                 interpolation=a.interpolation, bias=bias, n_pairs_ref=_convs.pairs_ref(nns),
-                                neighbors_row_count=getattr(nns, "row_count", None))
+                                neighbors_row_count=getattr(nns, "row_count", None), **geo)
         a.nns = self.obs_convs.nns = None
         return out, nns
 
diff --git a/dmcf_amd/ops.py b/dmcf_amd/ops.py
--- a/dmcf_amd/ops.py
+++ b/dmcf_amd/ops.py
@@ -14,6 +14,9 @@
 
 
 class NeighborSearchResult:
+
+    cache_slot = None
+    _pair_geometry = None
 
     def __init__(self, index_buf, row_splits, dist_buf, total=None, redo=None):
         self._index_buf, self._dist_buf = index_buf, dist_buf
@@ -29,6 +32,7 @@
             self._capacity = self._index_buf.shape[0]
         self._index_buf = self._dist_buf = None
         self._redo = None
+        self._pair_geometry = None
 
     @property
     def total_ref(self):
@@ -131,6 +135,7 @@
 WINDOWS = {None: 0, "explicit": 1, "poly6": 2, "cubic": 3, "linear": 4, "peak": 5, "cubic_grad": 6}
 
 FLAG_ALIGN_CORNERS, FLAG_NORMALIZE, FLAG_SYMMETRIC, FLAG_ACCUMULATE, FLAG_SKIP_SELF, FLAG_FILTER_PACKED = 1, 2, 4, 8, 16, 32
+GEOMETRY_WRITE, GEOMETRY_READ = 1, 2
 
 
 class LaunchTimer:
@@ -475,7 +480,7 @@
                 neighbors_value=None, window=None, window_fac=1.0, inp_importance=None, align_corners=True,
                 coordinate_mapping="ball_to_cube_volume_preserving", interpolation="linear", normalize=False, symmetric=False,
                 sym_axis=2, bias=None, out=None, accumulate=False, neighbors_row_count=None, filter_tile_mask=0,
-                skip_self=False, row_length_hint=0):
+                skip_self=False, row_length_hint=0, pair_geometry_out=None, pair_geometry=None):
     filters = _dev_f32(filters, "filters")
     if filters.dim() != 5:
         raise ValueError("filters must have shape [D,H,W,Cin,Cout]")
@@ -539,8 +544,15 @@
             raise TypeError("neighbors_row_count must be int32 [n_out]")
         neighbors_row_count = neighbors_row_count.contiguous()
         a.neighbors_row_count = neighbors_row_count.data_ptr()
+    for name, rec in (("pair_geometry_out", pair_geometry_out), ("pair_geometry", pair_geometry)):
+        if rec is None:
+            continue
+        if (not isinstance(rec, torch.Tensor) or rec.dtype != torch.float32 or rec.dim() != 2 or rec.shape[1] != 4
+                or not rec.is_contiguous() or rec.shape[0] < neighbors_index.shape[0] or rec.device != neighbors_index.device):
+            raise ValueError(f"{name} must be a contiguous float32 [>= entries of neighbors_index, 4] tensor on the list's device")
+        setattr(a, name, rec.data_ptr())
     keep = (neighbors_row_count, filters, out_positions, inp_positions, inp_features, inp_importance, neighbors_index, neighbors_row_splits,
-            neighbors_value, bias, out)
+            neighbors_value, bias, out, pair_geometry_out, pair_geometry)
     return a, keep
 
 
@@ -743,13 +755,16 @@
                   align_corners=True, coordinate_mapping="ball_to_cube_volume_preserving", interpolation="linear",
                   normalize=False, symmetric=False, sym_axis=2, bias=None, out=None, accumulate=False,
                   n_pairs_ref=None, neighbors_row_count=None, filter_tile_mask=0, skip_self=False, name_only=False,
-                  row_length_hint=0, packed_cache=None, record_per_point_extents=False):
-    if not name_only and torch.is_grad_enabled() and (
+                  row_length_hint=0, packed_cache=None, record_per_point_extents=False, pair_geometry_out=None,
+                  pair_geometry=None, caps_only=False):
+    if not name_only and not caps_only and torch.is_grad_enabled() and (
             (isinstance(filters, torch.Tensor) and filters.requires_grad) or
             (isinstance(inp_features, torch.Tensor) and inp_features.requires_grad) or
             (isinstance(bias, torch.Tensor) and bias.requires_grad)):
         if out is not None or accumulate:
             raise ValueError("out= / accumulate=True cannot be recorded by autograd: use the returned tensor")
+        if pair_geometry_out is not None or pair_geometry is not None:
+            raise ValueError("the pair geometry record is not recorded by autograd")
         ext = per_point_extents(extent, out_positions.shape[0])
         if ext is not None and not record_per_point_extents:
             raise NotImplementedError("recording CConv with per-point extents is opt-in: pass record_per_point_extents=True "
@@ -774,6 +789,8 @@
     elif out.shape != (n_out, cout) or out.dtype != torch.float32 or not out.is_contiguous():
         raise ValueError("out has the wrong shape / dtype / layout")
     if inp_positions.shape[0] == 0 or n_out == 0:
+        if caps_only:
+            return 0
         b = 0.0 if bias is None else bias.to(torch.float32)
         if accumulate:
             out += b
@@ -785,7 +802,12 @@
                           align_corners=align_corners, coordinate_mapping=coordinate_mapping, interpolation=interpolation,
                           normalize=normalize, symmetric=symmetric, sym_axis=sym_axis, bias=bias, out=out, accumulate=accumulate,
                           neighbors_row_count=neighbors_row_count, filter_tile_mask=filter_tile_mask, skip_self=skip_self,
-                          row_length_hint=row_length_hint)
+                          row_length_hint=row_length_hint, pair_geometry_out=pair_geometry_out, pair_geometry=pair_geometry)
+    if caps_only:
+        caps = 0 if ext is not None else L.dmcf_cconv_geometry_caps(ctypes.byref(a))
+        if caps < 0:
+            _lib.check(caps, "dmcf_cconv_geometry_caps")
+        return caps
     kernel_name = L.dmcf_cconv_kernel_name if ext is None else L.dmcf_cconv_extents_kernel_name
     if name_only:
         return _kernel_name(kernel_name, ctypes.byref(a), what="dmcf_cconv_kernel_name").decode()
@@ -816,6 +838,12 @@
                                 K=kdims[0] * kdims[1] * kdims[2], symmetric=bool(symmetric), kernel=_kernel_name(kernel_name, ctypes.byref(a)).decode(),
                                 pair_values=bool(a.neighbors_value), accumulate=bool(accumulate)), t0)
     return out
+
+
+def cconv_geometry_caps(filters, *args, **kw):
+    if not isinstance(filters, torch.Tensor) or not filters.is_cuda:
+        return 0
+    return cconv_forward(filters, *args, caps_only=True, **kw)
 
 
 InvertedNeighbors = collections.namedtuple("InvertedNeighbors",
diff --git a/dmcf_amd/utils/convolutions.py b/dmcf_amd/utils/convolutions.py
--- a/dmcf_amd/utils/convolutions.py
+++ b/dmcf_amd/utils/convolutions.py
@@ -26,6 +26,8 @@
         self.last_overflow = []
         self.expect = {}
         self.uses = {}
+        self.geo_expect = {}
+        self.geo_uses = {}
         self.slot_of = {}
         self.done = []
         self.use_hints = False
@@ -42,10 +44,10 @@
     def select(self, key):
         if key == self.key:
             return
-        self.states[self.key] = (self.hints, self.caps, self.expect, self.totals)
+        self.states[self.key] = (self.hints, self.caps, self.expect, self.totals, self.geo_expect)
         while len(self.states) > 16:
             self.states.pop(next(iter(self.states)))
-        self.hints, self.caps, self.expect, self.totals = self.states.pop(key, ({}, {}, {}, {}))
+        self.hints, self.caps, self.expect, self.totals, self.geo_expect = self.states.pop(key, ({}, {}, {}, {}, {}))
         self.key = key
 
     def __enter__(self):
@@ -71,8 +73,10 @@
                 r.release()
             if exc_type is None:
                 self.expect = dict(self.uses)
+                self.geo_expect = {k: tuple(v) for k, v in self.geo_uses.items()}
             self._maxc = None
             self.uses = {}
+            self.geo_uses = {}
             self.slot_of = {}
             from .. import lattice
             lattice.clear()
@@ -152,6 +156,28 @@
             self.lists.pop(key, None)
             self.done.append(res)
 
+    def pair_geometry(self, res, geokey, caps, index_buf):
+        slot = getattr(res, "cache_slot", None)
+        if self.depth == 0 or slot is None or not caps:
+            return {}
+        key = (slot, geokey)
+        seq = self.geo_uses.setdefault(key, [])
+        k = len(seq)
+        seq.append(caps)
+        if os.environ.get("DMCF_PAIR_GEOMETRY", "1") == "0":
+            return {}
+        rec = (res._pair_geometry or {}).get(geokey)
+        if rec is not None:
+            return {"pair_geometry": rec} if caps & ops.GEOMETRY_READ else {}
+        exp = self.geo_expect.get(key, ())
+        if caps & ops.GEOMETRY_WRITE and k < len(exp) and exp[k] == caps and any(c & ops.GEOMETRY_READ for c in exp[k + 1:]):
+            rec = torch.empty((index_buf.shape[0], 4), dtype=torch.float32, device=index_buf.device)
+            if res._pair_geometry is None:
+                res._pair_geometry = {}
+            res._pair_geometry[geokey] = rec
+            return {"pair_geometry_out": rec}
+        return {}
+
     def scatter_plan(self, inp_positions, out_positions, voxel, radius, block_cells):
         key = (self._key(inp_positions), self._key(out_positions), float(radius), int(block_cells))
         plan = self.plans.get(key) if self.depth > 0 else None
@@ -208,6 +234,7 @@
                 self.caps[slot] = getattr(res, "capacity", None)
         else:
             res = frs(points, queries, radius, hash_table=table)
+        res.cache_slot = slot
         self.pending.append((hkey, slot, res))
         self.lists[key] = res
         self.slot_of[key] = slot
@@ -400,6 +427,7 @@
         self._device = device
         self.nns = None
         self._direct_kernel = None
+        self._geometry_caps = None
         self.row_length_hint = 0
         self.accumulate_into = None
         self.extra_bias = None
@@ -672,6 +700,18 @@
             "normalize": self.normalize,
         }
         fuse_bias = self.use_bias and not self.use_dense_layer_for_center
+        geo = {}
+        if (in_step and getattr(getattr(self, "nns", None), "cache_slot", None) is not None and user_neighbors_index is None
+                and window is not None and neighbors_value is None and not symmetric and not skip_self and not self.normalize
+                and tuple(kernel.shape[:3]) == (4, 4, 4) and (inp_importance is None or inp_importance.numel() == 0)):
+            ck = (os.environ.get("DMCF_CCONV_KERNEL"), window, tuple(kernel.shape), row_count is None, neighbors_index.shape[0] >> 28)
+            if self._geometry_caps is None or self._geometry_caps[0] != ck:
+                d["_geometry_caps"] = (ck, ops.cconv_geometry_caps(
+                    kernel, out_positions, extent, inp_positions, inp_features, neighbors_index, neighbors_row_splits,
+                    window=window, window_fac=window_fac, align_corners=self.align_corners,
+                    coordinate_mapping=self.coordinate_mapping, interpolation=self.interpolation,
+                    neighbors_row_count=row_count, row_length_hint=self.row_length_hint))
+            geo = _CACHE.pair_geometry(self.nns, (extent, window, float(window_fac), (4, 4, 4)), self._geometry_caps[1], neighbors_index)
         out_features = ops.cconv_forward(
             kernel, out_positions, extent, inp_positions, inp_features, neighbors_index, neighbors_row_splits,
             neighbors_value=neighbors_value, window=window, window_fac=window_fac, inp_importance=inp_importance,
@@ -679,7 +719,7 @@
             interpolation=self.interpolation, normalize=self.normalize, symmetric=symmetric, sym_axis=self.sym_axis,
             bias=self._epilogue_bias(fuse_bias, extra_bias), n_pairs_ref=n_pairs_ref,
             neighbors_row_count=row_count, skip_self=skip_self, row_length_hint=self.row_length_hint,
-            out=acc, accumulate=acc is not None,
+            out=acc, accumulate=acc is not None, **geo,
             packed_cache=self._packed if (kernel is self.kernel and os.environ.get("DMCF_CACHE_PACKED_FILTERS", "1") != "0")
             else None)
         if self._direct_kernel is None and in_step and self.radius_search_ignore_query_points:
diff --git a/include/dmcf_hip.h b/include/dmcf_hip.h
--- a/include/dmcf_hip.h
+++ b/include/dmcf_hip.h
@@ -104,7 +104,13 @@
     const int32_t* neighbors_row_count;
     uint32_t filter_tile_mask;
     int32_t row_length_hint;
+    float* pair_geometry_out;
+    const float* pair_geometry;
 } dmcf_cconv_args;
+
+#define DMCF_GEOMETRY_WRITE 1
+#define DMCF_GEOMETRY_READ 2
+int dmcf_cconv_geometry_caps(const dmcf_cconv_args* args);
 
 size_t dmcf_cconv_workspace_bytes(const dmcf_cconv_args* args);
 
```

Result: no change. 13.28 million (-0.8%).
